# blairstar/NaturalDiffusion

Measured on AMD Instinct MI355X. Metric: images/sec at 15-step Natural Inference (CIFAR10 32x32, NCSN++), 3-stream throughput, higher is better.
Workload: dtype bf16; 1 GPU; CIFAR10 NI 15-step step_15_weight_173.npz B=512/GPU NCSN++ 61.8M bf16, ni_step fp64 history; nfe=15, batch_per_gpu=512, streams=3

## Files before the change

include/natinf_ncsnpp.h:

```cpp
#ifndef NATINF_NCSNPP_H
#define NATINF_NCSNPP_H

#include <stdint.h>
#include "natinf.h"

#ifdef __cplusplus
extern "C" {
#endif

typedef struct natinf_ncsnpp* natinf_ncsnpp_t;

#define NATINF_NCSNPP_KEEP_ACTIVATIONS 1
#define NATINF_NCSNPP_DDPM 2

int64_t natinf_ncsnpp_param_count(void);
int64_t natinf_ncsnpp_packed_bytes(void);
int64_t natinf_ncsnpp_handle_param_count(natinf_ncsnpp_t h);
int64_t natinf_ncsnpp_handle_packed_bytes(natinf_ncsnpp_t h);
int64_t natinf_ncsnpp_workspace_bytes(natinf_ncsnpp_t h, int max_batch);

int natinf_ncsnpp_create(natinf_ncsnpp_t* out, int flags);
int natinf_ncsnpp_destroy(natinf_ncsnpp_t h);

int natinf_ncsnpp_describe(natinf_ncsnpp_t h, char* buf, int cap);

int natinf_ncsnpp_load(natinf_ncsnpp_t h, const float* params_f32, int64_t n_params,
                       void* packed, int64_t packed_bytes, natinf_stream_t stream);

int natinf_ncsnpp_share(natinf_ncsnpp_t h, natinf_ncsnpp_t loaded);

int natinf_ncsnpp_forward(natinf_ncsnpp_t h, const float* x, const float* labels, float* out, int B,
                          void* workspace, int64_t workspace_bytes, natinf_stream_t stream);

int natinf_ncsnpp_describe_gemms(natinf_ncsnpp_t h, int B, char* buf, int cap);

int natinf_debug_gemm(int variant, int M, int N, int K0, int K1, int taps, int logW, int batch,
                      const void* a0, const void* a1, const void* b, const float* bias_n, void* c, int c_f32, float scale,
                      int iters, natinf_stream_t stream);
int natinf_debug_quant_fp8_rows(const float* w, void* q, float* row_scale, int rows, int cols, natinf_stream_t stream);
int natinf_debug_gemm_fused(int variant, int M, int N, int K, const void* a, const void* b, const float* bias_n, const float* bias_m,
                            const float* rowvec, const float* gate, int log_rows_per_sample, const void* resid_bf16, const float* resid_f32,
                            float scale, int act, void* c, int c_f32, float* gn_part, int* bm_out, int fp32_slab, natinf_stream_t stream);
int natinf_debug_set_conv_operand(int logW, const void* a1, int c1);
int natinf_debug_gemm_fp8(int M, int N, int K, const void* a8, const float* a_scale, const void* a_mx, const void* b8, const float* b_scale,
                          const float* bias_n, void* c, void* c_mx, int c_mode, int iters, natinf_stream_t stream);
int natinf_debug_conv_gn_up(int flags);
int natinf_debug_conv_gn(int res, int B, int N, int cin, int c1, const void* x, const float* scale, const float* shift, const void* w_packed, void* w_frag,
                         const void* a1, const float* bias_n, const void* resid, float out_scale, void* out, float* gn_part, int iters,
                         natinf_stream_t stream);
int natinf_set_gemm_variant(int variant);
int natinf_set_gemm_epilogue(int fp32_slab);
int natinf_set_gemm_pref512(int on);
int natinf_set_gemm_half_issue(int on);
int natinf_set_gemm_round_model(int on);
int natinf_set_gemm_w128(int on);
int natinf_set_gemm_raster(int rows);
int natinf_set_fuse_gn(int on);
int natinf_set_conv_gn_wide(int mask);
int natinf_set_conv_gn_w128(int mask);
int natinf_set_conv_gn_w128_min_k(int shape, int k);
int natinf_set_conv_gn_regw(int on);
int natinf_set_fuse_up(int on);
int natinf_set_fuse_head(int on);
int natinf_set_fuse_gn8(int on);
int natinf_set_fuse_gn4(int on);
int natinf_set_fuse_fin(int on);
int natinf_set_conv_gn_warm(int mask);
int natinf_set_attn256(int on);
int natinf_set_attn_proj(int on);
int natinf_set_attn_waves8(int on);
int natinf_set_attn_block(int on);
int natinf_set_attn_qkv(int on);
int natinf_set_conv_gn8_tile(int one_image);
int natinf_set_gemm_splitk(int on);
int natinf_debug_set_splitk_workspace(float* ws, int max_slices);
int natinf_debug_timestamps(void* dev_buf16);

int natinf_ncsnpp_profile(natinf_ncsnpp_t h, int enable);
int natinf_ncsnpp_profile_read(natinf_ncsnpp_t h, double* ms_by_class , int64_t* launches_by_class );

int natinf_gemm_profile(int enable);
int natinf_gemm_profile_read(char* buf, int cap);

int natinf_ncsnpp_debug_tap(natinf_ncsnpp_t h, int module_idx, float* out, int64_t capacity_elems,
                            natinf_stream_t stream);

#ifdef __cplusplus
}
#endif
#endif
```

naturaldiffusion_amd/_lib.py:

```python
from __future__ import annotations

import ctypes as C
import os
from pathlib import Path

os.environ.setdefault("GPU_MAX_HW_QUEUES", "8")

_HERE = Path(__file__).resolve().parent
LIB_PATH = Path(os.environ.get("NATINF_LIB", _HERE / "libnatinf.so"))

if not LIB_PATH.exists():
    raise ImportError(
        f"{LIB_PATH} not found: build it with `make -C {_HERE / 'csrc'}` "
        "(or `python -c 'import __graft_entry__ as g; g.build()'`). "
        "naturaldiffusion_amd has no CPU or eager-PyTorch fallback.")

lib = C.CDLL(str(LIB_PATH))

_p, _i32, _i64, _f32, _f64 = C.c_void_p, C.c_int, C.c_int64, C.c_float, C.c_double

SIGNATURES = {
    "natinf_abi_version": (C.c_int, []),
    "natinf_strerror": (C.c_char_p, [_i32]),
    "natinf_probe": (C.c_int, []),
    "natinf_step_f64hist": (C.c_int, [_p, _p, _p, _p, _p, _p, _p, _i32, _f64, _i32, _f64, _f64, _f32, _f32, _i64, _p]),
    "natinf_step_f32hist": (C.c_int, [_p, _p, _p, _p, _p, _p, _p, _i32, _f32, _i32, _f32, _f32, _f32, _f32, _i64, _p]),
    "natinf_weighted_sum_f64": (C.c_int, [_p, _p, _p, _p, _i32, _i64, _p]),
    "natinf_randn_philox_f32": (C.c_int, [_p, _i64, _i64, _p, _i64, _i64, C.c_uint64, _p]),
    "natinf_randn_philox_col_f32": (C.c_int, [_p, _i64, _i64, _p, _i64, _i64, C.c_uint64, C.c_uint32, _p]),
    "natinf_step_f64hist_noise": (C.c_int, [_p, _p, _p, _p, _p, _p, _p, _i32, _f64, _p, _p, _i32, _i32, _f64, _f64, _f32,
                                            C.c_uint64, _p, _i64, _i64, _i64, _i64, _p]),
    "natinf_to_pixel_u8": (C.c_int, [_p, _p, _i32, _i32, _i32, _i32, _i32, _p]),
    "natinf_step_f32prod": (C.c_int, [_p, _p, _p, _f32, _i64, _i64, _p, _p, _p, _p, _p, _i32, _f32, _p, _p, _i32,
                                      _i32, _f32, _f32, _i64, _p]),
    "natinf_step_f32prod_noise": (C.c_int, [_p, _p, _p, _f32, _i64, _i64, _p, _p, _p, _p, _p, _i32, _f32, _p, _p, _i32,
                                            _i32, _f32, _f32, C.c_uint64, _p, _i64, _i64, _i64, _p]),
    "natinf_weighted_sum_f32prod": (C.c_int, [_p, _p, _p, _p, _i32, _i64, _p]),
    "natinf_step_f16chain": (C.c_int, [_p, _p, _p, _p, _p, _p, _p, _p, _p, _i32, _f32, _f32, _i32, _f32, _f32, _f32,
                                       _f32, _i32, _i64, _p]),
    "natinf_weighted_mean_f16": (C.c_int, [_p, _p, _p, _p, _i32, _f32, _i64, _p]),
    "natinf_flow_input_f16": (C.c_int, [_p, _p, _p, _f32, _f32, _i64, _p]),
    "natinf_ncsnpp_param_count": (C.c_int64, []),
    "natinf_ncsnpp_workspace_bytes": (C.c_int64, [_p, _i32]),
    "natinf_ncsnpp_packed_bytes": (C.c_int64, []),
    "natinf_ncsnpp_handle_param_count": (_i64, [_p]),
    "natinf_ncsnpp_handle_packed_bytes": (_i64, [_p]),
    "natinf_ncsnpp_create": (C.c_int, [C.POINTER(_p), _i32]),
    "natinf_ncsnpp_describe": (C.c_int, [_p, C.c_char_p, _i32]),
    "natinf_ncsnpp_destroy": (C.c_int, [_p]),
    "natinf_ncsnpp_load": (C.c_int, [_p, _p, _i64, _p, _i64, _p]),
    "natinf_ncsnpp_share": (C.c_int, [_p, _p]),
    "natinf_ncsnpp_forward": (C.c_int, [_p, _p, _p, _p, _i32, _p, _i64, _p]),
    "natinf_ncsnpp_debug_tap": (C.c_int, [_p, _i32, _p, _i64, _p]),
    "natinf_ncsnpp_describe_gemms": (C.c_int, [_p, _i32, C.c_char_p, _i32]),
    "natinf_debug_gemm": (C.c_int, [_i32, _i32, _i32, _i32, _i32, _i32, _i32, _i32, _p, _p, _p, _p, _p, _i32, _f32, _i32, _p]),
    "natinf_set_gemm_variant": (C.c_int, [_i32]),
    "natinf_debug_timestamps": (C.c_int, [_p]),
    "natinf_set_gemm_epilogue": (C.c_int, [_i32]),
    "natinf_debug_gemm_fused": (C.c_int, [_i32, _i32, _i32, _i32, _p, _p, _p, _p, _p, _p, _i32, _p, _p, _f32, _i32, _p, _i32, _p, _p, _i32, _p]),
    "natinf_set_gemm_pref512": (C.c_int, [_i32]),
    "natinf_set_gemm_half_issue": (C.c_int, [_i32]),
    "natinf_set_gemm_raster": (C.c_int, [_i32]),
    "natinf_set_gemm_round_model": (C.c_int, [_i32]),
    "natinf_set_gemm_w128": (C.c_int, [_i32]),
    "natinf_set_fuse_gn": (C.c_int, [_i32]),
    "natinf_set_conv_gn_wide": (C.c_int, [_i32]),
    "natinf_set_attn_block": (C.c_int, [_i32]),
    "natinf_set_conv_gn_w128": (C.c_int, [_i32]),
    "natinf_set_conv_gn_w128_min_k": (C.c_int, [_i32, _i32]),
    "natinf_set_conv_gn_regw": (C.c_int, [_i32]),
    "natinf_set_fuse_up": (C.c_int, [_i32]),
    "natinf_set_fuse_head": (C.c_int, [_i32]),
    "natinf_set_fuse_gn8": (C.c_int, [_i32]),
    "natinf_set_fuse_gn4": (C.c_int, [_i32]),
    "natinf_set_fuse_fin": (C.c_int, [_i32]),
    "natinf_set_attn_proj": (C.c_int, [_i32]),
    "natinf_set_attn_waves8": (C.c_int, [_i32]),
    "natinf_set_attn_qkv": (C.c_int, [_i32]),
    "natinf_set_conv_gn_warm": (C.c_int, [_i32]),
    "natinf_set_attn256": (C.c_int, [_i32]),
    "natinf_set_conv_gn8_tile": (C.c_int, [_i32]),
    "natinf_set_gemm_splitk": (C.c_int, [_i32]),
    "natinf_debug_set_splitk_workspace": (C.c_int, [_p, _i32]),
    "natinf_debug_set_conv_operand": (C.c_int, [_i32, _p, _i32]),
    "natinf_debug_conv_gn": (C.c_int, [_i32, _i32, _i32, _i32, _i32, _p, _p, _p, _p, _p, _p, _p, _p, _f32, _p, _p, _i32, _p]),
    "natinf_debug_conv_gn_up": (C.c_int, [_i32]),
    "natinf_ncsnpp_profile": (C.c_int, [_p, _i32]),
    "natinf_ncsnpp_profile_read": (C.c_int, [_p, C.POINTER(C.c_double), C.POINTER(C.c_int64)]),
    "natinf_debug_quant_fp8_rows": (C.c_int, [_p, _p, _p, _i32, _i32, _p]),
    "natinf_debug_gemm_fp8": (C.c_int, [_i32, _i32, _i32, _p, _p, _p, _p, _p, _p, _p, _p, _i32, _i32, _p]),
    "natinf_dit_create": (C.c_int, [C.POINTER(_p), _i32, _i32, _i32, _i32]),
    "natinf_dit_create_sized": (C.c_int, [C.POINTER(_p), _i32, _i32, _i32, _i32, _i32]),
    "natinf_dit_input_size": (C.c_int, [_p]),
    "natinf_dit_attention_bf16": (C.c_int, [_p, _p, _p, _i32, _p, _i32, _i32, _i32, _i32, _i32, _i32, _p]),
    "natinf_dit_destroy": (C.c_int, [_p]),
    "natinf_dit_param_count": (C.c_int64, [_p]),
    "natinf_dit_packed_bytes": (C.c_int64, [_p]),
    "natinf_dit_workspace_bytes": (C.c_int64, [_p, _i32]),
    "natinf_dit_load": (C.c_int, [_p, _p, _i64, _p, _i64, _p]),
    "natinf_dit_forward": (C.c_int, [_p, _p, _p, _p, _p, _i32, _p, _i64, _p]),
    "natinf_mmdit_create": (C.c_int, [C.POINTER(_p), _i32, _i32, _i32, _i32, _i32, _i32, _i32, _i32]),
    "natinf_mmdit_destroy": (C.c_int, [_p]),
    "natinf_mmdit_param_count": (C.c_int64, [_p]),
    "natinf_mmdit_packed_bytes": (C.c_int64, [_p]),
    "natinf_mmdit_workspace_bytes": (C.c_int64, [_p, _i32]),
    "natinf_mmdit_load": (C.c_int, [_p, _p, _i64, _p, _i64, _p]),
    "natinf_mmdit_forward": (C.c_int, [_p, _p, _p, _p, _p, _p, _i32, _p, _i64, _p]),
    "natinf_attention_hd64_bf16": (C.c_int, [_p, _p, _i32, _i64, _p, _p, _i32, _i64, _i32, _i32, _i32, _i32, C.c_float, _p]),
    "natinf_inception_create": (C.c_int, [_p, _i32, _i32]),
    "natinf_inception_destroy": (C.c_int, [_p]),
    "natinf_set_inception_conv": (C.c_int, [_i32]),
    "natinf_debug_conv_ring": (C.c_int, [_i32] * 14 + [_p, _p, _p, _p, _p, _p, _i32, _p]),
    "natinf_inception_param_count": (_i64, [_p]),
    "natinf_inception_packed_bytes": (_i64, [_p]),
    "natinf_inception_workspace_bytes": (_i64, [_p, _i32]),
    "natinf_inception_load": (C.c_int, [_p, _p, _i64, _p, _i64, _p]),
    "natinf_inception_forward": (C.c_int, [_p, _p, _i32, _p, _i32, _p, _i64, _p]),
    "natinf_gemm_profile": (C.c_int, [_i32]),
    "natinf_gemm_profile_read": (C.c_int, [_p, _i32]),
    "natinf_set_mmdit_stream16": (C.c_int, [_i32]),
    "natinf_set_dit_stream16": (C.c_int, [_i32]),
    "natinf_set_mmdit_text_flat": (C.c_int, [_i32]),
    "natinf_attention_profile": (C.c_int, [_i32]),
    "natinf_set_mmdit_text_stream": (C.c_int, [_i32]),
    "natinf_set_flash_mode": (C.c_int, [_i32]),
    "natinf_attention_profile_read": (C.c_int, [_p, _p]),
    "natinf_vae_create": (C.c_int, [C.POINTER(_p), _i32, _i32]),
    "natinf_vae_destroy": (C.c_int, [_p]),
    "natinf_vae_param_count": (C.c_int64, [_p]),
    "natinf_vae_packed_bytes": (C.c_int64, [_p]),
    "natinf_vae_workspace_bytes": (C.c_int64, [_p, _i32]),
    "natinf_vae_load": (C.c_int, [_p, _p, _i64, _p, _i64, _p]),
    "natinf_vae_decode": (C.c_int, [_p, _p, _p, _i32, _p, _i64, _p]),
}

for _name, (_res, _args) in SIGNATURES.items():
    try:
        _fn = getattr(lib, _name)
    except AttributeError as e:
        raise ImportError(f"{LIB_PATH} does not export {_name}; rebuild it") from e
    _fn.restype, _fn.argtypes = _res, _args

SD3_CFG_ON_VELOCITY = 1


def check(rc: int, what: str) -> None:
    if rc != 0:
        raise RuntimeError(f"{what} failed: {lib.natinf_strerror(rc).decode()} ({rc})")


def stream_ptr(stream=None) -> int:
    import torch
    s = stream if stream is not None else torch.cuda.current_stream()
    return int(s.cuda_stream)


def ptr(t) -> int:
    return 0 if t is None else int(t.data_ptr())


def require_gpu() -> None:
    import torch
    if not torch.cuda.is_available():
        raise RuntimeError("naturaldiffusion_amd needs an MI355X (gfx950) GPU: torch.cuda.is_available() is False "
                           "and there is no CPU fallback")
    check(lib.natinf_probe(), "natinf_probe")
```

naturaldiffusion_amd/csrc/attn_blk256.h:

```cpp
#pragma once
#include "attn_qkv.h"
#include "attn256.h"

namespace ncsn {

constexpr int ABLK_STAGES = 4, ABLK_LDS_BYTES = ABLK_STAGES * A256_STAGE + QKV_BIAS_BYTES;

__device__ __forceinline__ float dpp_row_sum_tau(float a, float b) {
    asm volatile("s_nop 4" : "+v"(a), "+v"(b));
    a += __builtin_bit_cast(float, __builtin_amdgcn_update_dpp(0, __builtin_bit_cast(int, a), 0x128, 0xF, 0xF, true));
    b += __builtin_bit_cast(float, __builtin_amdgcn_update_dpp(0, __builtin_bit_cast(int, b), 0x128, 0xF, 0xF, true));
    asm volatile("" : "+v"(a), "+v"(b));
    a += __builtin_bit_cast(float, __builtin_amdgcn_update_dpp(0, __builtin_bit_cast(int, a), 0xB1, 0xF, 0xF, true));
    b += __builtin_bit_cast(float, __builtin_amdgcn_update_dpp(0, __builtin_bit_cast(int, b), 0xB1, 0xF, 0xF, true));
    asm volatile("" : "+v"(a), "+v"(b));
    a += __builtin_bit_cast(float, __builtin_amdgcn_update_dpp(0, __builtin_bit_cast(int, a), 0x4E, 0xF, 0xF, true));
    b += __builtin_bit_cast(float, __builtin_amdgcn_update_dpp(0, __builtin_bit_cast(int, b), 0x4E, 0xF, 0xF, true));
    asm volatile("" : "+v"(a), "+v"(b));
    float v = a + b;
    asm volatile("s_nop 1" : "+v"(v));
    v += __builtin_bit_cast(float, __builtin_amdgcn_update_dpp(0, __builtin_bit_cast(int, v), 0x141, 0xF, 0xF, true));
    asm volatile("" : "+v"(v));
    return v;
}
// ... 167 lines not shown
#pragma unroll
    for (int kt = 0; kt < NKT; ++kt) {
        asm volatile("s_waitcnt vmcnt(8)" ::: "memory");
        __builtin_amdgcn_s_barrier();
        issue(kt + 3);
        __builtin_amdgcn_sched_barrier(0);
        const unsigned char* sK = smem + (kt & 3) * A256_STAGE;
#pragma unroll
        for (int tl = 0; tl < 4; ++tl)
#pragma unroll
            for (int c = 0; c < 8; ++c) {
                const int row = 32 * (tl >> 1) + 4 * (tl & 1) + krow;
                const bf16x8 fa = *reinterpret_cast<const bf16x8*>(sK + row * 512 + (((4 * c + q) ^ r) << 4));
                acc[0][4 * kt + tl] = __builtin_amdgcn_mfma_f32_16x16x32_bf16(fa, qf[0][c], acc[0][4 * kt + tl], 0, 0, 0);
                acc[1][4 * kt + tl] = __builtin_amdgcn_mfma_f32_16x16x32_bf16(fa, qf[1][c], acc[1][4 * kt + tl], 0, 0, 0);
            }
    }
    float inv[2];
#pragma unroll
    for (int g = 0; g < 2; ++g) {
        float mx = -INFINITY;
#pragma unroll
        for (int t = 0; t < 16; ++t)
#pragma unroll
            for (int i = 0; i < 4; ++i) mx = fmaxf(mx, acc[g][t][i]);
        mx = fmaxf(mx, __shfl_xor(mx, 16));
        mx = fmaxf(mx, __shfl_xor(mx, 32));
        float sum = 0.f;
#pragma unroll
        for (int t = 0; t < 16; ++t)
#pragma unroll
            for (int i = 0; i < 4; ++i) { const float p = __expf((acc[g][t][i] - mx) * scale); acc[g][t][i] = p; sum += p; }
        sum += __shfl_xor(sum, 16);
        sum += __shfl_xor(sum, 32);
        inv[g] = 1.0f / sum;
        __builtin_amdgcn_sched_barrier(0);
    }
    bf16x8 pf[2][8];
#pragma unroll
    for (int c = 0; c < 8; ++c)
#pragma unroll
        for (int g = 0; g < 2; ++g)
#pragma unroll
            for (int i = 0; i < 4; ++i) { pf[g][c][i] = (bf16)(acc[g][2 * c][i] * inv[g]); pf[g][c][4 + i] = (bf16)(acc[g][2 * c + 1][i] * inv[g]); }
    __builtin_amdgcn_sched_barrier(0);
    f32x4 oacc[2][16];
#pragma unroll
    for (int dt = 0; dt < 16; ++dt) { oacc[0][dt] = f32x4{0.f, 0.f, 0.f, 0.f}; oacc[1][dt] = f32x4{0.f, 0.f, 0.f, 0.f}; }
#pragma unroll
    for (int vt = 0; vt < NKT; ++vt) {
        asm volatile("s_waitcnt vmcnt(8)" ::: "memory");
        __builtin_amdgcn_s_barrier();
        issue(NKT + vt + 3);
        __builtin_amdgcn_sched_barrier(0);
        const unsigned char* sV = smem + ((NKT + vt) & 3) * A256_STAGE;
#pragma unroll
        for (int cc = 0; cc < 2; ++cc)
#pragma unroll
            for (int dt = 0; dt < 16; ++dt) {
                const bf16x8 fv = *reinterpret_cast<const bf16x8*>(sV + (16 * dt + r) * 128 + (((4 * cc + q) ^ (r >> 1)) << 4));
                oacc[0][dt] = __builtin_amdgcn_mfma_f32_16x16x32_bf16(fv, pf[0][2 * vt + cc], oacc[0][dt], 0, 0, 0);
                oacc[1][dt] = __builtin_amdgcn_mfma_f32_16x16x32_bf16(fv, pf[1][2 * vt + cc], oacc[1][dt], 0, 0, 0);
            }
    }
    bf16x8 of[2][8];
#pragma unroll
    for (int g = 0; g < 2; ++g)
#pragma unroll
        for (int kc = 0; kc < 8; ++kc)
#pragma unroll
            for (int i = 0; i < 4; ++i) { of[g][kc][i] = (bf16)oacc[g][2 * kc][i]; of[g][kc][4 + i] = (bf16)oacc[g][2 * kc + 1][i]; }
    __builtin_amdgcn_sched_barrier(0);
    int le;
    asm volatile("v_mbcnt_lo_u32_b32 %0, -1, 0\n\tv_mbcnt_hi_u32_b32 %0, -1, %0" : "=v"(le));
    const int re = le & 15, qe = le >> 4;
    float2* const sred = reinterpret_cast<float2*>(smem);
    float2 part[16];
#pragma unroll
    for (int t = 0; t < 4; ++t) {
        asm volatile("s_waitcnt vmcnt(0)" ::: "memory");
        __syncthreads();
        if (t + 3 < 4) issue(2 * NKT + t + 3);
        __builtin_amdgcn_sched_barrier(0);
        const unsigned char* sW = smem + ((2 * NKT + t) & 3) * A256_STAGE;
        f32x4 a3[2][4];
#pragma unroll
        for (int ntl = 0; ntl < 4; ++ntl) { a3[0][ntl] = f32x4{0.f, 0.f, 0.f, 0.f}; a3[1][ntl] = f32x4{0.f, 0.f, 0.f, 0.f}; }
#pragma unroll
        for (int ntl = 0; ntl < 4; ++ntl)
#pragma unroll
            for (int kc = 0; kc < 8; ++kc) {
                const bf16x8 fa = *reinterpret_cast<const bf16x8*>(sW + (ntl * 8 + kc) * 1024 + le * 16);
                a3[0][ntl] = __builtin_amdgcn_mfma_f32_16x16x32_bf16(fa, of[0][kc], a3[0][ntl], 0, 0, 0);
                a3[1][ntl] = __builtin_amdgcn_mfma_f32_16x16x32_bf16(fa, of[1][kc], a3[1][ntl], 0, 0, 0);
            }
#pragma unroll
        for (int pr = 0; pr < 2; ++pr) {
            const int n = 64 * t + 32 * pr + 8 * qe;
            const float4 b0 = *reinterpret_cast<const float4*>(b3 + n), b1 = *reinterpret_cast<const float4*>(b3 + n + 4);
            float s0[2], ss0[2], s1[2], ss1[2];
#pragma unroll
            for (int g = 0; g < 2; ++g) {
                const int64_t row = (int64_t)b * T + tok0 + 8 * (re >> 2) + 4 * g + (re & 3);
                const bf16x8 rx = *reinterpret_cast<const bf16x8*>(x + row * x_ld + n);
                const f32x4 lo = a3[g][2 * pr], hi = a3[g][2 * pr + 1];
                float v[8] = {lo[0] + b0.x, lo[1] + b0.y, lo[2] + b0.z, lo[3] + b0.w, hi[0] + b1.x, hi[1] + b1.y, hi[2] + b1.z, hi[3] + b1.w};
                bf16x8 w;
#pragma unroll
                for (int i = 0; i < 8; ++i) { v[i] = (v[i] + (float)rx[i]) * out_scale; w[i] = (bf16)v[i]; }
                *reinterpret_cast<bf16x8*>(o + row * o_ld + n) = w;
                s0[g] = (v[0] + v[1]) + (v[2] + v[3]);  ss0[g] = (v[0] * v[0] + v[1] * v[1]) + (v[2] * v[2] + v[3] * v[3]);
                s1[g] = (v[4] + v[5]) + (v[6] + v[7]);  ss1[g] = (v[4] * v[4] + v[5] * v[5]) + (v[6] * v[6] + v[7] * v[7]);
            }
            part[4 * t + 2 * pr] = make_float2(dpp_row_sum_tau(s0[0], s0[1]), dpp_row_sum_tau(ss0[0], ss0[1]));
            part[4 * t + 2 * pr + 1] = make_float2(dpp_row_sum_tau(s1[0], s1[1]), dpp_row_sum_tau(ss1[0], ss1[1]));
        }
    }
    if (gn_part) {
        __syncthreads();
        if (re == 0) {
#pragma unroll
            for (int k = 0; k < 16; ++k) sred[wave * 64 + 8 * (k >> 1) + 2 * qe + (k & 1)] = part[k];
        }
        __syncthreads();
        if (tid < 64) {
            float s = 0.f, ss = 0.f;
#pragma unroll
            for (int w = 0; w < 8; ++w) { s += sred[w * 64 + tid].x; ss += sred[w * 64 + tid].y; }
            gn_part[(int64_t)b * gn_quads + tid] = make_float2(s, ss);
        }
    }
}

constexpr int ABLK2_IMG = 131072, ABLK2_LDS_BYTES = ABLK2_IMG + A256_STAGE;
static_assert(4 * QKV_STAGE <= ABLK2_IMG && ABLK2_LDS_BYTES <= 163840, "the q phase's four stages inside the image's bytes; image + one W3 tile in 160 KB");

__global__ __launch_bounds__(256) void k_attn_fold_w(const float* __restrict__ w0, const float* __restrict__ w1, const float* __restrict__ w2, const float* __restrict__ w3,
                                                      const float* __restrict__ b0, const float* __restrict__ b2, const float* __restrict__ b3,
                                                      float* __restrict__ wqk, float* __restrict__ cq, float* __restrict__ wvo, float* __restrict__ bo)
{
    const int o = threadIdx.x, i = blockIdx.x;
    float a = 0.f, c = 0.f;
    if (i < 256) {
        for (int m = 0; m < 256; ++m) { a += w0[i * 256 + m] * w1[o * 256 + m]; c += w2[i * 256 + m] * w3[m * 256 + o]; }
        wqk[i * 256 + o] = a; wvo[i * 256 + o] = c;
    } else {
        for (int m = 0; m < 256; ++m) { a += b0[m] * w1[o * 256 + m]; c += b2[m] * w3[m * 256 + o]; }
        cq[o] = a; bo[o] = c + b3[o];
    }
}

__global__ __launch_bounds__(512, 1) void k_attn_blk256_v2(const bf16* __restrict__ x, int x_ld, const float* __restrict__ gsc, const float* __restrict__ gsh,
                                                          const bf16* __restrict__ wqf, const float* __restrict__ cq, float scale, const bf16* __restrict__ wvof,
                                                          const float* __restrict__ bo, bf16* __restrict__ o, int o_ld, float out_scale, float2* __restrict__ gn_part, int gn_quads)
{
    constexpr int T = 256, C = 256, NTQ = 8;
    extern __shared__ __attribute__((aligned(16))) unsigned char smem[];
    lds_poison();
    typedef __attribute__((address_space(3))) void lds_void;
    typedef __attribute__((address_space(3))) unsigned char lds_u8;
    const int tid = threadIdx.x, lane = tid & 63, r = lane & 15, q = lane >> 4;
    const int wave = __builtin_amdgcn_readfirstlane(tid >> 6);
    const int b = blockIdx.x;
    const int tok0 = wave * 32;
    const unsigned lds0 = (unsigned)(uintptr_t)((lds_u8*)smem);

    constexpr int NST = 4, AHEAD = NST - 1;
    auto issue_w = [&](int i) __attribute__((always_inline)) {
        unsigned char* st = smem + (i & (NST - 1)) * QKV_STAGE;
        int l;
        asm volatile("v_mbcnt_lo_u32_b32 %0, -1, 0\n\tv_mbcnt_hi_u32_b32 %0, -1, %0" : "=v"(l));
        const bf16* base = wqf + (int64_t)i * (QKV_STAGE / 2);
#pragma unroll
        for (int j = 0; j < QKV_STAGE / 8192; ++j) {
            const int p = wave * (QKV_STAGE / 8192) + j;
            __builtin_amdgcn_global_load_lds(base + p * 512 + l * 8, (lds_void*)(st + p * 1024), 16, 0, 0);
        }
    };
    issue_w(0); issue_w(1); issue_w(2);
    float* const sBias = reinterpret_cast<float*>(smem + ABLK2_IMG);
    const unsigned lds_bias = lds0 + ABLK2_IMG;
    if (tid < 64) reinterpret_cast<float4*>(sBias)[tid] = reinterpret_cast<const float4*>(cq)[tid];

    bf16x8 qf[2][8];
    {
        bf16x8 hf[2][8];
        {
            const bf16* xb = x + ((int64_t)b * T + tok0 + 8 * (r >> 2) + (r & 3)) * x_ld + 8 * q;
            bf16x8 raw[2][8];
#pragma unroll
            for (int g = 0; g < 2; ++g)
#pragma unroll
                for (int kc = 0; kc < 8; ++kc) raw[g][kc] = *reinterpret_cast<const bf16x8*>(xb + (int64_t)(4 * g) * x_ld + 32 * kc);
            const float* sc = gsc + (int64_t)b * C + 8 * q;
            const float* sh = gsh + (int64_t)b * C + 8 * q;
#pragma unroll
            for (int kc = 0; kc < 8; ++kc) {
                const float4 s0 = *reinterpret_cast<const float4*>(sc + 32 * kc), s1 = *reinterpret_cast<const float4*>(sc + 32 * kc + 4);
                const float4 h0 = *reinterpret_cast<const float4*>(sh + 32 * kc), h1 = *reinterpret_cast<const float4*>(sh + 32 * kc + 4);
                const float s[8] = {s0.x, s0.y, s0.z, s0.w, s1.x, s1.y, s1.z, s1.w}, h[8] = {h0.x, h0.y, h0.z, h0.w, h1.x, h1.y, h1.z, h1.w};
#pragma unroll
                for (int g = 0; g < 2; ++g)
#pragma unroll
                    for (int j = 0; j < 8; ++j) hf[g][kc][j] = (bf16)((float)raw[g][kc][j] * s[j] + h[j]);
            }
        }
        int le;
        asm volatile("v_mbcnt_lo_u32_b32 %0, -1, 0\n\tv_mbcnt_hi_u32_b32 %0, -1, %0" : "=v"(le));
        const int qe = le >> 4;
        auto q_tile = [&](auto t_tag, bf16x8 (&w)[2]) __attribute__((always_inline)) {
            constexpr int t = decltype(t_tag)::value;
            constexpr int ahead = 2 * ((t + 1 < NTQ) + (t + 2 < NTQ));
            asm volatile("s_waitcnt vmcnt(%0) lgkmcnt(0)" :: "n"(ahead) : "memory");
            __builtin_amdgcn_s_barrier();
            if constexpr (t + AHEAD < NTQ) issue_w(t + AHEAD);
            __builtin_amdgcn_sched_barrier(0);
            const unsigned char* sW = smem + (t & (NST - 1)) * QKV_STAGE;
            f32x4 a[2][2];
#pragma unroll
            for (int ntl = 0; ntl < 2; ++ntl) {
                a[ntl][0] = f32x4{0.f, 0.f, 0.f, 0.f}; a[ntl][1] = a[ntl][0];
#pragma unroll
                for (int kc = 0; kc < 8; ++kc) {
                    const bf16x8 fa = *reinterpret_cast<const bf16x8*>(sW + (ntl * 8 + kc) * 1024 + le * 16);
                    a[ntl][0] = __builtin_amdgcn_mfma_f32_16x16x32_bf16(fa, hf[0][kc], a[ntl][0], 0, 0, 0);
                    a[ntl][1] = __builtin_amdgcn_mfma_f32_16x16x32_bf16(fa, hf[1][kc], a[ntl][1], 0, 0, 0);
                }
            }
            const int n = 32 * t + 8 * qe;
            f32x4 b0, b1;
            asm volatile("ds_read_b128 %0, %2\n\tds_read_b128 %1, %2 offset:16" : "=&v"(b0), "=&v"(b1) : "v"(lds_bias + (unsigned)n * 4u) : "memory");
            asm volatile("s_waitcnt lgkmcnt(0)" : "+v"(b0), "+v"(b1) :: "memory");
#pragma unroll
            for (int g = 0; g < 2; ++g)
#pragma unroll
                for (int i = 0; i < 4; ++i) { w[g][i] = (bf16)(a[0][g][i] + b0[i]); w[g][4 + i] = (bf16)(a[1][g][i] + b1[i]); }
        };
        using std::integral_constant;
#define NATINF_BLK2_Q(t) { bf16x8 w[2]; q_tile(integral_constant<int, t>{}, w); qf[0][t] = w[0]; qf[1][t] = w[1]; }
        NATINF_BLK2_Q(0) NATINF_BLK2_Q(1) NATINF_BLK2_Q(2) NATINF_BLK2_Q(3) NATINF_BLK2_Q(4) NATINF_BLK2_Q(5) NATINF_BLK2_Q(6) NATINF_BLK2_Q(7)
#undef NATINF_BLK2_Q
        asm volatile("s_waitcnt vmcnt(0) lgkmcnt(0)" ::: "memory");
        __syncthreads();
#pragma unroll
        for (int g = 0; g < 2; ++g) {
            const int row = tok0 + 8 * (r >> 2) + 4 * g + (r & 3);
            const int key = 3 * (row & 1) + 4 * ((row >> 1) & 1) + 8 * ((row >> 3) & 1);
#pragma unroll
            for (int kc = 0; kc < 8; ++kc) *reinterpret_cast<bf16x8*>(smem + row * 512 + (((4 * kc + q) ^ key) << 4)) = hf[g][kc];
        }
    }
    __syncthreads();

    f32x4 acc[2][16];
#pragma unroll
    for (int t = 0; t < 16; ++t) { acc[0][t] = f32x4{0.f, 0.f, 0.f, 0.f}; acc[1][t] = f32x4{0.f, 0.f, 0.f, 0.f}; }
    {
        const int krow = 8 * (r >> 2) + (r & 3);
        const int keyr = 3 * (r & 1) + 4 * ((r >> 1) & 1) + 8 * ((r >> 2) & 1);
#pragma unroll
        for (int kt = 0; kt < 4; ++kt)
#pragma unroll
            for (int tl = 0; tl < 4; ++tl)
#pragma unroll
                for (int c = 0; c < 8; ++c) {
                    const int row = 64 * kt + 32 * (tl >> 1) + 4 * (tl & 1) + krow;
                    const bf16x8 fa = *reinterpret_cast<const bf16x8*>(smem + row * 512 + (((4 * c + q) ^ keyr) << 4));
                    acc[0][4 * kt + tl] = __builtin_amdgcn_mfma_f32_16x16x32_bf16(fa, qf[0][c], acc[0][4 * kt + tl], 0, 0, 0);
                    acc[1][4 * kt + tl] = __builtin_amdgcn_mfma_f32_16x16x32_bf16(fa, qf[1][c], acc[1][4 * kt + tl], 0, 0, 0);
                }
    }
    float inv[2];
#pragma unroll
    for (int g = 0; g < 2; ++g) {
        float mx = -INFINITY;
#pragma unroll
        for (int t = 0; t < 16; ++t)
#pragma unroll
            for (int i = 0; i < 4; ++i) mx = fmaxf(mx, acc[g][t][i]);
        mx = fmaxf(mx, __shfl_xor(mx, 16));
        mx = fmaxf(mx, __shfl_xor(mx, 32));
        float sum = 0.f;
#pragma unroll
        for (int t = 0; t < 16; ++t)
#pragma unroll
            for (int i = 0; i < 4; ++i) { const float p = __expf((acc[g][t][i] - mx) * scale); acc[g][t][i] = p; sum += p; }
        sum += __shfl_xor(sum, 16);
        sum += __shfl_xor(sum, 32);
        inv[g] = 1.0f / sum;
        __builtin_amdgcn_sched_barrier(0);
    }
    bf16x8 pf[2][8];
#pragma unroll
    for (int c = 0; c < 8; ++c)
#pragma unroll
        for (int g = 0; g < 2; ++g)
#pragma unroll
            for (int i = 0; i < 4; ++i) { pf[g][c][i] = (bf16)(acc[g][2 * c][i] * inv[g]); pf[g][c][4 + i] = (bf16)(acc[g][2 * c + 1][i] * inv[g]); }
    __builtin_amdgcn_sched_barrier(0);

    constexpr int NP = 4;
    auto issue3 = [&](int i) __attribute__((always_inline)) {
        unsigned char* st = i == 0 ? smem + ABLK2_IMG : smem + (i - 1) * A256_STAGE;
        int l;
        asm volatile("v_mbcnt_lo_u32_b32 %0, -1, 0\n\tv_mbcnt_hi_u32_b32 %0, -1, %0" : "=v"(l));
        const bf16* base = wvof + (int64_t)i * (A256_STAGE / 2);
#pragma unroll
        for (int j = 0; j < NP; ++j) {
            const int p = wave * NP + j;
            __builtin_amdgcn_global_load_lds(base + p * 512 + l * 8, (lds_void*)(st + p * 1024), 16, 0, 0);
        }
    };
    issue3(0);
    f32x4 oacc[2][16];
#pragma unroll
    for (int dt = 0; dt < 16; ++dt) { oacc[0][dt] = f32x4{0.f, 0.f, 0.f, 0.f}; oacc[1][dt] = f32x4{0.f, 0.f, 0.f, 0.f}; }
    {
        typedef short s16x4 __attribute__((ext_vector_type(4)));
        typedef __attribute__((address_space(3))) s16x4 lds_s16x4;
        const int qp = r >> 2, pp = r & 3;
        const int keyt = 3 * (qp & 1) + 4 * (qp >> 1) + 8 * (q & 1);
        const unsigned abase = lds0 + (unsigned)((8 * q + qp) * 512 + 8 * (pp & 1));
        const unsigned kh = (unsigned)(keyt >> 1), kl = (unsigned)(keyt & 1) ^ (unsigned)(pp >> 1);
#pragma unroll
        for (int vt = 0; vt < 4; ++vt)
#pragma unroll
            for (int cc = 0; cc < 2; ++cc)
#pragma unroll
                for (int dt = 0; dt < 16; ++dt) {
                    const unsigned a = abase + (unsigned)((64 * vt + 32 * cc) * 512) + ((((unsigned)dt ^ kh) << 5) | (kl << 4));
                    const s16x4 lo = __builtin_amdgcn_ds_read_tr16_b64_v4i16((lds_s16x4*)(uintptr_t)a);
                    const s16x4 hi = __builtin_amdgcn_ds_read_tr16_b64_v4i16((lds_s16x4*)(uintptr_t)(a + 4 * 512));
                    typedef short s16x8 __attribute__((ext_vector_type(8)));
                    const s16x8 both = {lo[0], lo[1], lo[2], lo[3], hi[0], hi[1], hi[2], hi[3]};
                    const bf16x8 fv = __builtin_bit_cast(bf16x8, both);
                    oacc[0][dt] = __builtin_amdgcn_mfma_f32_16x16x32_bf16(fv, pf[0][2 * vt + cc], oacc[0][dt], 0, 0, 0);
                    oacc[1][dt] = __builtin_amdgcn_mfma_f32_16x16x32_bf16(fv, pf[1][2 * vt + cc], oacc[1][dt], 0, 0, 0);
                }
    }
    bf16x8 of[2][8];
#pragma unroll
    for (int g = 0; g < 2; ++g)
#pragma unroll
        for (int kc = 0; kc < 8; ++kc)
#pragma unroll
            for (int i = 0; i < 4; ++i) { of[g][kc][i] = (bf16)oacc[g][2 * kc][i]; of[g][kc][4 + i] = (bf16)oacc[g][2 * kc + 1][i]; }
    __builtin_amdgcn_sched_barrier(0);
    asm volatile("s_waitcnt lgkmcnt(0)" ::: "memory");
    __syncthreads();
    issue3(1); issue3(2); issue3(3);

    int le;
    asm volatile("v_mbcnt_lo_u32_b32 %0, -1, 0\n\tv_mbcnt_hi_u32_b32 %0, -1, %0" : "=v"(le));
    const int re = le & 15, qe = le >> 4;
    float2 part[16];
#pragma unroll
    for (int t = 0; t < 4; ++t) {
        if (t == 0) {
            asm volatile("s_waitcnt vmcnt(0)" ::: "memory");
            __syncthreads();
        }
        __builtin_amdgcn_sched_barrier(0);
        const unsigned char* sW = t == 0 ? smem + ABLK2_IMG : smem + (t - 1) * A256_STAGE;
        f32x4 a3[2][4];
#pragma unroll
        for (int ntl = 0; ntl < 4; ++ntl) { a3[0][ntl] = f32x4{0.f, 0.f, 0.f, 0.f}; a3[1][ntl] = f32x4{0.f, 0.f, 0.f, 0.f}; }
#pragma unroll
        for (int ntl = 0; ntl < 4; ++ntl)
#pragma unroll
            for (int kc = 0; kc < 8; ++kc) {
                const bf16x8 fa = *reinterpret_cast<const bf16x8*>(sW + (ntl * 8 + kc) * 1024 + le * 16);
                a3[0][ntl] = __builtin_amdgcn_mfma_f32_16x16x32_bf16(fa, of[0][kc], a3[0][ntl], 0, 0, 0);
                a3[1][ntl] = __builtin_amdgcn_mfma_f32_16x16x32_bf16(fa, of[1][kc], a3[1][ntl], 0, 0, 0);
            }
#pragma unroll
        for (int pr = 0; pr < 2; ++pr) {
            const int n = 64 * t + 32 * pr + 8 * qe;
            const float4 b0 = *reinterpret_cast<const float4*>(bo + n), b1 = *reinterpret_cast<const float4*>(bo + n + 4);
            float s0[2], ss0[2], s1[2], ss1[2];
#pragma unroll
            for (int g = 0; g < 2; ++g) {
                const int64_t row = (int64_t)b * T + tok0 + 8 * (re >> 2) + 4 * g + (re & 3);
                const bf16x8 rx = *reinterpret_cast<const bf16x8*>(x + row * x_ld + n);
                const f32x4 lo = a3[g][2 * pr], hi = a3[g][2 * pr + 1];
                float v[8] = {lo[0] + b0.x, lo[1] + b0.y, lo[2] + b0.z, lo[3] + b0.w, hi[0] + b1.x, hi[1] + b1.y, hi[2] + b1.z, hi[3] + b1.w};
                bf16x8 w;
#pragma unroll
                for (int i = 0; i < 8; ++i) { v[i] = (v[i] + (float)rx[i]) * out_scale; w[i] = (bf16)v[i]; }
                *reinterpret_cast<bf16x8*>(o + row * o_ld + n) = w;
                s0[g] = (v[0] + v[1]) + (v[2] + v[3]);  ss0[g] = (v[0] * v[0] + v[1] * v[1]) + (v[2] * v[2] + v[3] * v[3]);
                s1[g] = (v[4] + v[5]) + (v[6] + v[7]);  ss1[g] = (v[4] * v[4] + v[5] * v[5]) + (v[6] * v[6] + v[7] * v[7]);
            }
            part[4 * t + 2 * pr] = make_float2(dpp_row_sum_tau(s0[0], s0[1]), dpp_row_sum_tau(ss0[0], ss0[1]));
            part[4 * t + 2 * pr + 1] = make_float2(dpp_row_sum_tau(s1[0], s1[1]), dpp_row_sum_tau(ss1[0], ss1[1]));
        }
    }
    if (gn_part) {
        float2* const sred = reinterpret_cast<float2*>(smem + 3 * A256_STAGE);
        __syncthreads();
        if (re == 0) {
#pragma unroll
            for (int k = 0; k < 16; ++k) sred[wave * 64 + 8 * (k >> 1) + 2 * qe + (k & 1)] = part[k];
        }
        __syncthreads();
        if (tid < 64) {
            float s = 0.f, ss = 0.f;
#pragma unroll
            for (int w = 0; w < 8; ++w) { s += sred[w * 64 + tid].x; ss += sred[w * 64 + tid].y; }
            gn_part[(int64_t)b * gn_quads + tid] = make_float2(s, ss);
        }
    }
}

}
```

naturaldiffusion_amd/csrc/gemm_dma.h:

```cpp
#pragma once
#include "ncsnpp_kernels.h"

#ifndef NATINF_SETPRIO
#define NATINF_SETPRIO 0
#endif

namespace ncsn {

template <int WM, int WN, int TM, int TN, int AVAIL>
struct EpiCfg {
    static constexpr int CROW = WN * TN * 16 + 4;
    static constexpr int bytes(int rb) { return WM * rb * 16 * CROW * 4; }
    static constexpr int RB = bytes(TM) <= AVAIL ? TM : (bytes(TM / 2) <= AVAIL ? TM / 2 : (bytes(TM / 4) <= AVAIL ? TM / 4 : 1));
    static constexpr int SLAB_ROWS = WM * RB * 16;
    static constexpr int SLAB_BYTES = bytes(RB);
    static_assert(TM % RB == 0 && SLAB_BYTES <= AVAIL, "epilogue staging does not fit");
    static constexpr int PROW = WN * TN * 16 * 2 + 16;
    static constexpr int PACK_SLAB = WM * TM * 16 * PROW;
    static constexpr int PACK_BYTES = PACK_SLAB + WM * WN * TN * 4 * 8;
    static constexpr bool PACK_OK = PACK_BYTES <= AVAIL;
    static constexpr int NEED = PACK_OK && PACK_BYTES > SLAB_BYTES ? PACK_BYTES : SLAB_BYTES;
};

template <int WM, int WN, int TM, int TN>
// ... 136 lines not shown
                asm volatile("");
#pragma unroll
                for (int e = 0; e < 4; ++e) v[e] += rbm[i];
            }
        }
        if constexpr (LAZY_RV) { v[0] += lrv[j].x; v[1] += lrv[j].y; v[2] += lrv[j].z; v[3] += lrv[j].w; }
        if constexpr (RES) {
            const bf16x4_t x = __builtin_bit_cast(bf16x4_t, rs[i][j]);
#pragma unroll
            for (int e = 0; e < 4; ++e) v[e] += (float)x[e];
        }
        if constexpr (SCALE_ALWAYS) {
#pragma unroll
            for (int e = 0; e < 4; ++e) v[e] *= scale;
        } else if (!OUT8 && scale != 1.0f) {
            asm volatile("");
#pragma unroll
            for (int e = 0; e < 4; ++e) v[e] *= scale;
        }
        if constexpr (ACT != ACT_NONE && !ACT8) apply_act4(v, ACT);
        if constexpr (GN) {
            gs[sm][j] += (v[0] + v[1]) + (v[2] + v[3]);
            gq[sm][j] += (v[0] * v[0] + v[1] * v[1]) + (v[2] * v[2] + v[3] * v[3]);
        }
    };
    auto act8 = [&](float (&v0)[4], float (&v1)[4]) __attribute__((always_inline)) {
        float v8[8] = {v0[0], v0[1], v0[2], v0[3], v1[0], v1[1], v1[2], v1[3]};
        if constexpr (ACT == ACT_GELU_TANH) gelu_tanh_fast8(v8); else silu_fast8(v8);
#pragma unroll
        for (int e = 0; e < 4; ++e) { v0[e] = v8[e]; v1[e] = v8[4 + e]; }
    };
    constexpr int EB = OUT8 ? 1 : 2;
    unsigned char* wbase = smem + (wm * TM * 16 + r) * PROW + (wn * TN * 16 + q * 4) * EB;
    if constexpr (!OUT8 && PAIR) {
        unsigned char* wb2 = smem + (wm * TM * 16 + r) * PROW + (wn * TN * 16) * 2;
#pragma unroll
        for (int i = 0; i < TM; ++i) {
            fetch_rowvec(i);
#pragma unroll
            for (int p = 0; p < TN / 2; ++p) {
                float v0[4], v1[4];
                value(i, 2 * p, v0);
                value(i, 2 * p + 1, v1);
                if constexpr (ACT8) act8(v0, v1);
                bf16x4_t o0, o1;
#pragma unroll
                for (int e = 0; e < 4; ++e) { o0[e] = (bf16)v0[e]; o1[e] = (bf16)v1[e]; }
                const uint2 a = __builtin_bit_cast(uint2, o0), b = __builtin_bit_cast(uint2, o1);
                *reinterpret_cast<uint4*>(wb2 + i * 16 * PROW + ncol(2 * p) * 2) = make_uint4(a.x, a.y, b.x, b.y);
            }
        }
    } else if constexpr (!OUT8) {
#pragma unroll
        for (int i = 0; i < TM; ++i) {
            fetch_rowvec(i);
            if constexpr (ACT8) {
#pragma unroll
                for (int j = 0; j < TN; j += 2) {
                    float v0[4], v1[4];
                    value(i, j, v0);
                    value(i, j + 1, v1);
                    act8(v0, v1);
                    bf16x4_t o0, o1;
#pragma unroll
                    for (int e = 0; e < 4; ++e) { o0[e] = (bf16)v0[e]; o1[e] = (bf16)v1[e]; }
                    *reinterpret_cast<uint2*>(wbase + i * 16 * PROW + j * 32) = __builtin_bit_cast(uint2, o0);
                    *reinterpret_cast<uint2*>(wbase + i * 16 * PROW + (j + 1) * 32) = __builtin_bit_cast(uint2, o1);
                }
            } else {
#pragma unroll
            for (int j = 0; j < TN; ++j) {
                float v[4];
                value(i, j, v);
                bf16x4_t o;
#pragma unroll
                for (int e = 0; e < 4; ++e) o[e] = (bf16)v[e];
                *reinterpret_cast<uint2*>(wbase + i * 16 * PROW + j * 32) = __builtin_bit_cast(uint2, o);
            }
            }
        }
    } else {
#pragma unroll
        for (int i = 0; i < TM; ++i) {
            const int m = m0 + wm * TM * 16 + i * 16 + r;
            unsigned e8pair = 0;
#pragma unroll
            for (int b = 0; b < TN / 2; ++b) {
                float v0[4], v1[4];
                value(i, 2 * b, v0);
                value(i, 2 * b + 1, v1);
                if constexpr (ACT8) act8(v0, v1);
                float amax = fmaxf(fmaxf(fmaxf(fabsf(v0[0]), fabsf(v0[1])), fmaxf(fabsf(v0[2]), fabsf(v0[3]))),
                                   fmaxf(fmaxf(fabsf(v1[0]), fabsf(v1[1])), fmaxf(fabsf(v1[2]), fabsf(v1[3]))));
                amax = group4_max_nonneg(amax);
                float inv;
                const unsigned e8 = mx_scale_of(amax, inv);
                *reinterpret_cast<unsigned*>(wbase + i * 16 * PROW + (2 * b) * 16) = pack_fp8x4<false>(v0[0] * inv, v0[1] * inv, v0[2] * inv, v0[3] * inv);
                *reinterpret_cast<unsigned*>(wbase + i * 16 * PROW + (2 * b + 1) * 16) = pack_fp8x4<false>(v1[0] * inv, v1[1] * inv, v1[2] * inv, v1[3] * inv);
                e8pair |= e8 << (8 * b);
            }
            static_assert(TN == 4, "scale bytes are stored as one 16-bit pair per row and wave");
            const int nb = n0 + wn * 64;
            if (q == 0 && m < g.M && nb < g.N)
                *reinterpret_cast<unsigned short*>(g.c_mx + (int64_t)z * g.c_mx_bs + ((int64_t)(nb >> 7) * g.c_mx_ld + m) * 4 + ((nb >> 5) & 3)) = (unsigned short)e8pair;
        }
    }
    float2* const sred = reinterpret_cast<float2*>(smem + Cfg::PACK_SLAB);
    if constexpr (GN) {
#pragma unroll
        for (int sm = 0; sm < NSAMP; ++sm)
#pragma unroll
            for (int j = 0; j < TN; ++j) { gs[sm][j] = dpp_row_sum(gs[sm][j]); gq[sm][j] = dpp_row_sum(gq[sm][j]); }
        if (r == 0) {
#pragma unroll
            for (int sm = 0; sm < NSAMP; ++sm)
#pragma unroll
                for (int j = 0; j < TN; ++j) sred[(NSAMP > 1 ? sm : wm) * (BN_ / 4) + wn * TN * 4 + (ncol(j) >> 2)] = make_float2(gs[sm][j], gq[sm][j]);
        }
    }
    __syncthreads();
    NATINF_TS(3);
    constexpr int CPR = BN_ * EB / 16, RPS = THREADS / CPR, NSW = BM_ / RPS;
    const int cchunk = tid % CPR, rsub = tid / CPR, n = n0 + cchunk * (16 / EB);
    if (n < g.N) {
        const unsigned char* src = smem + rsub * PROW + cchunk * 16;
        if constexpr (OUT8) {
            uint8_t* dst = reinterpret_cast<uint8_t*>(g.c) + (int64_t)z * g.c_bs + (int64_t)(m0 + rsub) * g.c_ld + n;
            if (m0 + BM_ <= g.M) SlabCopy<0, NSW, RPS, PROW, false>::run(src, dst, g.c_ld, m0 + rsub, g.M);
            else SlabCopy<0, NSW, RPS, PROW, true>::run(src, dst, g.c_ld, m0 + rsub, g.M);
        } else {
            bf16* dst = reinterpret_cast<bf16*>(g.c) + (int64_t)z * g.c_bs + (int64_t)(m0 + rsub) * g.c_ld + n;
            if (m0 + BM_ <= g.M) SlabCopy<0, NSW, RPS, PROW, false>::run(src, dst, g.c_ld, m0 + rsub, g.M);
            else SlabCopy<0, NSW, RPS, PROW, true>::run(src, dst, g.c_ld, m0 + rsub, g.M);
        }
    }
    NATINF_TS(4);
    if constexpr (GN) {
        if (tid < BN_ / 4 && n0 + tid * 4 < g.N) {
            if constexpr (NSAMP > 1) {
#pragma unroll
                for (int sm = 0; sm < NSAMP; ++sm)
                    if (m0 + sm * (BM_ / NSAMP) < g.M)
                        reinterpret_cast<float2*>(g.gn_part)[(int64_t)((m0 / BM_) * NSAMP + sm) * g.gn_quads + (n0 >> 2) + tid] = sred[sm * (BN_ / 4) + tid];
            } else {
                float s = 0.f, qq = 0.f;
#pragma unroll
                for (int w = 0; w < WM; ++w) { s += sred[w * (BN_ / 4) + tid].x; qq += sred[w * (BN_ / 4) + tid].y; }
                reinterpret_cast<float2*>(g.gn_part)[(int64_t)(m0 / BM_) * g.gn_quads + (n0 >> 2) + tid] = make_float2(s, qq);
            }
        }
        if constexpr (FIN) {
            static_assert((WM == 1 || NSAMP == 1) && BN_ <= THREADS, "one channel per thread; several samples per tile: one wave row");
            const int n = n0 + tid;
            if (g.fin_scale && tid < BN_ && n < g.N) {
                constexpr int HWS = BM_ / NSAMP;
                const int cg = g.fin_cg, qpg = cg >> 2, q0 = (n / cg) * qpg - (n0 >> 2);
                const float inv = 1.0f / (float)(cg * HWS), ga = g.fin_gamma[n], be = g.fin_beta[n];
#pragma unroll
                for (int sm = 0; sm < NSAMP; ++sm) {
                    if (m0 + sm * HWS >= g.M) break;
                    float s = 0.f, qq = 0.f;
                    for (int i = 0; i < qpg; ++i) {
                        if constexpr (NSAMP == 1 && WM > 1) {
                            float ps = 0.f, pq = 0.f;
#pragma unroll
                            for (int w = 0; w < WM; ++w) { ps += sred[w * (BN_ / 4) + q0 + i].x; pq += sred[w * (BN_ / 4) + q0 + i].y; }
                            s += ps; qq += pq;
                        } else { const float2 v = sred[sm * (BN_ / 4) + q0 + i]; s += v.x; qq += v.y; }
                    }
                    const float mean = s * inv;
                    float var = qq * inv - mean * mean;
                    var = var < 0.f ? 0.f : var;
                    const float sc = (1.0f / sqrtf(var + g.fin_eps)) * ga;
                    const int64_t o = (int64_t)(m0 / HWS + sm) * g.fin_ld + n;
                    g.fin_scale[o] = sc * g.fin_mul;
                    g.fin_shift[o] = (be - mean * sc) * g.fin_mul;
                }
            }
        }
    }
}

template <int WM, int WN, int TM, int TN, class Cfg>
__device__ __forceinline__ void dma_tile_epilogue(const GemmArgs& g, unsigned char* smem, f32x4 (&acc)[TM][TN],
                                                  int m0, int n0, int z, int tid, int lane, int wm, int wn)
{
    constexpr int BN_ = WN * TN * 16, BM_ = WM * TM * 16, THREADS = WM * WN * 64;
    float* sC = reinterpret_cast<float*>(smem);
    NATINF_TS(2);
#ifdef NATINF_DEV
    if (g.c_mode == 102) {
        float t = 0.f;
#pragma unroll
        for (int i = 0; i < TM; ++i)
#pragma unroll
            for (int j = 0; j < TN; ++j) t += acc[i][j][0] + acc[i][j][1] + acc[i][j][2] + acc[i][j][3];
        if (t == 123.456f) reinterpret_cast<float*>(g.c)[tid] = t;
        return;
    }
#endif
    float st[4] = {0.f, 0.f, 0.f, 0.f};
    constexpr int CROW = Cfg::CROW, RB = Cfg::RB, CPR = BN_ / 8;
    constexpr int ROWS_PER_SWEEP = THREADS / CPR;
    constexpr int NP = TM / RB, NSW = Cfg::SLAB_ROWS / ROWS_PER_SWEEP;
    uint4 keep[NSW][2];
    const int cchunk = tid % CPR, rsub = tid / CPR;
    const int n = n0 + cchunk * 8;
    const bool n_in = n < g.N;
    float bn[8];
#pragma unroll
    for (int q = 0; q < 8; ++q) bn[q] = 0.f;
    if (g.bias_n && n_in && g.c_mode != OUT_F32_NCHW) {
        const float4 u = *reinterpret_cast<const float4*>(g.bias_n + n), w = *reinterpret_cast<const float4*>(g.bias_n + n + 4);
        bn[0] = u.x; bn[1] = u.y; bn[2] = u.z; bn[3] = u.w; bn[4] = w.x; bn[5] = w.y; bn[6] = w.z; bn[7] = w.w;
    }
    float dn[8];
#pragma unroll
    for (int q = 0; q < 8; ++q) dn[q] = 1.f;
    if (g.deq_n && n_in) {
        const float* pd = g.deq_n + (int64_t)z * g.deq_n_bs + n;
        const float4 u = *reinterpret_cast<const float4*>(pd), w = *reinterpret_cast<const float4*>(pd + 4);
        dn[0] = u.x; dn[1] = u.y; dn[2] = u.z; dn[3] = u.w; dn[4] = w.x; dn[5] = w.y; dn[6] = w.z; dn[7] = w.w;
    }
    asm volatile("s_waitcnt vmcnt(0)" : "+v"(dn[0]), "+v"(dn[1]), "+v"(dn[2]), "+v"(dn[3]), "+v"(dn[4]), "+v"(dn[5]), "+v"(dn[6]), "+v"(dn[7]));
    asm volatile("s_waitcnt vmcnt(0)" : "+v"(bn[0]), "+v"(bn[1]), "+v"(bn[2]), "+v"(bn[3]), "+v"(bn[4]), "+v"(bn[5]), "+v"(bn[6]), "+v"(bn[7]));
#pragma unroll
    for (int pass = 0; pass < NP; ++pass) {
        if (pass) __syncthreads();
#pragma unroll
        for (int ii = 0; ii < RB; ++ii)
#pragma unroll
            for (int j = 0; j < TN; ++j)
                *reinterpret_cast<f32x4*>(sC + (wm * RB * 16 + ii * 16 + (lane & 15)) * CROW + wn * TN * 16 + j * 16 + (lane >> 4) * 4) = acc[pass * RB + ii][j];
        __syncthreads();
        NATINF_TS(3 + 3 * pass);
        if (g.c_mode == OUT_F32_NCHW) {
            float* out = reinterpret_cast<float*>(g.c);
            const int nvalid = min(BN_, g.N - n0);
            for (int e = tid; e < Cfg::SLAB_ROWS * nvalid; e += THREADS) {
                const int s = e % Cfg::SLAB_ROWS, nn = e / Cfg::SLAB_ROWS;
                const int m = m0 + (s / (RB * 16)) * (TM * 16) + pass * RB * 16 + s % (RB * 16);
                if (m < g.M) {
                    float v = sC[s * CROW + nn];
                    if (g.bias_n) v += g.bias_n[n0 + nn];
                    v *= g.scale;
                    const int b = m >> g.logHW, p = m & ((1 << g.logHW) - 1);
                    out[((int64_t)b * g.N + n0 + nn) * ((int64_t)1 << g.logHW) + p] = v;
                }
            }
            continue;
        }
#pragma unroll
        for (int sw = 0; sw < NSW; ++sw) {
            const int s = sw * ROWS_PER_SWEEP + rsub;
            const int m = m0 + (s / (RB * 16)) * (TM * 16) + pass * RB * 16 + s % (RB * 16);
            if (m >= g.M || !n_in) continue;
            const float4 u = *reinterpret_cast<const float4*>(sC + s * CROW + cchunk * 8);
            const float4 w = *reinterpret_cast<const float4*>(sC + s * CROW + cchunk * 8 + 4);
            float v[8] = {u.x, u.y, u.z, u.w, w.x, w.y, w.z, w.w};
            if (g.deq_m || g.deq_n) {
                const float dm = g.deq_m ? g.deq_m[(int64_t)z * g.deq_m_bs + m] : 1.f;
#pragma unroll
                for (int q = 0; q < 8; ++q) v[q] *= dm * dn[q];
            }
#pragma unroll
            for (int q = 0; q < 8; ++q) v[q] += bn[q];
            if (g.bias_m) {
                const float bm = g.bias_m[m];
#pragma unroll
                for (int q = 0; q < 8; ++q) v[q] += bm;
            }
            if (g.rowvec) {
                const float* rv = g.rowvec + (int64_t)((m >> g.log_rows_per_sample) + z * g.z_samples) * g.rowvec_ld + n;
                const float4 s4 = *reinterpret_cast<const float4*>(rv), t4 = *reinterpret_cast<const float4*>(rv + 4);
                v[0] += s4.x; v[1] += s4.y; v[2] += s4.z; v[3] += s4.w; v[4] += t4.x; v[5] += t4.y; v[6] += t4.z; v[7] += t4.w;
            }
            if (g.gate) {
                const float* gv = g.gate + (int64_t)((m >> g.log_rows_per_sample) + z * g.z_samples) * g.gate_ld + n;
                const float4 s4 = *reinterpret_cast<const float4*>(gv), t4 = *reinterpret_cast<const float4*>(gv + 4);
                v[0] *= s4.x; v[1] *= s4.y; v[2] *= s4.z; v[3] *= s4.w; v[4] *= t4.x; v[5] *= t4.y; v[6] *= t4.z; v[7] *= t4.w;
            }
            if (g.resid) {
                const bf16x8 rs = *reinterpret_cast<const bf16x8*>(g.resid + (int64_t)z * g.c_bs + (int64_t)m * g.resid_ld + n);
#pragma unroll
                for (int q = 0; q < 8; ++q) v[q] += (float)rs[q];
            }
            if (g.resid_f32) {
                const float* rp = g.resid_f32 + (int64_t)z * g.c_bs + (int64_t)m * g.resid_f32_ld + n;
                const float4 s4 = *reinterpret_cast<const float4*>(rp), t4 = *reinterpret_cast<const float4*>(rp + 4);
                v[0] += s4.x; v[1] += s4.y; v[2] += s4.z; v[3] += s4.w; v[4] += t4.x; v[5] += t4.y; v[6] += t4.z; v[7] += t4.w;
            }
#pragma unroll
            for (int q = 0; q < 8; ++q) v[q] *= g.scale;
            apply_act8(v, g.act);
            if (g.gn_part) {
                st[0] += (v[0] + v[1]) + (v[2] + v[3]); st[1] += (v[0] * v[0] + v[1] * v[1]) + (v[2] * v[2] + v[3] * v[3]);
                st[2] += (v[4] + v[5]) + (v[6] + v[7]); st[3] += (v[4] * v[4] + v[5] * v[5]) + (v[6] * v[6] + v[7] * v[7]);
            }
            if (g.c_mode == OUT_BF16) {
                bf16x8 o;
#pragma unroll
                for (int q = 0; q < 8; ++q) o[q] = (bf16)v[q];
                keep[sw][0] = __builtin_bit_cast(uint4, o);
            } else if (g.c_mode == OUT_FP8_MX) {
                float amax = 0.f;
#pragma unroll
                for (int q = 0; q < 8; ++q) amax = fmaxf(amax, fabsf(v[q]));
                amax = fmaxf(amax, __shfl_xor(amax, 1));
                amax = fmaxf(amax, __shfl_xor(amax, 2));
                float inv;
                const unsigned e8 = mx_scale_of(amax, inv);
                keep[sw][0] = make_uint4(pack_fp8x4(v[0] * inv, v[1] * inv, v[2] * inv, v[3] * inv),
                                         pack_fp8x4(v[4] * inv, v[5] * inv, v[6] * inv, v[7] * inv), e8, 0u);
            } else {
                keep[sw][0] = __builtin_bit_cast(uint4, make_float4(v[0], v[1], v[2], v[3]));
                keep[sw][1] = __builtin_bit_cast(uint4, make_float4(v[4], v[5], v[6], v[7]));
            }
        }
        NATINF_TS(4 + 3 * pass);
#pragma unroll
        for (int sw = 0; sw < NSW; ++sw) {
            const int s = sw * ROWS_PER_SWEEP + rsub;
            const int m = m0 + (s / (RB * 16)) * (TM * 16) + pass * RB * 16 + s % (RB * 16);
            if (m >= g.M || !n_in) continue;
#ifdef NATINF_DEV
            if (g.c_mode == 103) {
                if (keep[sw][0].x == 0x12345678u) *reinterpret_cast<uint4*>(g.c) = keep[sw][0];
            } else
#endif
// ... 538 lines not shown
```

naturaldiffusion_amd/csrc/gemm_launch.h:

```cpp
#pragma once
#include <hip/hip_runtime.h>
#include <stdint.h>
#include <stdio.h>
#include <string.h>
#include <string>
#include <type_traits>
#include <utility>
#include <vector>

#include "ncsnpp_kernels.h"
#include "gemm_dma.h"
#include "gemm_w128.h"
#include "conv_gn2.h"
#include "gemm_fp8.h"

using namespace ncsn;

bool configure_conv_ring();
namespace { bool configure_ncsnpp_kernels();
            bool configure_dit_attention();
            bool configure_flash_attention(); }
namespace ncsn_cg3 { bool configure(); int tile_rows(int shape); int tile_cols(int shape); void launch(const void* gemm_args, int shape, int epi, void* stream); }

namespace {
// ... 194 lines not shown
    const bool n_ok256 = g.N % 256 == 0 || (w128 && g.N % 128 == 0);
    if (g_round_model && g.taps == 1 && !g.gn_part && g.batch == 1 && n_ok256 && K0 + K1 >= 1024 && mt256 * nt256 < 2 * NUM_CU) {
        const int64_t r256 = (mt256 * nt256 + NUM_CU - 1) / NUM_CU, r128 = (mt128 * nt128 + 2 * NUM_CU - 1) / (2 * NUM_CU);
        const int64_t c256 = w128 ? g_round_model_w128 : 15;
        if (mt128 * nt128 >= NUM_CU / 2) return c256 * r256 < 10 * r128 ? (w128 ? V_W128 : V_DMA_256x256_H) : V_DMA_128x128_P;
    }
    if (n_ok256 && K0 + K1 >= 1024 && mt256 * nt256 * g.batch >= NUM_CU) return w128 ? V_W128 : V_DMA_256x256_H;
    if (g_pref_512 && g.N <= 128 && K0 + K1 >= 1024 && ((g.M + 511) / 512) * g.batch >= 2 * NUM_CU &&
        (!g.gn_part || (g.taps == 9 && (1 << g.logHW) % 512 == 0)))
        return V_DMA_512x128_H;
    if (mt256 * nt128 * g.batch >= 2 * NUM_CU) return V_RING_256x128_W4;
    if (mt128 * nt128 * g.batch >= NUM_CU) return V_DMA_128x128_P;
    return V_RING_64x128;
}

int fp8_epi(const GemmArgs& g) {
    if (g.epi_fp32_slab || g.resid || g.gn_part) return 0;
    if ((g.rowvec || g.gate) && g.log_rows_per_sample < 30 && ((1 << g.log_rows_per_sample) % 256 != 0)) return 0;
    if (g.c_mode == OUT_F32 && g.resid_f32 && !g.bias_m && g.act == ACT_NONE && g.resid_f32_ld % 4 == 0 && g.c_ld % 4 == 0) return 3;
    if (g.resid_f32 || g.gate) return 0;
    if (g.c_mode == OUT_BF16 && g.act == ACT_NONE) return 1;
    if (g.c_mode == OUT_FP8_MX && g.act == ACT_GELU_TANH && g.c_mx && g.N % 32 == 0 && !g.bias_m && g.scale == 1.0f) return 2;
    return 0;
}
bool w128_fp8_ok(const GemmArgs& g) {
    return g.taps == 1 && !g.a1 && g.a0_C % 256 == 0 && g.N % 8 == 0 && g.M % 8 == 0 && (!g.a_mx || g.M % 256 == 0) &&
           (int64_t)g.M * g.a0_ld < (int64_t)1 << 32 && (int64_t)g.N * g.b_ld < (int64_t)1 << 32;
}
bool fp8_on_w128(const GemmArgs& g) { return g_w128 && w128_fp8_ok(g) && (fp8_epi(g) != 2 || g_w128 != 2); }
template <bool MXA>
void launch_gemm_fp8_t(const GemmArgs& g, hipStream_t s) {
    if (fp8_on_w128(g)) launch_family<FamF8W128<MXA>>(fp8_epi(g), g, s);
    else launch_family<FamF8<MXA>>(fp8_epi(g), g, s);
}
std::string gemm_row(int M, int N, int K0, int K1, int taps, int batch, const std::string& name, int epi) {
    char line[160];
    snprintf(line, sizeof(line), "%d %d %d %d %d %d %s/e%d", M, N, K0, K1, taps, batch, name.c_str(), epi);
    return line;
}
void record_gemm(const GemmArgs& g, const std::string& name, int epi) { *g_record += gemm_row(g.M, g.N, g.taps * g.a0_C, g.a1 ? g.a1_C : 0, g.taps, g.batch, name, epi) + "\n"; }
struct GemmProf {
    struct Rec { hipEvent_t a, b; std::string tag; };
    bool on = false; std::vector<Rec> ev; std::vector<std::pair<hipEvent_t, hipEvent_t>> pool;
    bool begin(Rec& r, hipStream_t s) {
        r.a = r.b = nullptr;
        if (!pool.empty()) { r.a = pool.back().first; r.b = pool.back().second; pool.pop_back(); }
        else if (hipEventCreate(&r.a) != hipSuccess || hipEventCreate(&r.b) != hipSuccess) { r.a = r.b = nullptr; (void)hipGetLastError(); return false; }
        (void)hipEventRecord(r.a, s);
        return true;
    }
    void end(Rec& r, hipStream_t s) { (void)hipEventRecord(r.b, s); ev.push_back(std::move(r)); }
} g_gemm_prof;
void launch_gemm_fp8(const GemmArgs& g, hipStream_t s) {
    GemmProf::Rec r;
    const bool prof = g_gemm_prof.on && !g_record && g_gemm_prof.begin(r, s);
    if (prof) r.tag = gemm_row(g.M, g.N, g.taps * g.a0_C, 0, g.taps, g.batch, std::string(fp8_on_w128(g) ? "w128_fp8" : "fp8_256x256") + (g.a_mx ? "_mxa" : ""), fp8_epi(g));
    if (g.a_mx) launch_gemm_fp8_t<true>(g, s); else launch_gemm_fp8_t<false>(g, s);
    if (prof) g_gemm_prof.end(r, s);
}

int packed_epi(const GemmArgs& g, int bm) {
    if (g.epi_fp32_slab || g.deq_m || g.deq_n || g.act == ACT_RELU) return 0;
    if (g.bias_m) return (g.c_mode == OUT_BF16 && !g.resid && !g.resid_f32 && !g.gate && !g.rowvec && !g.gn_part && g.act == ACT_NONE) ? 8 : 0;
    if ((g.rowvec || g.gate) && g.log_rows_per_sample < 30 && ((1 << g.log_rows_per_sample) % bm != 0)) return 0;
    if (g.c_mode == OUT_F32 && g.resid_f32 && !g.resid && !g.gn_part && g.act == ACT_NONE && g.resid_f32_ld % 4 == 0 && g.c_ld % 4 == 0) return 7;
    if (g.c_mode != OUT_BF16 || g.resid_f32 || g.gate) return 0;
    if (g.resid && (g.act != ACT_NONE || g.resid_ld % 4 != 0)) return 0;
    if (g.gn_part) return (g.act == ACT_NONE && g.M % bm == 0) ? (g.resid ? 6 : 2) : 0;
    if (g.resid) return 5;
    return g.act == ACT_NONE ? 1 : (g.act == ACT_SILU ? 3 : 4);
}
inline int effective_epi(int v, const GemmArgs& g) { const int e = packed_epi(g, variant_bm(v)); return ((epi_mask(v) >> e) & 1u) ? e : 0; }

thread_local int g_launch_error = 0;
thread_local bool g_fin_written = false;
int g_splitk = 1;
float* g_dbg_splitk_ws = nullptr; int g_dbg_splitk_max = 0;
int splitk_slices(const GemmArgs& g) {
    if (!g_splitk || !g.splitk_ws || g.splitk_max < 2 || g.batch != 1 || g.gn_scale || g.c_mode != OUT_BF16 || g.N % 8 || 256 % (g.N / 8)) return 1;
    if (g.gn_part && (g.M % SPLITK_ROWS || g.act != ACT_NONE || (g.taps == 9 && (1 << g.logHW) % SPLITK_ROWS))) return 1;
    if (g.bias_m || g.gate || g.resid_f32 || g.deq_m || g.deq_n) return 1;
    const int K0 = g.taps * g.a0_C, K1 = g.a1 ? g.a1_C : 0;
    if (K0 % 64 || K1 % 64 || (g.taps == 9 && !g.a0_padded) || K0 + K1 < 2048) return 1;
    const int64_t tiles = ((g.M + 127) / 128) * ((g.N + 127) / 128);
    if (tiles >= 2 * NUM_CU) return 1;
    int S = (int)((2 * NUM_CU + tiles - 1) / tiles);
    if (S > g.splitk_max) S = g.splitk_max;
    while (S > 1 && (K0 + K1) / 32 / S < 16) --S;
    return S;
}
int w128_splitk_slices(const GemmArgs& g) {
    if (!g_splitk || !g_w128 || !g.splitk_ws || g.splitk_max < 2 || g.batch != 1 || !w128_ok(g) || g.a0_C < 3072) return 1;
    if (g.c_mode != OUT_F32 || !g.resid_f32 || g.resid || g.rowvec || g.bias_m || g.gn_part || g.act != ACT_NONE || g.epi_fp32_slab || g.N % 4 || g.c_ld % 4 || g.resid_f32_ld % 4) return 1;
    const int64_t tiles = (int64_t)((g.M + 255) / 256) * ((g.N + 255) / 256) * g.batch;
    if (tiles * 2 > NUM_CU) return 1;
    int S = (int)(NUM_CU / tiles);
    if (S > g.splitk_max) S = g.splitk_max;
    while (S > 1 && g.a0_C / BK / S < 16) --S;
    return S;
}
int launch_gemm_run(const GemmArgs& g0, hipStream_t s);
int launch_gemm(const GemmArgs& g0, hipStream_t s) {
    if (!g_gemm_prof.on || g_record) return launch_gemm_run(g0, s);
    GemmProf::Rec r;
    std::string tag;
    g_record = &tag; (void)launch_gemm_run(g0, s); g_record = nullptr;
    while (!tag.empty() && tag.back() == '\n') tag.pop_back();
    if (!g_gemm_prof.begin(r, s)) return launch_gemm_run(g0, s);
    r.tag = std::move(tag);
    const int bm = launch_gemm_run(g0, s);
    g_gemm_prof.end(r, s);
    return bm;
}
int launch_gemm_run(const GemmArgs& g0, hipStream_t s) {
    if (g_force_variant == V_AUTO) {
        const int S8 = w128_splitk_slices(g0);
        if (S8 > 1) {
            if (g_record) { record_gemm(g0, "splitk" + std::to_string(S8) + "_w128_256x256", 7); return 256; }
            GemmArgs p = g0;
            p.splitk = S8; p.c = g0.splitk_ws; p.c_mode = OUT_F32;
            const int nM = (p.M + 255) / 256, nN = (p.N + 255) / 256;
            p.raster_g = 0;
            hipLaunchKernelGGL((k_gemm_w128<9>), dim3(nM * nN, S8, p.batch), dim3(256), W128Cfg::LDS_BYTES, s, p);
            const int64_t per = (int64_t)g0.M * (g0.N / 4);
            hipLaunchKernelGGL(k_splitk_reduce_f32, dim3((unsigned)((per + 255) / 256), (unsigned)g0.batch), dim3(256), 0, s, g0.splitk_ws, S8, (int64_t)g0.batch * g0.M * g0.N, g0.M, g0.N,
                               g0.bias_n, g0.gate, g0.gate_ld, g0.log_rows_per_sample, g0.z_samples, g0.resid_f32, g0.resid_f32_ld, g0.c_bs, g0.scale,
                               reinterpret_cast<float*>(g0.c), g0.c_ld, g0.stream_f16);
            return 256;
        }
    }
    const int S = g_force_variant == V_AUTO ? splitk_slices(g0) : 1;
    if (S > 1) {
        if (g_record) { record_gemm(g0, "splitk" + std::to_string(S) + "_ring128x128", 9); return SPLITK_ROWS; }
        GemmArgs p = g0;
        p.splitk = S; p.c = g0.splitk_ws; p.c_mode = OUT_F32; p.batch = S;
        p.bias_n = nullptr; p.rowvec = nullptr; p.resid = nullptr; p.scale = 1.0f; p.act = ACT_NONE; p.gn_part = nullptr;
        launch_tiles<CfgR128x128>(&k_gemm_ring<2, 2, 4, 4, 4, 9>, p, s);
        hipLaunchKernelGGL(k_splitk_reduce, dim3((unsigned)((g0.M + SPLITK_ROWS - 1) / SPLITK_ROWS)), dim3(256), 0, s, g0.splitk_ws, S, g0.M, g0.N,
                           g0.bias_n, g0.rowvec, g0.rowvec_ld, g0.log_rows_per_sample, reinterpret_cast<const bf16*>(g0.resid), g0.resid_ld, g0.scale,
                           g0.act, reinterpret_cast<bf16*>(g0.c), g0.c_ld, reinterpret_cast<float2*>(g0.gn_part), g0.gn_quads);
        return SPLITK_ROWS;
    }
    const GemmArgs& g = g0;
    const int v = choose_variant(g);
    if (g.taps == 9 && v != V_CONV_GN && g.a0_C % BK) {
        if (g_record) record_gemm(g, "invalid_conv3x3", 0); else g_launch_error = 1;
        return 256;
    }
    if (v == V_CONV_GN && !conv_gn_ok(g)) {
        if (g_record) record_gemm(g, "invalid_conv_gn", 0); else g_launch_error = 1;
        return 256;
    }
    if (g_record) {
        record_gemm(g, v == V_CONV_GN && conv_gn3_shape(g) >= 0 ? "conv_gn3" : variant_name(v), v == V_CONV_GN ? conv_gn_epi(g) : effective_epi(v, g));
        return v == V_CONV_GN ? conv_gn_part_rows(g) : variant_bm(v);
    }
    if (v == V_GENERIC) {
        const int nM = (g.M + BM - 1) / BM, nN = (g.N + BN - 1) / BN;
        hipLaunchKernelGGL(k_gemm_bf16, dim3(nM * nN, 1, g.batch), dim3(256), GEMM_LDS_BYTES, s, g);
    } else if (v == V_CONV_GN) {
        GemmArgs gw = g0;
        gw.w_warm = (g_cg_warm >> (g0.logW - 2)) & 1;
        const int e = conv_gn_epi(gw);
        if (const int sh3 = conv_gn3_shape(gw); sh3 >= 0) {
            ncsn_cg3::launch(&gw, sh3, e, (void*)s);
            g_fin_written = sh3 == 2 && gw.fin_scale && (e == 2 || e == 6) && gw.N == 256;
        } else launch_conv_gn2(ConvGnShapes{}, 1 << gw.logW, conv_gn_bm(gw), e, gw, s);
        return conv_gn_part_rows(gw);
    } else with_family(v, [&](auto f) { launch_family<decltype(f)>(effective_epi(v, g), g, s); });
    return variant_bm(v);
}
inline int grid1d(int64_t n, int block = 256, int cap = 4096) {
    int64_t g = (n + block - 1) / block; return (int)(g < 1 ? 1 : (g > cap ? cap : g));
}

}
```

naturaldiffusion_amd/csrc/ncsnpp.hip:

```cpp
#include <hip/hip_runtime.h>
#include <stdint.h>
#include <stdio.h>
#include <string.h>
#include <stdlib.h>
#include <functional>
#include <map>
#include <memory>
#include <string>
#include <vector>

#include "natinf_ncsnpp.h"
#include "gemm_launch.h"
#include "engine_core.h"
#include "head_conv.h"
#include "attn256.h"
#include "attn_qkv.h"
#include "attn_blk256.h"

namespace {

constexpr int NF = 128, IMG = 32, TEMB = 512, NLEVEL = 4;
constexpr int CH_MULT[NLEVEL] = {1, 2, 2, 2};
constexpr float GN_EPS = 1e-6f;
constexpr float INV_SQRT2 = 0.70710678118654752440f;
inline bool attn_at(int res) { return res == 16; }

enum Kind { K_LIN, K_CONV, K_RES, K_ATTN, K_GN, K_DOWN, K_UP };
const char* kind_name(int k) { static const char* n[] = {"lin", "conv", "res", "attn", "gn", "down", "up"}; return n[k]; }

struct Mod { int idx, kind, cin, cout, up, down, res; int64_t poff; };

enum { CLS_GEMM = 0, CLS_OTHER = 1, CLS_CONV_GN = 2, CLS_CONV_GN8 = 3, N_CLS = 4 };

int g_fuse_head = 1;
constexpr int ATTN_BLK_DEFAULT = 2;
int g_attn_blk = ATTN_BLK_DEFAULT;
int g_attn_qkv = 1;
int g_attn_w8 = 1;
int g_attn_proj = 1;
int g_fuse_gn8 = 1;
int g_fuse_fin = 3;
int g_fuse_gn4 = 1;
int g_fuse_gn = 1;
int g_fuse_up = 1;

}

struct natinf_ncsnpp : EngineCore {
    int flags = 0;
    std::vector<Mod> mods;
    std::vector<int> op_cls;
    bool prof = false;
    struct Rec { hipEvent_t a, b; int cls; };
    std::vector<Rec> recs;
    std::vector<hipEvent_t> pool;
    std::map<int, TRef> taps;
    uint64_t plan_sig = 0;
    int last_B = 0; unsigned char* last_ws = nullptr;
    std::vector<unsigned char> fin_done;
};

namespace {

bool configure_ncsnpp_kernels() {
    return hipFuncSetAttribute(reinterpret_cast<const void*>(&k_head_conv), hipFuncAttributeMaxDynamicSharedMemorySize, HeadConvCfg::LDS_BYTES) == hipSuccess &&
           hipFuncSetAttribute(reinterpret_cast<const void*>(&k_qkv256), hipFuncAttributeMaxDynamicSharedMemorySize, QKV_LDS_BYTES) == hipSuccess &&
           hipFuncSetAttribute(reinterpret_cast<const void*>(&k_attn256<false>), hipFuncAttributeMaxDynamicSharedMemorySize, A256_LDS_BYTES) == hipSuccess &&
           hipFuncSetAttribute(reinterpret_cast<const void*>(&k_attn256<true>), hipFuncAttributeMaxDynamicSharedMemorySize, A256_LDS_BYTES) == hipSuccess &&
           hipFuncSetAttribute(reinterpret_cast<const void*>(&k_attn256<true, 8>), hipFuncAttributeMaxDynamicSharedMemorySize, A256_LDS_BYTES) == hipSuccess &&
           hipFuncSetAttribute(reinterpret_cast<const void*>(&k_attn_blk256), hipFuncAttributeMaxDynamicSharedMemorySize, ABLK_LDS_BYTES) == hipSuccess &&
           hipFuncSetAttribute(reinterpret_cast<const void*>(&k_attn_blk256_v2), hipFuncAttributeMaxDynamicSharedMemorySize, ABLK2_LDS_BYTES) == hipSuccess;
}

struct Builder : PlanBuilder {
    natinf_ncsnpp& E;
    int dense_total = 0; int64_t dense_w = 0, dense_b = 0, dense_out = 0;

    const bool ddpm;
    const int NUM_RES;
    const float res_scale;
    explicit Builder(natinf_ncsnpp& e) : PlanBuilder(e), E(e), ddpm((e.flags & NATINF_NCSNPP_DDPM) != 0), NUM_RES(ddpm ? 2 : 4), res_scale(ddpm ? 1.0f : INV_SQRT2) {
        arena.keep = (e.flags & NATINF_NCSNPP_KEEP_ACTIVATIONS) != 0;
    }

    void op(int cls, OpFn f) { E.ops.push_back(std::move(f)); E.op_cls.push_back(cls); }

    void pack_conv(int64_t src, int64_t dst, int N, int Cin, int taps, int dst_ld, int koff, int tapstride, float wmul = 1.0f) {
        const int chunked = taps == 9 && Cin % BK == 0;
        E.packs.push_back([=](const PackCtx& p) {
            const int64_t n = (int64_t)N * Cin * taps;
            hipLaunchKernelGGL(k_pack_conv, dim3(grid1d(n, 256, 1 << 30)), dim3(256), 0, p.stream, p.params + src,
                               reinterpret_cast<bf16*>(p.packed + dst), N, Cin, taps, dst_ld, koff, tapstride, chunked, wmul);
        });
    }
    void pack_frag(int64_t src_packed, int64_t dst, int N, int ld, int cin, int c1) {
        E.packs.push_back([=](const PackCtx& p) {
            const int64_t n = (int64_t)(N / 16) * (9 * (cin / 32) + c1 / 32) * 64;
            hipLaunchKernelGGL(k_pack_frag, dim3(grid1d(n, 256, 1 << 30)), dim3(256), 0, p.stream, reinterpret_cast<const bf16*>(p.packed + src_packed),
                               reinterpret_cast<bf16*>(p.packed + dst), N, ld, cin, c1);
        });
    }
    void pack_transpose(int64_t src, int64_t dst, int K, int N, int dst_ld) {
        E.packs.push_back([=](const PackCtx& p) {
            hipLaunchKernelGGL(k_pack_transpose, dim3(grid1d((int64_t)K * N, 256, 1 << 30)), dim3(256), 0, p.stream,
                               p.params + src, reinterpret_cast<bf16*>(p.packed + dst), K, N, dst_ld);
        });
    }
    void pack_zero(int64_t dst, int64_t n) {
        E.packs.push_back([=](const PackCtx& p) {
            hipLaunchKernelGGL(k_fill_bf16_zero, dim3(grid1d(n, 256, 1 << 30)), dim3(256), 0, p.stream,
                               reinterpret_cast<bf16*>(p.packed + dst), n);
        });
    }

    struct GN { int64_t gamma, beta; };
    GN take_gn(int C) { GN g; g.gamma = pack_f32(take(C), C); g.beta = pack_f32(take(C), C); return g; }

    void emit_gn_stats(const TRef& x, GN gn, int64_t& sc, int64_t& sh, float out_mul = 1.0f) {
        if (emit_gn_from_parts(x, gn, sc, sh, out_mul)) return;
        const int HW = x.res * x.res;
        op(CLS_OTHER, [=](const Ctx& c) {
            hipLaunchKernelGGL(k_gn_stats, dim3(c.B), dim3(256), 0, c.stream, c.act(x), x.ld, x.C, HW,
                               c.w<float>(gn.gamma), c.w<float>(gn.beta), c.at<float>(sc), c.at<float>(sh), GN_EPS, out_mul);
        });
    }
    void emit_gn_apply(const TRef& x, int64_t sc, int64_t sh, const TRef& y, const TRef* xr, int act, int mode) {
        const int logW = ilog2(x.res), logHW = 2 * logW;
        const int rd = mode == RS_UP ? 2 * x.res : (mode == RS_DOWN ? x.res / 2 : x.res);
        const int rows_per_img = rd + 2 * y.pad;
        const TRef xrr = xr ? *xr : TRef();
        op(CLS_OTHER, [=](const Ctx& c) {
            hipLaunchKernelGGL(k_gn_apply, dim3((unsigned)((rows_per_img + GN_ROWS - 1) / GN_ROWS), (unsigned)c.B), dim3(256), 0, c.stream, c.act(x), x.ld, x.C,
                               logW, logHW, c.at<float>(sc), c.at<float>(sh), c.act(y),
                               xrr.off >= 0 ? c.act(xrr) : (bf16*)nullptr, act, mode, y.pad);
        });
    }
    TRef new_act(int res, int C, int pad = 0) {
        TRef t; t.off = arena.alloc((int64_t)(res + 2 * pad) * (res + 2 * pad) * C * 2); t.C = C; t.ld = C; t.res = res; t.pad = pad;
        return t;
    }

    void emit_res(const Mod& m, const TRef& x, const TRef& out) {
        const int cin = m.cin, cout = m.cout;
        const int ro = m.up ? m.res * 2 : (m.down ? m.res / 2 : m.res);
        const bool shortcut = cin != cout || m.up || m.down;
        const GN gn0 = take_gn(cin);
        const int64_t p_c0w = take((int64_t)cout * cin * 9), p_c0b = take(cout);
        const int64_t p_dw = take((int64_t)cout * TEMB), p_db = take(cout);
        const GN gn1 = take_gn(cout);
        const int64_t p_c1w = take((int64_t)cout * cout * 9), p_c1b = take(cout);
        const int64_t p_c2w = shortcut ? take((int64_t)cout * cin) : -1, p_c2b = shortcut ? take(cout) : -1;

        const int K0a = 9 * cin, K1tot = 9 * cout + (shortcut ? cin : 0);
        const bool fusable_res = g_fuse_gn && (ro == 32 || ro == 16 || (ro == 8 && g_fuse_gn8 && cout % 256 == 0) || (ro == 4 && g_fuse_gn4 && cout % 256 == 0));
        const bool fuse1 = fusable_res && cout % BK == 0;
        const bool fuse_up = fuse1 && ro > 8 && g_fuse_up && m.up && cin % BK == 0 && cout % 128 == 0;
        const bool fuse = (fusable_res && !m.up && !m.down && cin % BK == 0) || fuse_up;
        const float LOG2E = 1.4426950408889634f, LN2 = 0.6931471805599453f;
        const float gn_mul = fuse ? -LOG2E : 1.0f, w_mul = fuse ? -LN2 : 1.0f, gn_mul1 = fuse1 ? -LOG2E : 1.0f, w_mul1 = fuse1 ? -LN2 : 1.0f;
        const int64_t w0 = wres((int64_t)cout * K0a * 2), w1 = wres((int64_t)cout * K1tot * 2);
        pack_conv(p_c0w, w0, cout, cin, 9, K0a, 0, cin, w_mul);
        pack_conv(p_c1w, w1, cout, cout, 9, K1tot, 0, cout, w_mul1);
        if (shortcut && !ddpm) pack_conv(p_c2w, w1, cout, cin, 1, K1tot, 9 * cout, cin);
        if (shortcut && ddpm) pack_transpose(p_c2w, w1 + (int64_t)9 * cout * 2, cin, cout, K1tot);
        const int64_t w0f = (fuse && cout % 16 == 0) ? wres((int64_t)cout * K0a * 2) : -1, w1f = (fuse1 && cout % 16 == 0) ? wres((int64_t)cout * K1tot * 2) : -1;
        if (w0f >= 0) pack_frag(w0, w0f, cout, K0a, cin, 0);
        if (w1f >= 0) pack_frag(w1, w1f, cout, K1tot, cout, shortcut ? cin : 0);
        const int64_t b0 = pack_f32(p_c0b, cout), b1 = pack_f32(p_c1b, cout, shortcut ? p_c2b : -1);
        const int drow = dense_rows_next;
        pack_conv(p_dw, dense_w + (int64_t)drow * TEMB * 2, cout, TEMB, 1, TEMB, 0, TEMB);
        pack_f32_at(p_db, cout, dense_b + (int64_t)drow * 4);
        dense_rows_next += cout;

        const int64_t own_sc = arena.alloc((int64_t)std::max(cin, cout) * 4), own_sh = arena.alloc((int64_t)std::max(cin, cout) * 4);
        int64_t sc = own_sc, sh = own_sh;
        emit_gn_stats(x, gn0, sc, sh, gn_mul);
        TRef h, xr;
        if (!fuse) {
            h = new_act(ro, cin, 1);
            if (m.up || m.down) xr = new_act(ro, cin);
            emit_gn_apply(x, sc, sh, h, (m.up || m.down) ? &xr : nullptr, ACT_SILU, m.up ? RS_UP : (m.down ? RS_DOWN : RS_NONE));
        }

        const int SK_MAX = 4;
        const int64_t skws = (ro <= 8) ? arena.alloc((int64_t)SK_MAX * ro * ro * cout * 4) : -1;
        TRef t = new_act(ro, cout);
        const Part pt = register_output(t, fuse);
        const int logW = ilog2(ro), logHW = 2 * logW, HWo = ro * ro;
        const int dtotal = dense_total; const int64_t dout = dense_out;
        op(fuse ? (ro <= 8 ? CLS_CONV_GN8 : CLS_CONV_GN) : CLS_GEMM, [=](const Ctx& c) {
            GemmArgs g = gemm_defaults();
            if (fuse) { g.a0 = c.act(x); g.a0_ld = x.ld; g.gn_scale = c.at<float>(sc); g.gn_shift = c.at<float>(sh); g.gn_ld = cin; g.gn_folded = 1; g.a0_up = fuse_up; }
            else { g.a0 = c.act(h); g.a0_ld = h.ld; g.a0_padded = 1; }
            g.a0_C = cin; g.taps = 9; g.logW = logW; g.logHW = logHW;
            g.M = c.B * HWo; g.N = cout; g.b = c.w<bf16>(w0); g.b_ld = K0a;
            if (w0f >= 0) g.b_frag = c.w<bf16>(w0f);
            g.bias_n = c.w<float>(b0);
            g.rowvec = c.at<float>(dout) + drow; g.rowvec_ld = dtotal; g.log_rows_per_sample = logHW;
            if (skws >= 0) { g.splitk_ws = c.at<float>(skws); g.splitk_max = SK_MAX; }
            g.c = c.act(t); g.c_ld = t.ld;
            if (pt.valid) { g.gn_part = c.at<float>(pt.off); g.gn_quads = pt.quads; set_fin(g, pt, c); }
            g_fin_written = false;
            const int bm = launch_gemm(g, c.stream);
            if (pt.valid) c.part_bm[pt.id] = bm;
            if (pt.fin && pt.fin->check) c.fin_done[pt.id] = g_fin_written;
        });
        if (!fuse) arena.release(h.off);
        int64_t sc1 = own_sc, sh1 = own_sh;
        emit_gn_stats(t, gn1, sc1, sh1, gn_mul1);
        TRef u;
        if (!fuse1) {
            u = new_act(ro, cout, 1);
            emit_gn_apply(t, sc1, sh1, u, nullptr, ACT_SILU, RS_NONE);
            arena.release(t.off);
        }
        if (pt.valid) arena.release(pt.off);
        const TRef xs = ((m.up || m.down) && !fuse_up) ? xr : x;
        const float rs = res_scale;
        const Part po = register_output(out, fuse1);
        op(fuse1 ? (ro <= 8 ? CLS_CONV_GN8 : CLS_CONV_GN) : CLS_GEMM, [=](const Ctx& c) {
            GemmArgs g = gemm_defaults();
            if (fuse1) { g.a0 = c.act(t); g.a0_ld = t.ld; g.gn_scale = c.at<float>(sc1); g.gn_shift = c.at<float>(sh1); g.gn_ld = cout; g.gn_folded = 1; }
            else { g.a0 = c.act(u); g.a0_ld = u.ld; g.a0_padded = 1; }
            g.a0_C = cout; g.taps = 9; g.logW = logW; g.logHW = logHW;
            if (shortcut) { g.a1 = c.act(xs); g.a1_ld = xs.ld; g.a1_C = cin; g.a1_up = fuse_up; }
            else { g.resid = c.act(xs); g.resid_ld = xs.ld; }
            g.M = c.B * HWo; g.N = cout; g.b = c.w<bf16>(w1); g.b_ld = K1tot;
            if (w1f >= 0) g.b_frag = c.w<bf16>(w1f);
            g.bias_n = c.w<float>(b1); g.scale = rs;
            if (skws >= 0) { g.splitk_ws = c.at<float>(skws); g.splitk_max = SK_MAX; }
            g.c = c.act(out); g.c_ld = out.ld;
            if (po.valid) { g.gn_part = c.at<float>(po.off); g.gn_quads = po.quads; set_fin(g, po, c); }
            g_fin_written = false;
            const int bm = launch_gemm(g, c.stream);
            if (po.valid) c.part_bm[po.id] = bm;
            if (po.fin && po.fin->check) c.fin_done[po.id] = g_fin_written;
        });
        if (skws >= 0) arena.release(skws);
        if (fuse1) arena.release(t.off); else arena.release(u.off);
        if ((m.up || m.down) && !fuse_up) arena.release(xr.off);
        arena.release(own_sc); arena.release(own_sh);
        if (sc != own_sc) { arena.release(sc); arena.release(sh); }
        if (sc1 != own_sc) { arena.release(sc1); arena.release(sh1); }
        E.taps[m.idx] = out;
    }

    void emit_attn(const Mod& m, const TRef& x, const TRef& out) {
        const int C = m.cin, T = m.res * m.res;
        const GN gn = take_gn(C);
        int64_t pw[4], pb[4];
        for (int i = 0; i < 4; ++i) { pw[i] = take((int64_t)C * C); pb[i] = take(C); }
        const int64_t wqk = wres((int64_t)2 * C * C * 2), wv = wres((int64_t)C * C * 2), w3 = wres((int64_t)C * C * 2);
        pack_transpose(pw[0], wqk, C, C, C);
        pack_transpose(pw[1], wqk + (int64_t)C * C * 2, C, C, C);
        pack_transpose(pw[2], wv, C, C, C);
        pack_transpose(pw[3], w3, C, C, C);
        const int64_t bqk = wres((int64_t)2 * C * 4);
        pack_f32_at(pb[0], C, bqk); pack_f32_at(pb[1], C, bqk + (int64_t)C * 4);
        const int64_t bv = pack_f32(pb[2], C), b3 = pack_f32(pb[3], C);

        const int64_t own_sc = arena.alloc((int64_t)C * 4), own_sh = arena.alloc((int64_t)C * 4);
        int64_t sc = own_sc, sh = own_sh;
        emit_gn_stats(x, gn, sc, sh);
        const bool fuse_qkv = T == 256 && C == 256 && g_attn_qkv;
        TRef h = new_act(m.res, C);
        if (!fuse_qkv) emit_gn_apply(x, sc, sh, h, nullptr, ACT_NONE, RS_NONE);
        const int64_t qk = arena.alloc((int64_t)T * 2 * C * 2), vT = arena.alloc((int64_t)C * T * 2);
        const bool blk = fuse_qkv && g_attn_proj && g_attn_w8 && g_attn_blk;
        int64_t wqkvf = -1;
        const int64_t sc_q = sc, sh_q = sh;
        if (fuse_qkv) {
            wqkvf = wres((int64_t)3 * C * C * 2);
            const int64_t s0 = pw[0], s1 = pw[1], s2 = pw[2];
            E.packs.push_back([=](const PackCtx& p) {
                hipLaunchKernelGGL(k_pack_qkv_w, dim3(3 * 256), dim3(256), 0, p.stream, p.params + s0, p.params + s1, p.params + s2, reinterpret_cast<bf16*>(p.packed + wqkvf));
            });
            const int64_t sc_ = sc, sh_ = sh;
            if (!blk)
            op(CLS_GEMM, [=](const Ctx& c) {
                if (g_record) return;
                hipLaunchKernelGGL(k_qkv256, dim3((unsigned)c.B), dim3(512), QKV_LDS_BYTES, c.stream, (const bf16*)c.act(x), x.ld, c.at<float>(sc_), c.at<float>(sh_),
                                   c.w<bf16>(wqkvf), c.w<float>(bqk), c.w<float>(bv), c.at<bf16>(qk), c.at<bf16>(vT));
            });
        }
        if (!fuse_qkv)
        op(CLS_GEMM, [=](const Ctx& c) {
            GemmArgs g = gemm_defaults();
            g.a0 = c.act(h); g.a0_ld = C; g.a0_C = C; g.M = c.B * T; g.N = 2 * C;
            g.b = c.w<bf16>(wqk); g.b_ld = C; g.bias_n = c.w<float>(bqk);
            g.c = c.at<bf16>(qk); g.c_ld = 2 * C;
            launch_gemm(g, c.stream);
        });
        if (!fuse_qkv)
        op(CLS_GEMM, [=](const Ctx& c) {
            GemmArgs g = gemm_defaults();
            g.a0 = c.w<bf16>(wv); g.a0_ld = C; g.a0_C = C; g.a_bs = 0; g.M = C; g.N = T;
            g.b = c.act(h); g.b_ld = C; g.b_bs = (int64_t)T * C; g.bias_m = c.w<float>(bv);
            g.c = c.at<bf16>(vT); g.c_ld = T; g.c_bs = (int64_t)C * T; g.batch = c.B;
            launch_gemm(g, c.stream);
        });
        arena.release(h.off);
        const bool proj = T == 256 && C == 256 && g_attn_proj;
        int64_t w3f = -1;
        if (proj) {
            w3f = wres((int64_t)C * C * 2);
            const int64_t src = pw[3];
            E.packs.push_back([=](const PackCtx& p) {
                hipLaunchKernelGGL(k_pack_attn_w3, dim3(256), dim3(256), 0, p.stream, p.params + src, reinterpret_cast<bf16*>(p.packed + w3f));
            });
        }
        const bool blk2 = blk && g_attn_blk == 2;
        int64_t wqf2 = -1, wvof2 = -1, cq2 = -1, bo2 = -1;
        if (blk2) {
            const int64_t fq = wres((int64_t)C * C * 4), fv = wres((int64_t)C * C * 4);
            cq2 = wres((int64_t)C * 4); bo2 = wres((int64_t)C * 4);
            wqf2 = wres((int64_t)C * C * 2); wvof2 = wres((int64_t)C * C * 2);
            const int64_t w0_ = pw[0], w1_ = pw[1], w2_ = pw[2], w3_ = pw[3], b0_ = pb[0], b2_ = pb[2], b3_ = pb[3], cq_ = cq2, bo_ = bo2, wq_ = wqf2, wv_ = wvof2;
            E.packs.push_back([=](const PackCtx& p) {
                float* fqp = reinterpret_cast<float*>(p.packed + fq); float* fvp = reinterpret_cast<float*>(p.packed + fv);
                hipLaunchKernelGGL(k_attn_fold_w, dim3(257), dim3(256), 0, p.stream, p.params + w0_, p.params + w1_, p.params + w2_, p.params + w3_, p.params + b0_, p.params + b2_,
                                   p.params + b3_, fqp, reinterpret_cast<float*>(p.packed + cq_), fvp, reinterpret_cast<float*>(p.packed + bo_));
                hipLaunchKernelGGL(k_pack_qkv_w, dim3(256), dim3(256), 0, p.stream, (const float*)fqp, (const float*)fqp, (const float*)fqp, reinterpret_cast<bf16*>(p.packed + wq_), 1);
                hipLaunchKernelGGL(k_pack_attn_w3, dim3(256), dim3(256), 0, p.stream, (const float*)fvp, reinterpret_cast<bf16*>(p.packed + wv_));
            });
        }
        const Part po_attn = proj ? register_output(out) : Part();
        const float rs_attn = res_scale;
        TRef O = new_act(m.res, C);
        if (T == 256 && C == 256) {
            op(CLS_GEMM, [=](const Ctx& c) {
                if (g_record) return;
                if (blk2) {
                    hipLaunchKernelGGL(k_attn_blk256_v2, dim3((unsigned)c.B), dim3(512), ABLK2_LDS_BYTES, c.stream, (const bf16*)c.act(x), x.ld, c.at<float>(sc_q), c.at<float>(sh_q),
                                       c.w<bf16>(wqf2), c.w<float>(cq2), 1.0f / sqrtf((float)C), c.w<bf16>(wvof2), c.w<float>(bo2),
                                       c.act(out), out.ld, rs_attn, po_attn.valid ? c.at<float2>(po_attn.off) : (float2*)nullptr, po_attn.quads);
                    if (po_attn.valid) c.part_bm[po_attn.id] = 256;
                } else if (blk) {
                    hipLaunchKernelGGL(k_attn_blk256, dim3((unsigned)c.B), dim3(512), ABLK_LDS_BYTES, c.stream, (const bf16*)c.act(x), x.ld, c.at<float>(sc_q), c.at<float>(sh_q),
                                       c.w<bf16>(wqkvf), c.w<float>(bqk), c.w<float>(bv), c.at<bf16>(qk), c.at<bf16>(vT), 1.0f / sqrtf((float)C), c.w<bf16>(w3f), c.w<float>(b3),
                                       c.act(out), out.ld, rs_attn, po_attn.valid ? c.at<float2>(po_attn.off) : (float2*)nullptr, po_attn.quads);
                    if (po_attn.valid) c.part_bm[po_attn.id] = 256;
                } else if (proj) {
                    if (g_attn_w8) {
                        hipLaunchKernelGGL((k_attn256<true, 8>), dim3((unsigned)c.B), dim3(512), A256_LDS_BYTES, c.stream, c.at<bf16>(qk), 2 * C, C, c.at<bf16>(vT), c.act(out), out.ld,
                                           1.0f / sqrtf((float)C), c.w<bf16>(w3f), c.w<float>(b3), (const bf16*)c.act(x), x.ld, rs_attn,
                                           po_attn.valid ? c.at<float2>(po_attn.off) : (float2*)nullptr, po_attn.quads);
                        if (po_attn.valid) c.part_bm[po_attn.id] = 256;
                    } else {
                    hipLaunchKernelGGL(k_attn256<true>, dim3((unsigned)(2 * c.B)), dim3(256), A256_LDS_BYTES, c.stream, c.at<bf16>(qk), 2 * C, C, c.at<bf16>(vT), c.act(out), out.ld,
                                       1.0f / sqrtf((float)C), c.w<bf16>(w3f), c.w<float>(b3), (const bf16*)c.act(x), x.ld, rs_attn,
                                       po_attn.valid ? c.at<float2>(po_attn.off) : (float2*)nullptr, po_attn.quads);
                    if (po_attn.valid) c.part_bm[po_attn.id] = 128;
                    }
                }
                else
                    hipLaunchKernelGGL(k_attn256<false>, dim3((unsigned)(2 * c.B)), dim3(256), A256_LDS_BYTES, c.stream, c.at<bf16>(qk), 2 * C, C, c.at<bf16>(vT), c.act(O), C,
                                       1.0f / sqrtf((float)C), (const bf16*)nullptr, (const float*)nullptr, (const bf16*)nullptr, 0, 1.0f, (float2*)nullptr, 0);
            });
            arena.release(vT); arena.release(qk);
        } else {
        const int64_t S = arena.alloc((int64_t)T * T * 4);
            op(CLS_GEMM, [=](const Ctx& c) {
                GemmArgs g = gemm_defaults();
                g.a0 = c.at<bf16>(qk); g.a0_ld = 2 * C; g.a0_C = C; g.a_bs = (int64_t)T * 2 * C; g.M = T; g.N = T;
                g.b = c.at<bf16>(qk) + C; g.b_ld = 2 * C; g.b_bs = (int64_t)T * 2 * C;
                g.scale = 1.0f / sqrtf((float)C);
                g.c = c.at<float>(S); g.c_ld = T; g.c_bs = (int64_t)T * T; g.c_mode = OUT_F32; g.batch = c.B;
                launch_gemm(g, c.stream);
            });
            const int64_t P = arena.alloc((int64_t)T * T * 2);
            op(CLS_OTHER, [=](const Ctx& c) {
                const int64_t rows = (int64_t)c.B * T;
                hipLaunchKernelGGL(k_softmax_rows, dim3((unsigned)((rows + 3) / 4)), dim3(256), 0, c.stream,
                                   c.at<float>(S), c.at<bf16>(P), T, rows);
            });
            arena.release(S);
            op(CLS_GEMM, [=](const Ctx& c) {
                GemmArgs g = gemm_defaults();
                g.a0 = c.at<bf16>(P); g.a0_ld = T; g.a0_C = T; g.a_bs = (int64_t)T * T; g.M = T; g.N = C;
                g.b = c.at<bf16>(vT); g.b_ld = T; g.b_bs = (int64_t)C * T;
                g.c = c.act(O); g.c_ld = C; g.c_bs = (int64_t)T * C; g.batch = c.B;
                launch_gemm(g, c.stream);
            });
            arena.release(P); arena.release(vT); arena.release(qk);
        }
        if (proj) {
            arena.release(O.off); arena.release(own_sc); arena.release(own_sh);
            if (sc != own_sc) { arena.release(sc); arena.release(sh); }
            E.taps[m.idx] = out;
            return;
        }
        const Part po = register_output(out);
        const float rs = res_scale;
        op(CLS_GEMM, [=](const Ctx& c) {
            GemmArgs g = gemm_defaults();
            g.a0 = c.act(O); g.a0_ld = C; g.a0_C = C; g.M = c.B * T; g.N = C;
            g.b = c.w<bf16>(w3); g.b_ld = C; g.bias_n = c.w<float>(b3);
            g.resid = c.act(x); g.resid_ld = x.ld; g.scale = rs;
            g.c = c.act(out); g.c_ld = out.ld;
            if (po.valid) { g.gn_part = c.at<float>(po.off); g.gn_quads = po.quads; }
            const int bm = launch_gemm(g, c.stream);
            if (po.valid) c.part_bm[po.id] = bm;
        });
        arena.release(O.off); arena.release(own_sc); arena.release(own_sh);
        if (sc != own_sc) { arena.release(sc); arena.release(sh); }
        E.taps[m.idx] = out;
    }

    void emit_downconv(const Mod& m, const TRef& x, const TRef& out) {
        const int C = m.cin, ro = m.res / 2, Kd = 9 * C;
        const int64_t pw = take((int64_t)C * C * 9), pb = take(C);
        const int64_t w = wres((int64_t)C * Kd * 2);
        E.packs.push_back([=](const PackCtx& p) {
            const int64_t n = (int64_t)C * C * 9;
            hipLaunchKernelGGL(k_pack_conv, dim3(grid1d(n, 256, 1 << 30)), dim3(256), 0, p.stream, p.params + pw, reinterpret_cast<bf16*>(p.packed + w), C, C, 9, Kd, 0, C, 0, 1.0f);
        });
        const int64_t b = pack_f32(pb, C);
        const int64_t col = arena.alloc((int64_t)ro * ro * Kd * 2);
        const Part po = register_output(out);
        const int rin = m.res;
        op(CLS_GEMM, [=](const Ctx& c) {
            const int64_t M = (int64_t)c.B * ro * ro;
            if (!g_record) {
                const int64_t total = M * (Kd / 8);
                hipLaunchKernelGGL(k_inc_im2col, dim3(grid1d(total, 256, 1 << 30)), dim3(256), 0, c.stream, c.act(x), rin, rin, x.ld, C, 3, 3, 2, 0, 0, ro, ro, Kd,
                                   c.at<bf16>(col), total);
            }
            GemmArgs g = gemm_defaults();
            g.a0 = c.at<bf16>(col); g.a0_ld = Kd; g.a0_C = Kd; g.M = (int)M; g.N = C; g.b = c.w<bf16>(w); g.b_ld = Kd; g.bias_n = c.w<float>(b);
            g.log_rows_per_sample = 2 * ilog2(ro); g.logHW = 2 * ilog2(ro); g.logW = ilog2(ro);
            g.c = c.act(out); g.c_ld = out.ld;
            if (po.valid) { g.gn_part = c.at<float>(po.off); g.gn_quads = po.quads; }
            const int bm = launch_gemm(g, c.stream);
            if (po.valid) c.part_bm[po.id] = bm;
        });
        arena.release(col);
        E.taps[m.idx] = out;
    }
    int64_t ident_sc = -1, ident_sh = -1;
    void emit_upconv(const Mod& m, const TRef& x, const TRef& out) {
        const int C = m.cin, ro = m.res * 2, Ku = 9 * C;
        const int64_t pw = take((int64_t)C * C * 9), pb = take(C);
        const int64_t w = wres((int64_t)C * Ku * 2);
        pack_conv(pw, w, C, C, 9, Ku, 0, C);
        const int64_t b = pack_f32(pb, C);
        if (ident_sc < 0) {
            ident_sc = arena.alloc((int64_t)2 * NF * 4); ident_sh = arena.alloc((int64_t)2 * NF * 4);
            const int64_t isc = ident_sc, ish = ident_sh;
            op(CLS_OTHER, [=](const Ctx& c) {
                const int64_t n = (int64_t)c.B * 2 * NF;
                hipLaunchKernelGGL(k_fill_f32, dim3(grid1d(n, 256, 1 << 30)), dim3(256), 0, c.stream, c.at<float>(isc), 1.0f, n);
                hipLaunchKernelGGL(k_fill_f32, dim3(grid1d(n, 256, 1 << 30)), dim3(256), 0, c.stream, c.at<float>(ish), 0.0f, n);
            });
        }
        TRef u = new_act(ro, C, 1);
        emit_gn_apply(x, ident_sc, ident_sh, u, nullptr, ACT_NONE, RS_UP);
        const Part po = register_output(out);
        const int logW = ilog2(ro);
        op(CLS_GEMM, [=](const Ctx& c) {
            GemmArgs g = gemm_defaults();
            g.a0 = c.act(u); g.a0_ld = u.ld; g.a0_C = C; g.taps = 9; g.logW = logW; g.logHW = 2 * logW; g.a0_padded = 1;
            g.M = c.B * ro * ro; g.N = C; g.b = c.w<bf16>(w); g.b_ld = Ku; g.bias_n = c.w<float>(b); g.log_rows_per_sample = 2 * logW;
            g.c = c.act(out); g.c_ld = out.ld;
            if (po.valid) { g.gn_part = c.at<float>(po.off); g.gn_quads = po.quads; }
            const int bm = launch_gemm(g, c.stream);
            if (po.valid) c.part_bm[po.id] = bm;
        });
        arena.release(u.off);
        E.taps[m.idx] = out;
    }

    int dense_rows_next = 0;

    struct Fin { int64_t sc = -1, sh = -1, gamma = -1, beta = -1; int C = 0; float out_mul = 1.0f; bool claimed = false, check = false; };
    struct Part { int64_t off = -1; int quads = 0, id = -1, res = 0; bool valid = false; std::shared_ptr<Fin> fin; };
    static void set_fin(GemmArgs& g, const Part& p, const Ctx& c) {
        if (!p.fin || !p.fin->claimed) return;
        const Fin& f = *p.fin;
        g.fin_scale = c.at<float>(f.sc); g.fin_shift = c.at<float>(f.sh); g.fin_gamma = c.w<float>(f.gamma); g.fin_beta = c.w<float>(f.beta);
        g.fin_ld = f.C; g.fin_cg = f.C / 32; g.fin_mul = f.out_mul; g.fin_eps = GN_EPS;
    }
    std::map<std::pair<int64_t, int>, Part> parts;
    int n_parts = 0;
    static bool fusable(int res) { return res >= 16; }
    Part new_part(int res, int C) {
        Part p; p.quads = C / 4; p.res = res; p.id = n_parts++; p.valid = true;
        p.off = arena.alloc((int64_t)std::max(res * res / 64, 1) * p.quads * 8);
        return p;
    }
    Part register_output(const TRef& out, bool fused8 = false) {
        Part p;
        if (fusable(out.res) || (out.res <= 8 && fused8)) p = new_part(out.res, out.C);
        if (p.valid && out.res <= 8 && fused8 && (g_fuse_fin & 1) && out.C == 256) {
            p.fin = std::make_shared<Fin>();
            p.fin->sc = arena.alloc((int64_t)out.C * 4); p.fin->sh = arena.alloc((int64_t)out.C * 4); p.fin->C = out.C;
        }
        if (p.valid && out.res == 16 && fused8 && (g_fuse_fin & 2) && out.C == 256 && !ddpm) {
            p.fin = std::make_shared<Fin>();
            p.fin->sc = arena.alloc((int64_t)out.C * 4); p.fin->sh = arena.alloc((int64_t)out.C * 4); p.fin->C = out.C; p.fin->check = true;
        }
        parts[{out.off, out.coff}] = p;
        return p;
    }
    bool emit_gn_from_parts(const TRef& x, GN gn, int64_t& sc, int64_t& sh, float out_mul) {
        std::vector<Part> src;
        int ch = 0;
        while (ch < x.C) {
            auto it = parts.find({x.off, x.coff + ch});
            if (it == parts.end() || !it->second.valid || it->second.res != x.res) return false;
            src.push_back(it->second);
            ch += it->second.quads * 4;
        }
        if (ch != x.C || src.empty() || src.size() > 2) return false;
        const Part p0 = src[0], p1 = src.size() > 1 ? src[1] : Part();
        const int HW = x.res * x.res, C = x.C;
        if (src.size() == 1 && p0.fin && !p0.fin->claimed && p0.fin->C == C) {
            Fin& f = *p0.fin;
            f.gamma = gn.gamma; f.beta = gn.beta; f.out_mul = out_mul; f.claimed = true;
            sc = f.sc; sh = f.sh;
            if (f.check) {
                const std::shared_ptr<Fin> fp = p0.fin;
                const int64_t fsc = f.sc, fsh = f.sh;
                op(CLS_OTHER, [=](const Ctx& c) {
                    if (c.fin_done[p0.id]) return;
                    hipLaunchKernelGGL(k_gn_finalize, dim3(c.B), dim3(256), 0, c.stream, c.at<float2>(p0.off), HW / c.part_bm[p0.id], p0.quads, (const float2*)nullptr, 0, 0, C, HW,
                                       c.w<float>(gn.gamma), c.w<float>(gn.beta), c.at<float>(fsc), c.at<float>(fsh), GN_EPS, out_mul);
                });
            }
            return true;
        }
        const int64_t sc_ = sc, sh_ = sh;
        op(CLS_OTHER, [=](const Ctx& c) {
            const int tps0 = HW / c.part_bm[p0.id], tps1 = p1.valid ? HW / c.part_bm[p1.id] : 0;
            hipLaunchKernelGGL(k_gn_finalize, dim3(c.B), dim3(256), 0, c.stream, c.at<float2>(p0.off), tps0, p0.quads,
                               p1.valid ? c.at<float2>(p1.off) : (const float2*)nullptr, tps1, p1.valid ? p1.quads : 0, C, HW,
                               c.w<float>(gn.gamma), c.w<float>(gn.beta), c.at<float>(sc_), c.at<float>(sh_), GN_EPS, out_mul);
        });
        return true;
    }

    void list_modules() {
        auto add = [&](int kind, int cin, int cout, int up, int down, int res) {
            Mod m; m.idx = (int)E.mods.size(); m.kind = kind; m.cin = cin; m.cout = cout; m.up = up; m.down = down; m.res = res; m.poff = 0;
            E.mods.push_back(m);
        };
        add(K_LIN, NF, TEMB, 0, 0, 0); add(K_LIN, TEMB, TEMB, 0, 0, 0); add(K_CONV, 3, NF, 0, 0, IMG);
        std::vector<int> skip = {NF};
        int ch = NF, res = IMG;
        for (int l = 0; l < NLEVEL; ++l) {
            for (int b = 0; b < NUM_RES; ++b) {
                add(K_RES, ch, NF * CH_MULT[l], 0, 0, res); ch = NF * CH_MULT[l];
                if (attn_at(res)) add(K_ATTN, ch, ch, 0, 0, res);
                skip.push_back(ch);
            }
            if (l != NLEVEL - 1) { if (ddpm) add(K_DOWN, ch, ch, 0, 0, res); else add(K_RES, ch, ch, 0, 1, res); res /= 2; skip.push_back(ch); }
        }
        add(K_RES, ch, ch, 0, 0, res); add(K_ATTN, ch, ch, 0, 0, res); add(K_RES, ch, ch, 0, 0, res);
        for (int l = NLEVEL - 1; l >= 0; --l) {
            for (int b = 0; b < NUM_RES + 1; ++b) { add(K_RES, ch + skip.back(), NF * CH_MULT[l], 0, 0, res); skip.pop_back(); ch = NF * CH_MULT[l]; }
            if (attn_at(res)) add(K_ATTN, ch, ch, 0, 0, res);
            if (l != 0) { if (ddpm) add(K_UP, ch, ch, 0, 0, res); else add(K_RES, ch, ch, 1, 0, res); res *= 2; }
        }
        add(K_GN, ch, ch, 0, 0, res); add(K_CONV, ch, 3, 0, 0, res);
    }

    void build() {
        list_modules();
        auto& M = E.mods;
        struct Cat { TRef buf; int ch_h, ch_s; };
        std::vector<Cat> cats;
        std::vector<int> skip_ch, skip_res;
        {
            int ch = NF, res = IMG; skip_ch.push_back(NF); skip_res.push_back(IMG);
            for (int l = 0; l < NLEVEL; ++l) {
                for (int b = 0; b < NUM_RES; ++b) { ch = NF * CH_MULT[l]; skip_ch.push_back(ch); skip_res.push_back(res); }
                if (l != NLEVEL - 1) { res /= 2; skip_ch.push_back(ch); skip_res.push_back(res); }
            }
            int sp = (int)skip_ch.size();
            for (int l = NLEVEL - 1; l >= 0; --l) {
                for (int b = 0; b < NUM_RES + 1; ++b) {
                    --sp;
                    Cat c; c.ch_h = ch; c.ch_s = skip_ch[sp];
                    c.buf = new_act(res, c.ch_h + c.ch_s);
                    cats.push_back(c);
                    ch = NF * CH_MULT[l];
                }
                if (l != 0) res *= 2;
            }
        }
        const int P = (int)skip_ch.size();
        auto skip_slot = [&](int i) { const Cat& c = cats[P - 1 - i]; TRef t = c.buf; t.C = c.ch_s; t.coff = c.ch_h; return t; };
        auto h_slot = [&](int j) { const Cat& c = cats[j]; TRef t = c.buf; t.C = c.ch_h; t.coff = 0; return t; };

        for (auto& m : M) if (m.kind == K_RES) dense_total += m.cout;
        dense_w = wres((int64_t)dense_total * TEMB * 2); dense_b = wres((int64_t)dense_total * 4);
        dense_out = arena.alloc((int64_t)dense_total * 4);
        const int64_t emb = arena.alloc(128 * 2), t1 = arena.alloc(TEMB * 2), t2 = arena.alloc(TEMB * 2);

        size_t mi = 0;
        {
            const Mod& m0 = M[mi++]; const Mod& m1 = M[mi++]; (void)m0; (void)m1;
            const int64_t pw0 = take((int64_t)TEMB * NF), pb0 = take(TEMB), pw1 = take((int64_t)TEMB * TEMB), pb1 = take(TEMB);
            const int64_t w0 = wres((int64_t)TEMB * NF * 2), w1 = wres((int64_t)TEMB * TEMB * 2);
            pack_conv(pw0, w0, TEMB, NF, 1, NF, 0, NF); pack_conv(pw1, w1, TEMB, TEMB, 1, TEMB, 0, TEMB);
            const int64_t b0 = pack_f32(pb0, TEMB), b1 = pack_f32(pb1, TEMB);
            const int64_t dw = dense_w, db = dense_b, dout = dense_out; const int dtot = dense_total;
            op(CLS_OTHER, [=](const Ctx& c) {
                hipLaunchKernelGGL(k_time_embed, dim3(grid1d((int64_t)c.B * 128)), dim3(256), 0, c.stream, c.labels, c.at<bf16>(emb), c.B);
            });
            op(CLS_GEMM, [=](const Ctx& c) {
                GemmArgs g = gemm_defaults();
                g.a0 = c.at<bf16>(emb); g.a0_ld = NF; g.a0_C = NF; g.M = c.B; g.N = TEMB;
                g.b = c.w<bf16>(w0); g.b_ld = NF; g.bias_n = c.w<float>(b0); g.act = ACT_SILU;
                g.c = c.at<bf16>(t1); g.c_ld = TEMB;
                launch_gemm(g, c.stream);
                g = gemm_defaults();
                g.a0 = c.at<bf16>(t1); g.a0_ld = TEMB; g.a0_C = TEMB; g.M = c.B; g.N = TEMB;
                g.b = c.w<bf16>(w1); g.b_ld = TEMB; g.bias_n = c.w<float>(b1); g.act = ACT_SILU;
                g.c = c.at<bf16>(t2); g.c_ld = TEMB;
                launch_gemm(g, c.stream);
                g = gemm_defaults();
                g.a0 = c.at<bf16>(t2); g.a0_ld = TEMB; g.a0_C = TEMB; g.M = c.B; g.N = dtot;
                g.b = c.w<bf16>(dw); g.b_ld = TEMB; g.bias_n = c.w<float>(db);
                g.c = c.at<float>(dout); g.c_ld = dtot; g.c_mode = OUT_F32;
                launch_gemm(g, c.stream);
            });
        }
        int si = 0;
        TRef cur = skip_slot(si++);
        {
            const Mod& m = M[mi++];
            const int64_t pw = take((int64_t)NF * 27), pb = take(NF);
            const int64_t w = wres((int64_t)NF * 64 * 2);
            pack_zero(w, (int64_t)NF * 64);
            pack_conv(pw, w, NF, 3, 9, 64, 0, 3);
            const int64_t b = pack_f32(pb, NF);
            const int64_t a0 = arena.alloc((int64_t)IMG * IMG * 64 * 2);
            const TRef dst = cur;
            const Part po = register_output(dst);
            op(CLS_OTHER, [=](const Ctx& c) {
                const int64_t rows = (int64_t)c.B * IMG * IMG;
                hipLaunchKernelGGL(k_stem_im2col, dim3((unsigned)((rows * 8 + 255) / 256)), dim3(256), 0, c.stream, c.x, c.at<bf16>(a0), rows);
            });
            op(CLS_GEMM, [=](const Ctx& c) {
                const int64_t rows = (int64_t)c.B * IMG * IMG;
                GemmArgs g = gemm_defaults();
                g.a0 = c.at<bf16>(a0); g.a0_ld = 64; g.a0_C = 64; g.M = (int)rows; g.N = NF;
                g.b = c.w<bf16>(w); g.b_ld = 64; g.bias_n = c.w<float>(b);
                g.c = c.act(dst); g.c_ld = dst.ld;
                if (po.valid) { g.gn_part = c.at<float>(po.off); g.gn_quads = po.quads; }
                const int bm = launch_gemm(g, c.stream);
                if (po.valid) c.part_bm[po.id] = bm;
            });
            arena.release(a0);
            E.taps[m.idx] = dst;
        }
        int res = IMG;
        for (int l = 0; l < NLEVEL; ++l) {
            for (int b = 0; b < NUM_RES; ++b) {
                const Mod& m = M[mi++];
                const TRef dst = skip_slot(si++);
                if (attn_at(res)) {
                    TRef tmp = new_act(res, m.cout);
                    emit_res(m, cur, tmp);
                    emit_attn(M[mi++], tmp, dst);
                    arena.release(tmp.off);
                } else {
                    emit_res(m, cur, dst);
                }
                cur = dst;
            }
            if (l != NLEVEL - 1) {
                const Mod& m = M[mi++];
                const TRef dst = skip_slot(si++);
                if (ddpm) emit_downconv(m, cur, dst); else emit_res(m, cur, dst);
                cur = dst; res /= 2;
            }
        }
        {
            TRef a = new_act(res, cur.C), b = new_act(res, cur.C);
            emit_res(M[mi++], cur, a);
            emit_attn(M[mi++], a, b);
            arena.release(a.off);
            emit_res(M[mi++], b, h_slot(0));
            arena.release(b.off);
        }
        int j = 0;
        TRef last;
        for (int l = NLEVEL - 1; l >= 0; --l) {
            for (int b = 0; b < NUM_RES + 1; ++b) {
                const Mod& m = M[mi++];
                const bool level_end = b == NUM_RES;
                TRef in = cats[j].buf;
                TRef dst = level_end ? new_act(res, m.cout) : h_slot(j + 1);
                emit_res(m, in, dst);
                arena.release(cats[j].buf.off);
                last = dst; ++j;
            }
            if (attn_at(res)) {
                TRef dst = new_act(res, last.C);
                emit_attn(M[mi++], last, dst);
                arena.release(last.off);
                last = dst;
            }
            if (l != 0) {
                const Mod& m = M[mi++];
                if (ddpm) emit_upconv(m, last, h_slot(j)); else emit_res(m, last, h_slot(j));
                arena.release(last.off);
                res *= 2;
            }
        }
        {
            const Mod& mg = M[mi++]; const Mod& mc = M[mi++];
            const GN gn = take_gn(mg.cin);
            const int64_t pw = take((int64_t)3 * mc.cin * 9), pb = take(3);
            const int Kf = 9 * mc.cin;
            const int64_t w = wres((int64_t)3 * Kf * 2);
            pack_conv(pw, w, 3, mc.cin, 9, Kf, 0, mc.cin);
            const int64_t b = pack_f32(pb, 3);
            int64_t sc = arena.alloc((int64_t)mg.cin * 4), sh = arena.alloc((int64_t)mg.cin * 4);
            const int logW = ilog2(res), cinf = mc.cin;
            if (g_fuse_head && res == HeadConvCfg::RES && mc.cin == HeadConvCfg::C) {
                const int64_t w16 = wres((int64_t)16 * Kf * 2);
                pack_zero(w16, (int64_t)16 * Kf);
                pack_conv(pw, w16, 3, mc.cin, 9, Kf, 0, mc.cin, -0.6931471805599453f);
                emit_gn_stats(last, gn, sc, sh, -1.4426950408889634f);
                const TRef src = last;
                op(CLS_GEMM, [=](const Ctx& c) {
                    if (g_record) { *g_record += gemm_row(c.B * res * res, 3, Kf, 0, 9, 1, "head_conv", 0) + "\n"; return; }
                    hipLaunchKernelGGL(k_head_conv, dim3((unsigned)(c.B * (HeadConvCfg::RES / HeadConvCfg::ROWS))), dim3(256), HeadConvCfg::LDS_BYTES, c.stream,
                                       c.act(src), src.ld, c.at<float>(sc), c.at<float>(sh), c.w<bf16>(w16), c.w<float>(b), c.out);
                });
            } else {
            emit_gn_stats(last, gn, sc, sh);
            TRef u = new_act(res, mg.cin, 1);
            emit_gn_apply(last, sc, sh, u, nullptr, ACT_SILU, RS_NONE);
            op(CLS_GEMM, [=](const Ctx& c) {
                GemmArgs g = gemm_defaults();
                g.a0 = c.act(u); g.a0_ld = u.ld; g.a0_C = cinf; g.taps = 9; g.logW = logW; g.logHW = 2 * logW; g.a0_padded = 1;
                g.M = c.B * res * res; g.N = 3; g.b = c.w<bf16>(w); g.b_ld = Kf; g.bias_n = c.w<float>(b);
                g.c = c.out; g.c_mode = OUT_F32_NCHW;
                launch_gemm(g, c.stream);
            });
            }
            E.taps[mg.idx] = last;
        }
        finish();
        E.part_bm.assign(n_parts > 0 ? n_parts : 1, 128);
        E.fin_done.assign(n_parts > 0 ? n_parts : 1, 0);
    }
};

int64_t module_param_count(const Mod& m) {
    switch (m.kind) {
        case K_LIN: return (int64_t)m.cout * m.cin + m.cout;
        case K_CONV: return (int64_t)m.cout * m.cin * 9 + m.cout;
        case K_GN: return 2 * (int64_t)m.cin;
        case K_DOWN: case K_UP: return (int64_t)m.cout * m.cin * 9 + m.cout;
        case K_ATTN: return 2 * (int64_t)m.cin + 4 * ((int64_t)m.cin * m.cin + m.cin);
        case K_RES: {
            int64_t n = 2 * (int64_t)m.cin + (int64_t)m.cout * m.cin * 9 + m.cout + (int64_t)m.cout * TEMB + m.cout +
                        2 * (int64_t)m.cout + (int64_t)m.cout * m.cout * 9 + m.cout;
            if (m.cin != m.cout || m.up || m.down) n += (int64_t)m.cout * m.cin + m.cout;
            return n;
        }
    }
    return 0;
}

natinf_ncsnpp* make_engine(int flags) {
    natinf_ncsnpp* e = new natinf_ncsnpp();
    e->flags = flags;
    Builder b(*e);
    b.build();
    int64_t off = 0;
    for (auto& m : e->mods) { m.poff = off; off += module_param_count(m); }
    if (off != e->n_params) { delete e; return nullptr; }
    return e;
}

const natinf_ncsnpp& reference_engine() {
    static natinf_ncsnpp* e = [] {
        int* knobs[] = {&g_fuse_gn, &g_fuse_up, &g_fuse_head, &g_fuse_gn8, &g_fuse_gn4, &g_fuse_fin, &g_attn_qkv, &g_attn_proj};
        int saved[sizeof(knobs) / sizeof(knobs[0])];
        for (size_t i = 0; i < sizeof(knobs) / sizeof(knobs[0]); ++i) { saved[i] = *knobs[i]; *knobs[i] = 1; }
        g_fuse_fin = 3;
        natinf_ncsnpp* r = make_engine(0);
        for (size_t i = 0; i < sizeof(knobs) / sizeof(knobs[0]); ++i) *knobs[i] = saved[i];
        return r;
    }();
    return *e;
}

}

extern "C" {

int64_t natinf_ncsnpp_param_count(void) { return reference_engine().n_params; }
int64_t natinf_ncsnpp_packed_bytes(void) { return reference_engine().packed_bytes; }

int64_t natinf_ncsnpp_handle_param_count(natinf_ncsnpp_t h) { return h ? h->n_params : NATINF_EINVAL; }
int64_t natinf_ncsnpp_handle_packed_bytes(natinf_ncsnpp_t h) { return h ? h->packed_bytes : NATINF_EINVAL; }

int64_t natinf_ncsnpp_workspace_bytes(natinf_ncsnpp_t h, int max_batch) {
    if (!h || max_batch <= 0) return NATINF_EINVAL;
    return h->ws_per_image * (int64_t)max_batch;
}

static uint64_t plan_signature() {
    const int k[] = {g_fuse_head, g_attn_qkv, g_attn_w8, g_attn_proj, g_fuse_gn8, g_fuse_fin, g_fuse_gn4, g_fuse_gn, g_cg_wide, g_fuse_up,
                     g_attn_blk , g_cg3 };
    uint64_t h = 1469598103934665603ull;
    for (int v : k) h = (h ^ (uint64_t)(v & 0xff)) * 1099511628211ull;
    return h;
}

int natinf_ncsnpp_create(natinf_ncsnpp_t* out, int flags) {
    if (!out || (flags & ~(NATINF_NCSNPP_KEEP_ACTIVATIONS | NATINF_NCSNPP_DDPM))) return NATINF_EINVAL;
    natinf_ncsnpp* e = make_engine(flags);
    if (!e) return NATINF_ESTATE;
    e->plan_sig = plan_signature();
    *out = e;
    return NATINF_OK;
}

int natinf_ncsnpp_destroy(natinf_ncsnpp_t h) {
    if (!h) return NATINF_EINVAL;
    for (auto& r : h->recs) { (void)hipEventDestroy(r.a); (void)hipEventDestroy(r.b); }
    for (auto e : h->pool) (void)hipEventDestroy(e);
    delete h;
    return NATINF_OK;
}

int natinf_ncsnpp_describe(natinf_ncsnpp_t h, char* buf, int cap) {
    if (!h || !buf || cap <= 0) return NATINF_EINVAL;
    std::string s;
    char line[160];
    for (const auto& m : h->mods) {
        snprintf(line, sizeof(line), "%d %s %d %d %d %d %d %lld\n", m.idx, kind_name(m.kind), m.cin, m.cout, m.up, m.down, m.res,
                 (long long)m.poff);
        s += line;
    }
    if ((int)s.size() + 1 > cap) return NATINF_EINVAL;
    memcpy(buf, s.c_str(), s.size() + 1);
    return (int)s.size();
}

int natinf_ncsnpp_load(natinf_ncsnpp_t h, const float* params_f32, int64_t n_params, void* packed, int64_t packed_bytes,
                       natinf_stream_t stream) {
    return h ? h->load(params_f32, n_params, packed, packed_bytes, (hipStream_t)stream) : NATINF_EINVAL;
}

int natinf_ncsnpp_share(natinf_ncsnpp_t h, natinf_ncsnpp_t loaded) {
    if (!h || !loaded || h == loaded) return NATINF_EINVAL;
    if (!loaded->packed) return NATINF_ESTATE;
    if ((h->flags & NATINF_NCSNPP_DDPM) != (loaded->flags & NATINF_NCSNPP_DDPM) || h->n_params != loaded->n_params || h->packed_bytes != loaded->packed_bytes ||
        h->packs.size() != loaded->packs.size() || h->plan_sig != loaded->plan_sig)
        return NATINF_EINVAL;
    h->packed = loaded->packed;
    return NATINF_OK;
}

int natinf_ncsnpp_forward(natinf_ncsnpp_t h, const float* x, const float* labels, float* out, int B, void* workspace,
                          int64_t workspace_bytes, natinf_stream_t stream) {
    if (!h || !x || !labels || !out || !workspace || B <= 0) return NATINF_EINVAL;
    if (!h->packed) return NATINF_ESTATE;
    if (workspace_bytes < h->ws_per_image * (int64_t)B || (int64_t)B * IMG * IMG >= (1LL << 31)) return NATINF_EINVAL;
    if (!h->configured) {
        if (!configure_gemm_kernels()) return NATINF_ENODEV;
        h->configured = true;
    }
    Ctx c{B, reinterpret_cast<unsigned char*>(workspace), h->packed, (hipStream_t)stream, x, labels, out, h->part_bm.data()};
    c.fin_done = h->fin_done.data();
    g_launch_error = 0;
    if (!h->prof) {
        for (const auto& f : h->ops) f(c);
    } else {
        for (size_t i = 0; i < h->ops.size(); ++i) {
            natinf_ncsnpp::Rec r; r.cls = h->op_cls[i];
            for (hipEvent_t* e : {&r.a, &r.b}) {
                if (!h->pool.empty()) { *e = h->pool.back(); h->pool.pop_back(); }
                else if (hipEventCreate(e) != hipSuccess) return NATINF_ELAUNCH;
            }
            (void)hipEventRecord(r.a, c.stream);
            h->ops[i](c);
            (void)hipEventRecord(r.b, c.stream);
            h->recs.push_back(r);
        }
    }
    h->last_B = B; h->last_ws = c.ws;
    if (g_launch_error) { g_launch_error = 0; return NATINF_ESTATE; }
    return hipGetLastError() == hipSuccess ? NATINF_OK : NATINF_ELAUNCH;
}

int natinf_ncsnpp_describe_gemms(natinf_ncsnpp_t h, int B, char* buf, int cap) {
    if (!h || !buf || cap <= 0 || B <= 0) return NATINF_EINVAL;
    std::string out;
    g_record = &out;
    std::vector<int> scratch_bm(h->part_bm.size(), 128);
    std::vector<unsigned char> scratch_done(h->part_bm.size(), 0);
    Ctx c{B, reinterpret_cast<unsigned char*>(4096), reinterpret_cast<const unsigned char*>(4096), nullptr, nullptr, nullptr, nullptr, scratch_bm.data()};
    c.fin_done = scratch_done.data();
    for (size_t i = 0; i < h->ops.size(); ++i)
        if (h->op_cls[i] == CLS_GEMM || h->op_cls[i] == CLS_CONV_GN || h->op_cls[i] == CLS_CONV_GN8) h->ops[i](c);
    g_record = nullptr;
    if ((int)out.size() + 1 > cap) return NATINF_EINVAL;
    memcpy(buf, out.c_str(), out.size() + 1);
    return (int)out.size();
}

int natinf_debug_gemm(int variant, int M, int N, int K0, int K1, int taps, int logW, int batch,
                      const void* a0, const void* a1, const void* b, const float* bias_n, void* c, int c_f32, float scale,
                      int iters, natinf_stream_t stream) {
    if (variant < 0 || variant >= V_COUNT || !a0 || !b || !c || M <= 0 || N <= 0 || K0 <= 0 || K1 < 0 || iters <= 0 || (taps != 1 && taps != 9)) return NATINF_EINVAL;
    if (K0 % taps || N % 8 || (a1 != nullptr) != (K1 > 0)) return NATINF_EINVAL;
    if (taps == 9 && ((K0 / 9) % BK || logW < 1 || logW > 12 || M % (1 << (2 * logW)) || batch != 1)) return NATINF_EINVAL;
    if (!variant_shipped(variant) || variant == V_CONV_GN || variant == V_FP8_256x256) return NATINF_ESTATE;
#ifndef NATINF_DEV
    if (c_f32 >= 2) return NATINF_ESTATE;
#endif
    static bool configured = false;
    if (!configured) { if (!configure_gemm_kernels()) return NATINF_ENODEV; configured = true; }
    GemmArgs g = gemm_defaults();
    g.a0 = (const bf16*)a0; g.a0_C = K0 / taps; g.a0_ld = g.a0_C; g.taps = taps; g.logW = logW; g.logHW = 2 * logW; g.a0_padded = taps == 9;
    if (a1) { g.a1 = (const bf16*)a1; g.a1_C = K1; g.a1_ld = K1; }
    g.M = M; g.N = N; g.b = (const bf16*)b; g.b_ld = K0 + (a1 ? K1 : 0); g.batch = batch;
    if (batch > 1) { g.a_bs = (int64_t)M * g.a0_ld; g.b_bs = (int64_t)N * g.b_ld; g.c_bs = (int64_t)M * N; }
    g.bias_n = bias_n; g.scale = scale; g.c = c; g.c_ld = N; g.c_mode = c_f32 == 1 ? OUT_F32 : (c_f32 >= 2 ? 100 + c_f32 : OUT_BF16);
    g.dbg_ts = g_dbg_ts;
    g.splitk_ws = g_dbg_splitk_ws; g.splitk_max = g_dbg_splitk_max;
    const int saved = g_force_variant;
    g_force_variant = variant;
    g_launch_error = 0;
    for (int i = 0; i < iters; ++i) launch_gemm(g, (hipStream_t)stream);
    g_force_variant = saved;
    if (g_launch_error) { g_launch_error = 0; return NATINF_EINVAL; }
    return hipGetLastError() == hipSuccess ? NATINF_OK : NATINF_ELAUNCH;
}

int g_dbg_conv_logW = 0; const void* g_dbg_conv_a1 = nullptr; int g_dbg_conv_c1 = 0;
int natinf_debug_set_conv_operand(int logW, const void* a1, int c1) {
    if (logW < 0 || logW > 12 || c1 < 0 || c1 % BK || (c1 > 0) != (a1 != nullptr) || (logW == 0 && a1)) return NATINF_EINVAL;
    g_dbg_conv_logW = logW; g_dbg_conv_a1 = a1; g_dbg_conv_c1 = c1;
    return NATINF_OK;
}

int natinf_debug_gemm_fused(int variant, int M, int N, int K, const void* a, const void* b, const float* bias_n, const float* bias_m,
                            const float* rowvec, const float* gate, int log_rows_per_sample, const void* resid_bf16, const float* resid_f32,
                            float scale, int act, void* c, int c_f32, float* gn_part, int* bm_out, int fp32_slab, natinf_stream_t stream) {
    const int logW = g_dbg_conv_logW, c1 = g_dbg_conv_c1;
    const void* a1 = g_dbg_conv_a1;
    g_dbg_conv_logW = 0; g_dbg_conv_a1 = nullptr; g_dbg_conv_c1 = 0;
    if (variant < 0 || variant >= V_COUNT || !a || !b || !c || M <= 0 || N <= 0 || K <= 0 || c_f32 < 0 || c_f32 > 2) return NATINF_EINVAL;
    if (c_f32 == 2) {
        if (!logW || bias_m || rowvec || gate || resid_bf16 || resid_f32 || gn_part || act != ACT_NONE) return NATINF_EINVAL;
    } else if (N % 8) return NATINF_EINVAL;
    if (logW && (K % 9 || (K / 9) % BK || M % (1 << (2 * logW)))) return NATINF_EINVAL;
    if (!variant_shipped(variant) || variant == V_CONV_GN || variant == V_FP8_256x256) return NATINF_ESTATE;
    if (!configure_gemm_kernels()) return NATINF_ENODEV;
    GemmArgs g = gemm_defaults();
    g.a0 = (const bf16*)a; g.a0_C = K; g.a0_ld = K; g.M = M; g.N = N; g.b = (const bf16*)b; g.b_ld = K;
    if (logW) {
        g.taps = 9; g.a0_C = g.a0_ld = K / 9; g.logW = logW; g.logHW = 2 * logW; g.a0_padded = 1; g.b_ld = K + c1;
        if (a1) { g.a1 = (const bf16*)a1; g.a1_C = g.a1_ld = c1; }
    }
    g.bias_n = bias_n; g.bias_m = bias_m; g.rowvec = rowvec; g.rowvec_ld = N; g.gate = gate; g.gate_ld = N; g.log_rows_per_sample = log_rows_per_sample;
    g.resid = (const bf16*)resid_bf16; g.resid_ld = N; g.resid_f32 = resid_f32; g.resid_f32_ld = N;
    g.scale = scale; g.act = act; g.c = c; g.c_ld = N; g.c_mode = c_f32 == 2 ? OUT_F32_NCHW : (c_f32 ? OUT_F32 : OUT_BF16);
    g.gn_part = gn_part; g.gn_quads = N / 4; g.epi_fp32_slab = fp32_slab != 0;
    g.splitk_ws = g_dbg_splitk_ws; g.splitk_max = g_dbg_splitk_max;
    g.dbg_ts = g_dbg_ts;
    const int saved = g_force_variant;
    g_force_variant = variant;
    g_launch_error = 0;
    const int bm = launch_gemm(g, (hipStream_t)stream);
    g_force_variant = saved;
    if (bm_out) *bm_out = bm;
    if (g_launch_error) { g_launch_error = 0; return NATINF_EINVAL; }
    return hipGetLastError() == hipSuccess ? NATINF_OK : NATINF_ELAUNCH;
}

int g_dbg_cg_up = 0;
int natinf_debug_conv_gn_up(int flags) { if (flags & ~3) return NATINF_EINVAL; g_dbg_cg_up = flags; return NATINF_OK; }
int natinf_debug_conv_gn(int res, int B, int N, int cin, int c1, const void* x, const float* scale, const float* shift, const void* w_packed,
                         void* w_frag, const void* a1, const float* bias_n, const void* resid, float out_scale, void* out, float* gn_part, int iters,
                         natinf_stream_t stream) {
    if ((res != 32 && res != 16 && res != 8 && res != 4) || B <= 0 || N <= 0 || N % 8 || cin <= 0 || cin % 64 || c1 < 0 || c1 % 64 || (c1 > 0) != (a1 != nullptr) ||
        !x || !scale || !shift || !w_packed || !out || iters <= 0) return NATINF_EINVAL;
    static bool configured = false;
    if (!configured) { if (!configure_gemm_kernels()) return NATINF_ENODEV; configured = true; }
    GemmArgs g = gemm_defaults();
    g.a0 = (const bf16*)x; g.a0_ld = cin; g.a0_C = cin; g.taps = 9; g.logW = ilog2(res); g.logHW = 2 * g.logW;
    g.gn_scale = scale; g.gn_shift = shift; g.gn_ld = cin; g.gn_folded = 1;
    if (a1) { g.a1 = (const bf16*)a1; g.a1_ld = c1; g.a1_C = c1; }
    g.M = B * res * res; g.N = N; g.b = (const bf16*)w_packed; g.b_ld = 9 * cin + c1; g.bias_n = bias_n;
    g.resid = (const bf16*)resid; g.resid_ld = N; g.scale = out_scale; g.c = out; g.c_ld = N;
    g.gn_part = gn_part; g.gn_quads = N / 4;
    g.dbg_ts = g_dbg_ts;
    g.a0_up = g_dbg_cg_up & 1; g.a1_up = (a1 && (g_dbg_cg_up & 2)) ? 1 : 0;
    if (w_frag && N % 16 == 0) g.b_frag = (const bf16*)w_frag;
    if (!conv_gn_ok(g)) return NATINF_EINVAL;
    if (g.b_frag) {
        const int64_t n = (int64_t)(N / 16) * (9 * (cin / 32) + c1 / 32) * 64;
        hipLaunchKernelGGL(k_pack_frag, dim3(grid1d(n, 256, 1 << 30)), dim3(256), 0, (hipStream_t)stream, (const bf16*)w_packed, (bf16*)w_frag, N, g.b_ld, cin, c1);
    }
    for (int i = 0; i < iters; ++i) launch_gemm(g, (hipStream_t)stream);
    return hipGetLastError() == hipSuccess ? NATINF_OK : NATINF_ELAUNCH;
}

int natinf_debug_quant_fp8_rows(const float* w, void* q, float* row_scale, int rows, int cols, natinf_stream_t stream) {
    if (!w || !q || !row_scale || rows <= 0 || cols <= 0 || cols % 2) return NATINF_EINVAL;
    hipLaunchKernelGGL(k_pack_fp8_rows, dim3((unsigned)((rows + 3) / 4)), dim3(256), 0, (hipStream_t)stream, w, (uint8_t*)q, row_scale, rows, cols);
    return hipGetLastError() == hipSuccess ? NATINF_OK : NATINF_ELAUNCH;
}

int natinf_debug_gemm_fp8(int M, int N, int K, const void* a8, const float* a_scale, const void* a_mx, const void* b8, const float* b_scale,
                          const float* bias_n, void* c, void* c_mx, int c_mode, int iters, natinf_stream_t stream) {
    if (!a8 || !b8 || !c || M <= 0 || N <= 0 || K <= 0 || K % 128 || N % 8 || iters <= 0) return NATINF_EINVAL;
    static bool configured = false;
    if (!configured) { if (!configure_gemm_kernels()) return NATINF_ENODEV; configured = true; }
    GemmArgs g = gemm_defaults();
    g.a0 = (const bf16*)a8; g.a0_C = K; g.a0_ld = K; g.M = M; g.N = N; g.b = (const bf16*)b8; g.b_ld = K;
    const int act = c_mode >> 8; c_mode &= 0xff;
    if (act != ACT_NONE && act != ACT_GELU_TANH) return NATINF_EINVAL;
    g.deq_m = a_scale; g.deq_n = b_scale; g.bias_n = bias_n; g.c = c; g.c_ld = N; g.c_mode = c_mode; g.act = act;
    g.a_mx = (const uint8_t*)a_mx; g.a_mx_ld = M; g.c_mx = (uint8_t*)c_mx; g.c_mx_ld = M;
    if ((c_mode == OUT_FP8_MX && (!c_mx || N % 32)) || c_mode < 0 || c_mode > OUT_FP8_MX || c_mode == OUT_F32_NCHW) return NATINF_EINVAL;
    for (int i = 0; i < iters; ++i) launch_gemm_fp8(g, (hipStream_t)stream);
    return hipGetLastError() == hipSuccess ? NATINF_OK : NATINF_ELAUNCH;
}

int natinf_debug_timestamps(void* dev_buf16) {
#ifdef NATINF_DEV
    g_dbg_ts = reinterpret_cast<unsigned long long*>(dev_buf16); return NATINF_OK;
#else
    (void)dev_buf16; return NATINF_ESTATE;
#endif
}

int natinf_set_gemm_raster(int rows) { g_raster_g = rows; return NATINF_OK; }
int natinf_set_fuse_gn(int on) { g_fuse_gn = on != 0; return NATINF_OK; }
int natinf_set_fuse_gn8(int on) { g_fuse_gn8 = on != 0; return NATINF_OK; }
int natinf_set_attn256(int on) { return on ? NATINF_OK : NATINF_ESTATE; }
int natinf_set_conv_gn_warm(int mask) { if (mask < 0 || mask > 15) return NATINF_EINVAL; g_cg_warm = mask; return NATINF_OK; }
int natinf_set_attn_block(int on) { g_attn_blk = on < 0 ? ATTN_BLK_DEFAULT : (on > 2 ? 2 : on); return NATINF_OK; }
int natinf_set_attn_qkv(int on) { g_attn_qkv = on != 0; return NATINF_OK; }
int natinf_set_attn_waves8(int on) { g_attn_w8 = on != 0; return NATINF_OK; }
int natinf_set_attn_proj(int on) { g_attn_proj = on != 0; return NATINF_OK; }
int natinf_set_fuse_fin(int on) {
    if (on < 0 || on > 3) return NATINF_EINVAL;
    static const int mask[4] = {0, 3, 1, 2};
    g_fuse_fin = mask[on];
    return NATINF_OK;
}
int natinf_set_gemm_round_model(int on) { g_round_model = on != 0; g_round_model_w128 = on >= 10 ? on : 13; return NATINF_OK; }
int natinf_set_gemm_w128(int on) { g_w128 = on < 0 ? 0 : (on > 2 ? 2 : on); return NATINF_OK; }
int natinf_set_fuse_gn4(int on) { g_fuse_gn4 = on != 0; return NATINF_OK; }
int natinf_set_conv_gn8_tile(int one_image) { return one_image ? NATINF_OK : NATINF_ESTATE; }
int natinf_set_fuse_head(int on) { g_fuse_head = on != 0; return NATINF_OK; }
int natinf_set_conv_gn_w128(int mask) { if (mask < 0 || mask > 7) return NATINF_EINVAL; g_cg3 = mask; return NATINF_OK; }
int natinf_set_conv_gn_w128_min_k(int shape, int k) { if (shape < 0 || shape > 2 || k < 0) return NATINF_EINVAL; g_cg3_min_k[shape] = k; return NATINF_OK; }
int natinf_set_conv_gn_wide(int mask) { if (mask < 0 || mask > 3) return NATINF_EINVAL; g_cg_wide = mask; return NATINF_OK; }
int natinf_set_conv_gn_regw(int on) { return on ? NATINF_OK : NATINF_ESTATE; }
int natinf_set_fuse_up(int on) { g_fuse_up = on != 0; return NATINF_OK; }
int natinf_set_gemm_splitk(int on) { g_splitk = on != 0; return NATINF_OK; }
int natinf_debug_set_splitk_workspace(float* ws, int max_slices) { g_dbg_splitk_ws = ws; g_dbg_splitk_max = ws ? max_slices : 0; return NATINF_OK; }
int natinf_set_gemm_half_issue(int on) { return on ? NATINF_OK : NATINF_ESTATE; }
int natinf_set_gemm_pref512(int on) { g_pref_512 = on != 0; return NATINF_OK; }
int natinf_set_gemm_epilogue(int fp32_slab) { g_epi_fp32_slab = fp32_slab != 0; return NATINF_OK; }

int natinf_set_gemm_variant(int variant) {
    if (variant < 0 || variant >= V_COUNT) return NATINF_EINVAL;
    if (!variant_shipped(variant) || variant == V_CONV_GN || variant == V_FP8_256x256) return NATINF_ESTATE;
    g_force_variant = variant;
    return NATINF_OK;
}

int natinf_gemm_profile(int enable) { g_gemm_prof.on = enable != 0; return NATINF_OK; }
int natinf_gemm_profile_read(char* buf, int cap) {
    if (!buf || cap <= 0) return NATINF_EINVAL;
    std::map<std::string, std::pair<double, int64_t>> by;
    std::vector<std::string> order;
    int rc = NATINF_OK;
    for (auto& e : g_gemm_prof.ev) {
        float ms = 0.f;
        if (hipEventSynchronize(e.b) != hipSuccess || hipEventElapsedTime(&ms, e.a, e.b) != hipSuccess) { (void)hipGetLastError(); rc = NATINF_ELAUNCH; }
        else {
            auto it = by.find(e.tag);
            if (it == by.end()) { order.push_back(e.tag); it = by.emplace(e.tag, std::make_pair(0.0, (int64_t)0)).first; }
            it->second.first += ms; it->second.second += 1;
        }
        g_gemm_prof.pool.emplace_back(e.a, e.b);
    }
    g_gemm_prof.ev.clear();
    if (rc != NATINF_OK) return rc;
    std::string out;
    for (auto& t : order) {
        char tail[64];
        snprintf(tail, sizeof(tail), " %lld %.6f\n", (long long)by[t].second, by[t].first);
        out += t + tail;
    }
    if ((int)out.size() + 1 > cap) return NATINF_EINVAL;
    memcpy(buf, out.c_str(), out.size() + 1);
    return (int)out.size();
}
int natinf_ncsnpp_profile(natinf_ncsnpp_t h, int enable) {
    if (!h) return NATINF_EINVAL;
    h->prof = enable != 0;
    return NATINF_OK;
}

int natinf_ncsnpp_profile_read(natinf_ncsnpp_t h, double* ms_by_class, int64_t* launches_by_class) {
    if (!h || !ms_by_class || !launches_by_class) return NATINF_EINVAL;
    for (int i = 0; i < N_CLS; ++i) { ms_by_class[i] = 0.0; launches_by_class[i] = 0; }
    for (const auto& r : h->recs) {
        float ms = 0.f;
        if (hipEventSynchronize(r.b) != hipSuccess || hipEventElapsedTime(&ms, r.a, r.b) != hipSuccess) {
            (void)hipGetLastError();
            return NATINF_ELAUNCH;
        }
        ms_by_class[r.cls] += ms; launches_by_class[r.cls] += 1;
        h->pool.push_back(r.a); h->pool.push_back(r.b);
    }
    h->recs.clear();
    return NATINF_OK;
}

int natinf_ncsnpp_debug_tap(natinf_ncsnpp_t h, int module_idx, float* out, int64_t capacity_elems, natinf_stream_t stream) {
    if (!h || !out) return NATINF_EINVAL;
    if (!(h->flags & NATINF_NCSNPP_KEEP_ACTIVATIONS) || !h->last_ws) return NATINF_ESTATE;
    auto it = h->taps.find(module_idx);
    if (it == h->taps.end()) return NATINF_EINVAL;
    const TRef& t = it->second;
    const int HW = t.res * t.res;
    const int64_t total = (int64_t)h->last_B * t.C * HW;
    if (capacity_elems < total) return NATINF_EINVAL;
    const bf16* src = reinterpret_cast<const bf16*>(h->last_ws + t.off * h->last_B) + t.coff;
    hipLaunchKernelGGL(k_nhwc_to_nchw_f32, dim3(grid1d(total, 256, 1 << 30)), dim3(256), 0, (hipStream_t)stream, src, t.ld, t.C, HW, out, total);
    return hipGetLastError() == hipSuccess ? NATINF_OK : NATINF_ELAUNCH;
}

}
#include "dit_engine.inc"
#include "mmdit_engine.inc"
#include "vae_engine.inc"
#include "inception_engine.inc"
```

naturaldiffusion_amd/csrc/ncsnpp_kernels.h:

```cpp
#pragma once
#include <hip/hip_runtime.h>
#include <stdint.h>
#include <type_traits>

namespace ncsn {

typedef __bf16 bf16;
typedef __bf16 bf16x8 __attribute__((ext_vector_type(8)));
typedef float f32x4 __attribute__((ext_vector_type(4)));

#ifdef NATINF_ASM_PAD
#define NATINF_PAD_PRE "s_nop 7\n\ts_nop 7\n\t"
#define NATINF_PAD_POST "\n\ts_nop 7\n\ts_nop 7"
#else
#define NATINF_PAD_PRE ""
#define NATINF_PAD_POST ""
#endif

#define NATINF_M0_ASM_BEGIN _Pragma("clang diagnostic push") _Pragma("clang diagnostic ignored \"-Winline-asm\"")
#define NATINF_M0_ASM_END _Pragma("clang diagnostic pop")

__device__ __forceinline__ void lds_poison()
{
#ifdef NATINF_LDS_POISON
    typedef uint32_t poison_u4 __attribute__((ext_vector_type(4)));
    const poison_u4 v = {0x7fc07fc0u, 0x7fc07fc0u, 0x7fc07fc0u, 0x7fc07fc0u};
    for (uint32_t a = threadIdx.x * 16; a < 163840u; a += blockDim.x * 16)
        asm volatile("ds_write_b128 %0, %1" ::"v"(a), "v"(v) : "memory");
    asm volatile("s_waitcnt lgkmcnt(0)" ::: "memory");
    __syncthreads();
#endif
}

constexpr int BM = 128, BN = 128, BK = 64;
constexpr int LDS_ROW = BK;
constexpr int TILE_ELEMS = BM * LDS_ROW;
constexpr int C_ROW = BN + 4;
constexpr int GEMM_LDS_BYTES = BM * C_ROW * 4;
static_assert(4 * TILE_ELEMS * 2 <= GEMM_LDS_BYTES, "tile buffers must fit");

enum { OUT_BF16 = 0, OUT_F32 = 1, OUT_F32_NCHW = 2, OUT_FP8_MX = 3 };
enum { ACT_NONE = 0, ACT_SILU = 1, ACT_GELU_TANH = 2, ACT_RELU = 3 };

struct GemmArgs {
    const bf16* a0; int a0_ld; int a0_C;
    const bf16* a1; int a1_ld; int a1_C;
    int taps; int logW; int logHW;
    int a0_padded;
    int M, N;
    const bf16* b; int b_ld;
    int64_t a_bs, b_bs, c_bs; int batch;
    const float* bias_n; const float* bias_m;
    const float* rowvec; int rowvec_ld; int log_rows_per_sample;
    int z_samples;
    const float* gate; int gate_ld;
    const bf16* resid; int resid_ld;
    const float* resid_f32; int resid_f32_ld;
    float scale; int act;
    const float* deq_m; const float* deq_n; int64_t deq_m_bs, deq_n_bs;
    const uint8_t* a_mx; int a_mx_ld; int64_t a_mx_bs;
    uint8_t* c_mx; int c_mx_ld; int64_t c_mx_bs;
    int raster_g;
    int epi_fp32_slab;
    unsigned long long* dbg_ts;
    void* c; int c_ld; int c_mode;
    float* gn_part; int gn_quads;
    float* fin_scale; float* fin_shift; const float* fin_gamma; const float* fin_beta; int fin_ld; int fin_cg; float fin_mul; float fin_eps;
    const float* gn_scale; const float* gn_shift; int gn_ld; int gn_folded;
    const bf16* b_frag;
    int w_warm;
    int a0_up; int a1_up;
    float* splitk_ws; int splitk_max; int splitk;
    int stream_f16;
};

__device__ __forceinline__ float silu_f(float v) { return v / (1.0f + __expf(-v)); }
__device__ __forceinline__ float silu_fast(float v) { return v * __builtin_amdgcn_rcpf(1.0f + __expf(-v)); }
__device__ __forceinline__ float gelu_tanh_f(float v) {
    const float u = 0.7978845608028654f * (v + 0.044715f * v * v * v);
    const float e = __expf(2.0f * u);
    return 0.5f * v * (2.0f - 2.0f / (e + 1.0f));
}
__device__ __forceinline__ float gelu_tanh_fast(float v) {
    const float t = v * __builtin_fmaf(v * v, -0.10294324f, -2.3022082f);
    return v * __builtin_amdgcn_rcpf(1.0f + __builtin_amdgcn_exp2f(t));
}
__device__ __forceinline__ void pin8(float (&x)[8]) {
    asm volatile("" : "+v"(x[0]), "+v"(x[1]), "+v"(x[2]), "+v"(x[3]), "+v"(x[4]), "+v"(x[5]), "+v"(x[6]), "+v"(x[7]));
}
__device__ __forceinline__ void gelu_tanh_fast8(float (&v)[8]) {
    float t[8];
#pragma unroll
    for (int k = 0; k < 8; ++k) t[k] = v[k] * __builtin_fmaf(v[k] * v[k], -0.10294324f, -2.3022082f);
    pin8(t);
#pragma unroll
    for (int k = 0; k < 8; ++k) t[k] = __builtin_amdgcn_exp2f(t[k]);
    pin8(t);
#pragma unroll
    for (int k = 0; k < 8; ++k) t[k] = 1.0f + t[k];
    pin8(t);
#pragma unroll
    for (int k = 0; k < 8; ++k) t[k] = __builtin_amdgcn_rcpf(t[k]);
    pin8(t);
#pragma unroll
    for (int k = 0; k < 8; ++k) v[k] *= t[k];
}
__device__ __forceinline__ void silu_fast8(float (&v)[8]) {
    float t[8];
#pragma unroll
    for (int k = 0; k < 8; ++k) t[k] = __expf(-v[k]);
    pin8(t);
#pragma unroll
    for (int k = 0; k < 8; ++k) t[k] = 1.0f + t[k];
    pin8(t);
#pragma unroll
    for (int k = 0; k < 8; ++k) t[k] = __builtin_amdgcn_rcpf(t[k]);
    pin8(t);
#pragma unroll
    for (int k = 0; k < 8; ++k) v[k] *= t[k];
}
__device__ __forceinline__ float apply_act(float v, int act) {
    return act == ACT_SILU ? silu_f(v) : (act == ACT_GELU_TANH ? gelu_tanh_f(v) : (act == ACT_RELU ? fmaxf(v, 0.f) : v));
}
__device__ __forceinline__ unsigned mx_scale_of(float amax, float& inv) {
    const unsigned bits = __float_as_uint(amax);
    int e = (int)((bits >> 23) & 0xff) - 127 - 8 + ((bits & 0x7fffff) > 0x600000 ? 1 : 0);
    e = amax > 0.f ? (e < -127 ? -127 : (e > 127 ? 127 : e)) : 0;
    inv = __uint_as_float((unsigned)(127 - e) << 23);
    return (unsigned)(e + 127);
}
__device__ __forceinline__ float group4_max_nonneg(float a) {
    unsigned u = __float_as_uint(a);
    const auto r = __builtin_amdgcn_permlane16_swap(u, u, false, false);
    u = r[0] > r[1] ? r[0] : r[1];
    const auto t = __builtin_amdgcn_permlane32_swap(u, u, false, false);
    u = t[0] > t[1] ? t[0] : t[1];
    return __uint_as_float(u);
}
template <bool CLAMP = true>
__device__ __forceinline__ unsigned pack_fp8x4(float a, float b, float c, float d) {
    if constexpr (CLAMP) {
        a = __builtin_amdgcn_fmed3f(a, -448.f, 448.f); b = __builtin_amdgcn_fmed3f(b, -448.f, 448.f);
        c = __builtin_amdgcn_fmed3f(c, -448.f, 448.f); d = __builtin_amdgcn_fmed3f(d, -448.f, 448.f);
    }
    int w = __builtin_amdgcn_cvt_pk_fp8_f32(a, b, 0, false);
    w = __builtin_amdgcn_cvt_pk_fp8_f32(c, d, w, true);
    return (unsigned)w;
}

__device__ __forceinline__ void apply_act8(float (&v)[8], int act) {
    if (act == ACT_SILU) {
        silu_fast8(v);
    } else if (act == ACT_GELU_TANH) {
        gelu_tanh_fast8(v);
    } else if (act == ACT_RELU) {
#pragma unroll
        for (int q = 0; q < 8; ++q) v[q] = fmaxf(v[q], 0.f);
    }
}

__device__ __forceinline__ void apply_act4(float (&v)[4], int act) {
    if (act == ACT_SILU) {
#pragma unroll
        for (int q = 0; q < 4; ++q) v[q] = v[q] * __builtin_amdgcn_rcpf(1.0f + __expf(-v[q]));
    } else if (act == ACT_GELU_TANH) {
#pragma unroll
        for (int q = 0; q < 4; ++q) v[q] = gelu_tanh_fast(v[q]);
    } else if (act == ACT_RELU) {
#pragma unroll
        for (int q = 0; q < 4; ++q) v[q] = fmaxf(v[q], 0.f);
    }
}

__device__ __forceinline__ void tile_coords(int tile, int nM, int nN, int g, int& mt, int& nt) {
    if (g > 1) {
        const int per = g * nN, grp = tile / per, r = tile - grp * per, rows = min(g, nM - grp * g);
        nt = r / rows; mt = grp * g + (r - nt * rows);
    } else { mt = tile / nN; nt = tile - mt * nN; }
}

__device__ __forceinline__ int xcd_remap(int bid, int n) {
    const int q = n >> 3, r = n & 7, x = bid & 7, l = bid >> 3;
    return (x < r ? x * (q + 1) : r * (q + 1) + (x - r) * q) + l;
}

__device__ __forceinline__ void gemm_epilogue(const GemmArgs& g, unsigned char* smem, f32x4 (&acc)[4][4],
                                              int m0, int n0, int z, int tid, int lane, int wm, int wn)
{
    float* sC = reinterpret_cast<float*>(smem);
#pragma unroll
    for (int i = 0; i < 4; ++i)
#pragma unroll
        for (int j = 0; j < 4; ++j)
#pragma unroll
            for (int r = 0; r < 4; ++r)
                sC[(wm * 64 + i * 16 + (lane >> 4) * 4 + r) * C_ROW + wn * 64 + j * 16 + (lane & 15)] = acc[i][j][r];
    __syncthreads();

    if (g.c_mode == OUT_F32_NCHW) {
        float* out = reinterpret_cast<float*>(g.c);
        const int nvalid = min(BN, g.N - n0);
        for (int e = tid; e < BM * nvalid; e += 256) {
            const int r = e & (BM - 1), n = e >> 7;
            const int m = m0 + r;
            if (m < g.M) {
                float v = sC[r * C_ROW + n];
                if (g.bias_n) v += g.bias_n[n0 + n];
                v *= g.scale;
                const int b = m >> g.logHW, p = m & ((1 << g.logHW) - 1);
                out[((int64_t)b * g.N + n0 + n) * ((int64_t)1 << g.logHW) + p] = v;
            }
        }
        return;
    }

    const int cchunk = tid & 15;
    const int n = n0 + cchunk * 8;
    const bool n_in = n < g.N;
    float bn[8];
#pragma unroll
// ... 80 lines not shown
    const int nk0 = (K0 + BK - 1) / BK, nk1 = (K1 + BK - 1) / BK, nk = nk0 + nk1;

    const int colc = tid & 7;
    const int row0 = tid >> 3;
    int a_y[4], a_x[4];
    int64_t a_off0[4], a_off1[4], b_off[4];
    bool a_ok[4], b_ok[4];
    const int Wd = 1 << g.logW, Hd = 1 << (g.logHW - g.logW);
    const int Wa = g.a0_padded ? Wd + 2 : Wd;
#pragma unroll
    for (int i = 0; i < 4; ++i) {
        const int m = m0 + row0 + 32 * i;
        a_ok[i] = m < g.M;
        const int p = m & ((1 << g.logHW) - 1);
        a_y[i] = p >> g.logW; a_x[i] = p & (Wd - 1);
        a_off0[i] = g.a0_padded ? ((int64_t)((m >> g.logHW) * (Hd + 2) + a_y[i] + 1) * Wa + a_x[i] + 1) * g.a0_ld : (int64_t)m * g.a0_ld;
        a_off1[i] = (int64_t)m * g.a1_ld;
        const int n = n0 + row0 + 32 * i;
        b_ok[i] = n < g.N;
        b_off[i] = (int64_t)n * g.b_ld;
    }

    uint4 ra[4], rb[4];
    auto load_tile = [&](int kt) __attribute__((always_inline)) {
        if (kt < nk0) {
            const int kbase = kt * BK;
            int tap = 0, c0 = kbase;
            if (g.taps == 9) { const int cch = kt / 9; tap = kt - 9 * cch; c0 = cch * BK; }
            const int dy = g.taps == 9 ? tap / 3 - 1 : 0, dx = g.taps == 9 ? tap % 3 - 1 : 0;
            const int cc = c0 + colc * 8;
            const bool kin = cc < (g.taps == 9 ? g.a0_C : K0);
            const int64_t shift = (int64_t)(dy * Wa + dx) * g.a0_ld + cc;
#pragma unroll
            for (int i = 0; i < 4; ++i) {
                const bool ok = a_ok[i] && kin && (unsigned)(a_y[i] + dy) < (unsigned)Hd && (unsigned)(a_x[i] + dx) < (unsigned)Wd;
                ra[i] = ld_or_zero(ok ? a0 + a_off0[i] + shift : a0, ok);
            }
        } else {
            const int cc = (kt - nk0) * BK + colc * 8;
            const bool kin = cc < K1;
#pragma unroll
            for (int i = 0; i < 4; ++i)
                ra[i] = ld_or_zero((a_ok[i] && kin) ? a1 + a_off1[i] + cc : a1, a_ok[i] && kin);
        }
        {
            const int kk = (kt < nk0 ? kt * BK : K0 + (kt - nk0) * BK) + colc * 8;
            const bool kin = kt < nk0 ? (kk < K0) : (kk < K0 + K1);
#pragma unroll
            for (int i = 0; i < 4; ++i)
                rb[i] = ld_or_zero((b_ok[i] && kin) ? bp + b_off[i] + kk : bp, b_ok[i] && kin);
        }
    };
    auto store_tile = [&](int buf) __attribute__((always_inline)) {
        bf16* da = sA + buf * TILE_ELEMS;
        bf16* db = sB + buf * TILE_ELEMS;
#pragma unroll
        for (int i = 0; i < 4; ++i) {
            const int r = row0 + 32 * i;
            const int o = r * LDS_ROW + ((colc ^ ((r >> 1) & 7)) << 3);
            *reinterpret_cast<uint4*>(da + o) = ra[i];
            *reinterpret_cast<uint4*>(db + o) = rb[i];
        }
    };

    f32x4 acc[4][4];
#pragma unroll
    for (int i = 0; i < 4; ++i)
#pragma unroll
        for (int j = 0; j < 4; ++j) acc[i][j] = f32x4{0.f, 0.f, 0.f, 0.f};

    load_tile(0);
    store_tile(0);
    __syncthreads();

    const int frow = lane & 15, fq = lane >> 4, fswz = (frow >> 1) & 7;
    for (int kt = 0; kt < nk; ++kt) {
        const int cur = kt & 1;
        if (kt + 1 < nk) load_tile(kt + 1);
        const bf16* ta = sA + cur * TILE_ELEMS + (wm * 64 + frow) * LDS_ROW;
        const bf16* tb = sB + cur * TILE_ELEMS + (wn * 64 + frow) * LDS_ROW;
#pragma unroll
        for (int ks = 0; ks < 2; ++ks) {
            bf16x8 fa[4], fb[4];
            const int ko = (((ks << 2) | fq) ^ fswz) << 3;
#pragma unroll
            for (int i = 0; i < 4; ++i) {
                fa[i] = *reinterpret_cast<const bf16x8*>(ta + i * 16 * LDS_ROW + ko);
                fb[i] = *reinterpret_cast<const bf16x8*>(tb + i * 16 * LDS_ROW + ko);
            }
#pragma unroll
            for (int i = 0; i < 4; ++i)
#pragma unroll
                for (int j = 0; j < 4; ++j)
                    acc[i][j] = __builtin_amdgcn_mfma_f32_16x16x32_bf16(fa[i], fb[j], acc[i][j], 0, 0, 0);
        }
        if (kt + 1 < nk) store_tile(cur ^ 1);
        __syncthreads();
    }

    gemm_epilogue(g, smem, acc, m0, n0, z, tid, lane, wm, wn);
}

__global__ __launch_bounds__(256) void k_gn_stats(const bf16* __restrict__ x, int ld, int C, int HW,
                                                  const float* __restrict__ gamma, const float* __restrict__ beta,
                                                  float* __restrict__ scale, float* __restrict__ shift, float eps, float out_mul)
{
    __shared__ float s_part[2][16 * 128 + 64];
    __shared__ float s_sum[512], s_sq[512], s_mean[32], s_rstd[32];
    lds_poison();
    const int tid = threadIdx.x, b = blockIdx.x;
    const int cpp = C >> 3;
    const int lanes = 256 / cpp;
    if (tid < cpp * lanes) {
        const int chunk = tid % cpp, pl = tid / cpp;
        float s[8], q[8];
#pragma unroll
        for (int i = 0; i < 8; ++i) { s[i] = 0.f; q[i] = 0.f; }
        const bf16* base = x + (int64_t)b * HW * ld + chunk * 8;
        for (int p = pl; p < HW; p += lanes) {
            const bf16x8 v = *reinterpret_cast<const bf16x8*>(base + (int64_t)p * ld);
#pragma unroll
            for (int i = 0; i < 8; ++i) { const float f = (float)v[i]; s[i] += f; q[i] += f * f; }
        }
#pragma unroll
        for (int i = 0; i < 8; ++i) { s_part[0][pl * C + chunk * 8 + i] = s[i]; s_part[1][pl * C + chunk * 8 + i] = q[i]; }
    }
    __syncthreads();
    for (int c = tid; c < C; c += 256) {
        float s = 0.f, q = 0.f;
        for (int l = 0; l < lanes; ++l) { s += s_part[0][l * C + c]; q += s_part[1][l * C + c]; }
        s_sum[c] = s; s_sq[c] = q;
    }
    __syncthreads();
    const int cg = C >> 5;
    if (tid < 32) {
        float s = 0.f, q = 0.f;
        for (int i = 0; i < cg; ++i) { s += s_sum[tid * cg + i]; q += s_sq[tid * cg + i]; }
        const float inv = 1.0f / (float)(cg * HW);
        const float mean = s * inv;
        float var = q * inv - mean * mean;
        var = var < 0.f ? 0.f : var;
        s_mean[tid] = mean;
        s_rstd[tid] = 1.0f / sqrtf(var + eps);
    }
    __syncthreads();
    for (int c = tid; c < C; c += 256) {
        const int gi = c / cg;
        const float sc = s_rstd[gi] * gamma[c];
        scale[(int64_t)b * C + c] = sc * out_mul;
        shift[(int64_t)b * C + c] = (beta[c] - s_mean[gi] * sc) * out_mul;
    }
}

__global__ __launch_bounds__(256) void k_gn_finalize(const float2* __restrict__ P0, int tps0, int quads0,
                                                     const float2* __restrict__ P1, int tps1, int quads1, int C, int HW,
                                                     const float* __restrict__ gamma, const float* __restrict__ beta,
                                                     float* __restrict__ scale, float* __restrict__ shift, float eps, float out_mul)
{
    __shared__ float2 s_p[128];
    lds_poison();
    const int tid = threadIdx.x, b = blockIdx.x, nq = quads0 + quads1;
    float ga[2] = {0.f, 0.f}, be[2] = {0.f, 0.f};
#pragma unroll
    for (int k = 0; k < 2; ++k) {
        const int c = tid + 256 * k;
        if (c < C) { ga[k] = gamma[c]; be[k] = beta[c]; }
    }
    for (int q = tid; q < nq; q += 256) {
        const bool first = q < quads0;
        const float2* P = first ? P0 + (int64_t)b * tps0 * quads0 + q : P1 + (int64_t)b * tps1 * quads1 + (q - quads0);
        const int tps = first ? tps0 : tps1, st = first ? quads0 : quads1;
        float s = 0.f, qq = 0.f;
        int t = 0;
        for (; t + 4 <= tps; t += 4) {
            const float2 v0 = P[(int64_t)t * st], v1 = P[(int64_t)(t + 1) * st], v2 = P[(int64_t)(t + 2) * st], v3 = P[(int64_t)(t + 3) * st];
            s += v0.x; qq += v0.y; s += v1.x; qq += v1.y; s += v2.x; qq += v2.y; s += v3.x; qq += v3.y;
        }
        for (; t < tps; ++t) { const float2 v = P[(int64_t)t * st]; s += v.x; qq += v.y; }
        s_p[q] = make_float2(s, qq);
    }
    __syncthreads();
    const int cg = C >> 5, qpg = cg >> 2;
    const float inv = 1.0f / (float)(cg * HW);
#pragma unroll
    for (int k = 0; k < 2; ++k) {
        const int c = tid + 256 * k;
        if (c >= C) break;
        const int gi = c / cg;
        float s = 0.f, q = 0.f;
        for (int i = 0; i < qpg; ++i) { const float2 v = s_p[gi * qpg + i]; s += v.x; q += v.y; }
        const float mean = s * inv;
        float var = q * inv - mean * mean;
        var = var < 0.f ? 0.f : var;
        const float sc = (1.0f / sqrtf(var + eps)) * ga[k];
        scale[(int64_t)b * C + c] = sc * out_mul;
        shift[(int64_t)b * C + c] = (be[k] - mean * sc) * out_mul;
    }
}

enum { RS_NONE = 0, RS_UP = 1, RS_DOWN = 2 };
constexpr int GN_ROWS = 4;
#ifndef GN_UNROLL
#define GN_UNROLL 4
#endif
__global__ __launch_bounds__(256) void k_gn_apply(const bf16* __restrict__ x, int ld, int C, int logW, int logHW,
                                                  const float* __restrict__ scale, const float* __restrict__ shift,
                                                  bf16* __restrict__ y, bf16* __restrict__ xr, int act, int mode, int pad)
{
    const int cpp = C >> 3, lanes = 256 / cpp;
    const int chunk = threadIdx.x % cpp, pl = threadIdx.x / cpp;
    if (pl >= lanes) return;
    const int Ws = 1 << logW, Hs = 1 << (logHW - logW);
    const int Wd = mode == RS_UP ? 2 * Ws : (mode == RS_DOWN ? Ws >> 1 : Ws);
    const int Hd = mode == RS_UP ? 2 * Hs : (mode == RS_DOWN ? Hs >> 1 : Hs);
    const int Wp = Wd + 2 * pad, Hp = Hd + 2 * pad;
    const int b = blockIdx.y, row0 = blockIdx.x * GN_ROWS;
    const int nrows = min(GN_ROWS, Hp - row0);
    float sc[8], sh[8];
    {
        const float* ps = scale + (int64_t)b * C + chunk * 8;
        const float* ph = shift + (int64_t)b * C + chunk * 8;
        const float4 s0 = *reinterpret_cast<const float4*>(ps), s1 = *reinterpret_cast<const float4*>(ps + 4);
        const float4 h0 = *reinterpret_cast<const float4*>(ph), h1 = *reinterpret_cast<const float4*>(ph + 4);
        sc[0] = s0.x; sc[1] = s0.y; sc[2] = s0.z; sc[3] = s0.w; sc[4] = s1.x; sc[5] = s1.y; sc[6] = s1.z; sc[7] = s1.w;
        sh[0] = h0.x; sh[1] = h0.y; sh[2] = h0.z; sh[3] = h0.w; sh[4] = h1.x; sh[5] = h1.y; sh[6] = h1.z; sh[7] = h1.w;
    }
    const bf16* xb = x + (int64_t)b * Hs * Ws * ld + chunk * 8;
    bf16* yb = y + ((int64_t)b * Hp + row0) * Wp * C + chunk * 8;
    bf16* xrb = xr ? xr + (int64_t)b * Hd * Wd * C + chunk * 8 : nullptr;
    int rr = 0, xx = pl;
    while (xx >= Wp) { xx -= Wp; ++rr; }
    auto advance = [&](int& r, int& c) __attribute__((always_inline)) { c += lanes; while (c >= Wp) { c -= Wp; ++r; } };
    auto interior = [&](int r, int c) __attribute__((always_inline)) {
        const int Y = row0 + r - pad, X = c - pad;
        return r < nrows && Y >= 0 && Y < Hd && X >= 0 && X < Wd;
    };
    auto finish = [&](int r, int c, bool in, const bf16x8& v) __attribute__((always_inline)) {
        if (r >= nrows) return;
        bf16x8 o;
        if (!in) {
#pragma unroll
            for (int q = 0; q < 8; ++q) o[q] = (bf16)0.0f;
        } else {
#pragma unroll
            for (int q = 0; q < 8; ++q) {
                float f = (float)v[q] * sc[q] + sh[q];
                if (act == ACT_SILU) f = silu_fast(f);
                o[q] = (bf16)f;
            }
            if (xrb) *reinterpret_cast<bf16x8*>(xrb + ((int64_t)(row0 + r - pad) * Wd + (c - pad)) * C) = v;
        }
        *reinterpret_cast<bf16x8*>(yb + ((int64_t)r * Wp + c) * C) = o;
    };
    if (mode != RS_DOWN) {
        const int sh_ = mode == RS_UP ? 1 : 0;
        constexpr int U = GN_UNROLL;
        while (rr < nrows) {
            int r[U], c[U];
            bool in[U];
            bf16x8 v[U];
            r[0] = rr; c[0] = xx;
#pragma unroll
            for (int u = 1; u < U; ++u) { r[u] = r[u - 1]; c[u] = c[u - 1]; advance(r[u], c[u]); }
#pragma unroll
            for (int u = 0; u < U; ++u) {
                in[u] = interior(r[u], c[u]);
                if (in[u]) v[u] = *reinterpret_cast<const bf16x8*>(xb + ((int64_t)((row0 + r[u] - pad) >> sh_) * Ws + ((c[u] - pad) >> sh_)) * ld);
            }
#pragma unroll
            for (int u = 0; u < U; ++u) finish(r[u], c[u], in[u], v[u]);
            rr = r[U - 1]; xx = c[U - 1];
            advance(rr, xx);
        }
        return;
    }
    for (; rr < nrows; ) {
        const int Y = row0 + rr - pad, X = xx - pad;
        bf16x8 o;
        if (Y < 0 || Y >= Hd || X < 0 || X >= Wd) {
#pragma unroll
            for (int q = 0; q < 8; ++q) o[q] = (bf16)0.0f;
        } else {
            float ay[8], ax[8];
#pragma unroll
            for (int q = 0; q < 8; ++q) { ay[q] = 0.f; ax[q] = 0.f; }
#pragma unroll
            for (int d = 0; d < 4; ++d) {
                const bf16x8 v = *reinterpret_cast<const bf16x8*>(xb + ((int64_t)(2 * Y + (d >> 1)) * Ws + 2 * X + (d & 1)) * ld);
#pragma unroll
                for (int q = 0; q < 8; ++q) {
                    const float raw = (float)v[q];
                    float f = raw * sc[q] + sh[q];
                    if (act == ACT_SILU) f = silu_fast(f);
                    ay[q] += f; ax[q] += raw;
                }
            }
            bf16x8 ox;
#pragma unroll
            for (int q = 0; q < 8; ++q) { o[q] = (bf16)(ay[q] * 0.25f); ox[q] = (bf16)(ax[q] * 0.25f); }
            if (xrb) *reinterpret_cast<bf16x8*>(xrb + ((int64_t)Y * Wd + X) * C) = ox;
        }
        *reinterpret_cast<bf16x8*>(yb + ((int64_t)rr * Wp + xx) * C) = o;
        xx += lanes;
        while (xx >= Wp) { xx -= Wp; ++rr; }
    }
}

__global__ __launch_bounds__(256) void k_softmax_rows(const float* __restrict__ S, bf16* __restrict__ P, int T, int64_t rows)
{
    const int lane = threadIdx.x & 63;
    const int64_t row = (int64_t)blockIdx.x * 4 + (threadIdx.x >> 6);
    if (row >= rows) return;
    const float* s = S + row * T;
    float v[4];
    float mx = -INFINITY;
#pragma unroll
    for (int i = 0; i < 4; ++i) {
        const int c = lane + 64 * i;
        v[i] = c < T ? s[c] : -INFINITY;
        mx = fmaxf(mx, v[i]);
    }
#pragma unroll
    for (int o = 32; o > 0; o >>= 1) mx = fmaxf(mx, __shfl_xor(mx, o));
    float sum = 0.f;
#pragma unroll
    for (int i = 0; i < 4; ++i) { v[i] = (lane + 64 * i < T) ? __expf(v[i] - mx) : 0.f; sum += v[i]; }
#pragma unroll
    for (int o = 32; o > 0; o >>= 1) sum += __shfl_xor(sum, o);
    const float inv = 1.0f / sum;
#pragma unroll
    for (int i = 0; i < 4; ++i) {
        const int c = lane + 64 * i;
        if (c < T) P[row * T + c] = (bf16)(v[i] * inv);
    }
}

__global__ void k_time_embed(const float* __restrict__ labels, bf16* __restrict__ emb, int B)
{
    const int i = blockIdx.x * blockDim.x + threadIdx.x;
    if (i >= B * 128) return;
    const int b = i >> 7, j = i & 127, h = j & 63;
    const float freq = expf((float)h * -(9.210340371976184f / 63.0f));
    const float a = labels[b] * freq;
    emb[i] = (bf16)(j < 64 ? sinf(a) : cosf(a));
}

__global__ __launch_bounds__(256) void k_stem_im2col(const float* __restrict__ x, bf16* __restrict__ A, int64_t rows)
{
    const int64_t idx = (int64_t)blockIdx.x * 256 + threadIdx.x;
// ... 76 lines not shown
```

Baseline: 3412 images/s.

## Fold GroupNorm finalize into producer epilogues for concat inputs and attention blocks

Extends the in-epilogue GroupNorm finalize so each producer can write scale/shift into up to two tables, with a channel offset. This lets concatenated skip+hidden buffers and the fused 256x256 attention block emit normalized stats directly, instead of launching a separate k_gn_finalize kernel per GroupNorm. The goal is fewer small launches and less partial-sum traffic per forward. The cost is extra epilogue work and register pressure in the GEMM and attention kernels, plus per-concat scale tables in the arena. It also adds debug counters and table readback APIs.

```diff
diff --git a/include/natinf_ncsnpp.h b/include/natinf_ncsnpp.h
--- a/include/natinf_ncsnpp.h
+++ b/include/natinf_ncsnpp.h
@@ -65,6 +65,10 @@
 int natinf_set_fuse_gn8(int on);
 int natinf_set_fuse_gn4(int on);
 int natinf_set_fuse_fin(int on);
+int natinf_set_fin_all(int on);
+int natinf_ncsnpp_count_gn_finalize(natinf_ncsnpp_t h, int B);
+int natinf_ncsnpp_gn_table_count(natinf_ncsnpp_t h);
+int natinf_ncsnpp_debug_gn_table(natinf_ncsnpp_t h, int i, float* out, int64_t capacity_elems, natinf_stream_t stream);
 int natinf_set_conv_gn_warm(int mask);
 int natinf_set_attn256(int on);
 int natinf_set_attn_proj(int on);
diff --git a/naturaldiffusion_amd/_lib.py b/naturaldiffusion_amd/_lib.py
--- a/naturaldiffusion_amd/_lib.py
+++ b/naturaldiffusion_amd/_lib.py
@@ -74,6 +74,10 @@
     "natinf_set_fuse_gn8": (C.c_int, [_i32]),
     "natinf_set_fuse_gn4": (C.c_int, [_i32]),
     "natinf_set_fuse_fin": (C.c_int, [_i32]),
+    "natinf_set_fin_all": (C.c_int, [_i32]),
+    "natinf_ncsnpp_count_gn_finalize": (C.c_int, [_p, _i32]),
+    "natinf_ncsnpp_gn_table_count": (C.c_int, [_p]),
+    "natinf_ncsnpp_debug_gn_table": (C.c_int, [_p, _i32, _p, _i64, _p]),
     "natinf_set_attn_proj": (C.c_int, [_i32]),
     "natinf_set_attn_waves8": (C.c_int, [_i32]),
     "natinf_set_attn_qkv": (C.c_int, [_i32]),
diff --git a/naturaldiffusion_amd/csrc/attn_blk256.h b/naturaldiffusion_amd/csrc/attn_blk256.h
--- a/naturaldiffusion_amd/csrc/attn_blk256.h
+++ b/naturaldiffusion_amd/csrc/attn_blk256.h
@@ -343,7 +343,8 @@
 
 __global__ __launch_bounds__(512, 1) void k_attn_blk256_v2(const bf16* __restrict__ x, int x_ld, const float* __restrict__ gsc, const float* __restrict__ gsh,
                                                           const bf16* __restrict__ wqf, const float* __restrict__ cq, float scale, const bf16* __restrict__ wvof,
-                                                          const float* __restrict__ bo, bf16* __restrict__ o, int o_ld, float out_scale, float2* __restrict__ gn_part, int gn_quads)
+                                                          const float* __restrict__ bo, bf16* __restrict__ o, int o_ld, float out_scale, float2* __restrict__ gn_part, int gn_quads,
+                                                          FinTab fin0, FinTab fin1, float fin_eps)
 {
     constexpr int T = 256, C = 256, NTQ = 8;
     extern __shared__ __attribute__((aligned(16))) unsigned char smem[];
@@ -599,6 +600,24 @@
 #pragma unroll
             for (int w = 0; w < 8; ++w) { s += sred[w * 64 + tid].x; ss += sred[w * 64 + tid].y; }
             gn_part[(int64_t)b * gn_quads + tid] = make_float2(s, ss);
+            sred[512 + tid] = make_float2(s, ss);
+        }
+        if (fin0.scale || fin1.scale) {
+            __syncthreads();
+            if (tid < 256) {
+#pragma unroll
+                for (int f = 0; f < 2; ++f) {
+                    const FinTab& ft = f ? fin1 : fin0;
+                    if (!ft.scale) continue;
+                    const int cg = ft.cg, qpg = cg >> 2, cn = ft.coff + tid, q0 = ((cn / cg) * cg - ft.coff) >> 2;
+                    float s = 0.f, ss = 0.f;
+                    for (int i = 0; i < qpg; ++i) { const float2 v = sred[512 + q0 + i]; s += v.x; ss += v.y; }
+                    float sc, sh;
+                    gn_scale_shift(s, ss, 1.0f / (float)(cg * 256), ft.gamma[cn], ft.beta[cn], fin_eps, ft.mul, sc, sh);
+                    ft.scale[(int64_t)b * ft.ld + cn] = sc;
+                    ft.shift[(int64_t)b * ft.ld + cn] = sh;
+                }
+            }
         }
     }
 }
diff --git a/naturaldiffusion_amd/csrc/gemm_dma.h b/naturaldiffusion_amd/csrc/gemm_dma.h
--- a/naturaldiffusion_amd/csrc/gemm_dma.h
+++ b/naturaldiffusion_amd/csrc/gemm_dma.h
@@ -312,29 +312,32 @@
         if constexpr (FIN) {
             static_assert((WM == 1 || NSAMP == 1) && BN_ <= THREADS, "one channel per thread; several samples per tile: one wave row");
             const int n = n0 + tid;
-            if (g.fin_scale && tid < BN_ && n < g.N) {
-                constexpr int HWS = BM_ / NSAMP;
-                const int cg = g.fin_cg, qpg = cg >> 2, q0 = (n / cg) * qpg - (n0 >> 2);
-                const float inv = 1.0f / (float)(cg * HWS), ga = g.fin_gamma[n], be = g.fin_beta[n];
-#pragma unroll
-                for (int sm = 0; sm < NSAMP; ++sm) {
-                    if (m0 + sm * HWS >= g.M) break;
-                    float s = 0.f, qq = 0.f;
-                    for (int i = 0; i < qpg; ++i) {
-                        if constexpr (NSAMP == 1 && WM > 1) {
-                            float ps = 0.f, pq = 0.f;
-#pragma unroll
-                            for (int w = 0; w < WM; ++w) { ps += sred[w * (BN_ / 4) + q0 + i].x; pq += sred[w * (BN_ / 4) + q0 + i].y; }
-                            s += ps; qq += pq;
-                        } else { const float2 v = sred[sm * (BN_ / 4) + q0 + i]; s += v.x; qq += v.y; }
+            if (tid < BN_ && n < g.N) {
+#pragma unroll
+                for (int f = 0; f < 2; ++f) {
+                    const FinTab& ft = g.fin[f];
+                    if (!ft.scale) continue;
+                    constexpr int HWS = BM_ / NSAMP;
+                    const int cg = ft.cg, qpg = cg >> 2, cn = ft.coff + n, q0 = ((cn / cg) * cg - ft.coff - n0) >> 2;
+                    const float inv = 1.0f / (float)(cg * HWS), ga = ft.gamma[cn], be = ft.beta[cn];
+#pragma unroll
+                    for (int sm = 0; sm < NSAMP; ++sm) {
+                        if (m0 + sm * HWS >= g.M) break;
+                        float s = 0.f, qq = 0.f;
+                        for (int i = 0; i < qpg; ++i) {
+                            if constexpr (NSAMP == 1 && WM > 1) {
+                                float ps = 0.f, pq = 0.f;
+#pragma unroll
+                                for (int w = 0; w < WM; ++w) { ps += sred[w * (BN_ / 4) + q0 + i].x; pq += sred[w * (BN_ / 4) + q0 + i].y; }
+                                s += ps; qq += pq;
+                            } else { const float2 v = sred[sm * (BN_ / 4) + q0 + i]; s += v.x; qq += v.y; }
+                        }
+                        float sc, sh;
+                        gn_scale_shift(s, qq, inv, ga, be, g.fin_eps, ft.mul, sc, sh);
+                        const int64_t o = (int64_t)(m0 / HWS + sm) * ft.ld + cn;
+                        ft.scale[o] = sc;
+                        ft.shift[o] = sh;
                     }
-                    const float mean = s * inv;
-                    float var = qq * inv - mean * mean;
-                    var = var < 0.f ? 0.f : var;
-                    const float sc = (1.0f / sqrtf(var + g.fin_eps)) * ga;
-                    const int64_t o = (int64_t)(m0 / HWS + sm) * g.fin_ld + n;
-                    g.fin_scale[o] = sc * g.fin_mul;
-                    g.fin_shift[o] = (be - mean * sc) * g.fin_mul;
                 }
             }
         }
diff --git a/naturaldiffusion_amd/csrc/gemm_launch.h b/naturaldiffusion_amd/csrc/gemm_launch.h
--- a/naturaldiffusion_amd/csrc/gemm_launch.h
+++ b/naturaldiffusion_amd/csrc/gemm_launch.h
@@ -370,6 +370,7 @@
         return 256;
     }
     if (g_record) {
+        if (v == V_CONV_GN) g_fin_written = conv_gn3_shape(g) == 2 && g.fin[0].scale && (conv_gn_epi(g) == 2 || conv_gn_epi(g) == 6) && g.N == 256;
         record_gemm(g, v == V_CONV_GN && conv_gn3_shape(g) >= 0 ? "conv_gn3" : variant_name(v), v == V_CONV_GN ? conv_gn_epi(g) : effective_epi(v, g));
         return v == V_CONV_GN ? conv_gn_part_rows(g) : variant_bm(v);
     }
@@ -382,7 +383,7 @@
         const int e = conv_gn_epi(gw);
         if (const int sh3 = conv_gn3_shape(gw); sh3 >= 0) {
             ncsn_cg3::launch(&gw, sh3, e, (void*)s);
-            g_fin_written = sh3 == 2 && gw.fin_scale && (e == 2 || e == 6) && gw.N == 256;
+            g_fin_written = sh3 == 2 && gw.fin[0].scale && (e == 2 || e == 6) && gw.N == 256;
         } else launch_conv_gn2(ConvGnShapes{}, 1 << gw.logW, conv_gn_bm(gw), e, gw, s);
         return conv_gn_part_rows(gw);
     } else with_family(v, [&](auto f) { launch_family<decltype(f)>(effective_epi(v, g), g, s); });
diff --git a/naturaldiffusion_amd/csrc/ncsnpp.hip b/naturaldiffusion_amd/csrc/ncsnpp.hip
--- a/naturaldiffusion_amd/csrc/ncsnpp.hip
+++ b/naturaldiffusion_amd/csrc/ncsnpp.hip
@@ -40,6 +40,8 @@
 int g_attn_proj = 1;
 int g_fuse_gn8 = 1;
 int g_fuse_fin = 3;
+int g_fin_all = 1;
+thread_local int g_fin_launches = 0;
 int g_fuse_gn4 = 1;
 int g_fuse_gn = 1;
 int g_fuse_up = 1;
@@ -58,6 +60,9 @@
     uint64_t plan_sig = 0;
     int last_B = 0; unsigned char* last_ws = nullptr;
     std::vector<unsigned char> fin_done;
+    std::vector<unsigned char> op_fin;
+    struct GnTab { int64_t sc, sh; int C; };
+    std::vector<GnTab> gn_tabs;
 };
 
 namespace {
@@ -83,7 +88,7 @@
         arena.keep = (e.flags & NATINF_NCSNPP_KEEP_ACTIVATIONS) != 0;
     }
 
-    void op(int cls, OpFn f) { E.ops.push_back(std::move(f)); E.op_cls.push_back(cls); }
+    void op(int cls, OpFn f, bool fin = false) { E.ops.push_back(std::move(f)); E.op_cls.push_back(cls); E.op_fin.push_back(fin); }
 
     void pack_conv(int64_t src, int64_t dst, int N, int Cin, int taps, int dst_ld, int koff, int tapstride, float wmul = 1.0f) {
         const int chunked = taps == 9 && Cin % BK == 0;
@@ -117,7 +122,8 @@
     GN take_gn(int C) { GN g; g.gamma = pack_f32(take(C), C); g.beta = pack_f32(take(C), C); return g; }
 
     void emit_gn_stats(const TRef& x, GN gn, int64_t& sc, int64_t& sh, float out_mul = 1.0f) {
-        if (emit_gn_from_parts(x, gn, sc, sh, out_mul)) return;
+        if (emit_gn_from_parts(x, gn, sc, sh, out_mul)) { E.gn_tabs.push_back({sc, sh, x.C}); return; }
+        E.gn_tabs.push_back({sc, sh, x.C});
         const int HW = x.res * x.res;
         op(CLS_OTHER, [=](const Ctx& c) {
             hipLaunchKernelGGL(k_gn_stats, dim3(c.B), dim3(256), 0, c.stream, c.act(x), x.ld, x.C, HW,
@@ -206,7 +212,8 @@
             if (pt.fin && pt.fin->check) c.fin_done[pt.id] = g_fin_written;
         });
         if (!fuse) arena.release(h.off);
-        int64_t sc1 = own_sc, sh1 = own_sh;
+        const int64_t own_sc1 = arena.keep ? arena.alloc((int64_t)cout * 4) : own_sc, own_sh1 = arena.keep ? arena.alloc((int64_t)cout * 4) : own_sh;
+        int64_t sc1 = own_sc1, sh1 = own_sh1;
         emit_gn_stats(t, gn1, sc1, sh1, gn_mul1);
         TRef u;
         if (!fuse1) {
@@ -241,7 +248,7 @@
         if ((m.up || m.down) && !fuse_up) arena.release(xr.off);
         arena.release(own_sc); arena.release(own_sh);
         if (sc != own_sc) { arena.release(sc); arena.release(sh); }
-        if (sc1 != own_sc) { arena.release(sc1); arena.release(sh1); }
+        if (sc1 != own_sc1) { arena.release(sc1); arena.release(sh1); }
         E.taps[m.idx] = out;
     }
 
@@ -324,16 +331,18 @@
                 hipLaunchKernelGGL(k_pack_attn_w3, dim3(256), dim3(256), 0, p.stream, (const float*)fvp, reinterpret_cast<bf16*>(p.packed + wv_));
             });
         }
-        const Part po_attn = proj ? register_output(out) : Part();
+        const Part po_attn = proj ? register_output(out, false, blk2 && T == 256 && C == 256) : Part();
         const float rs_attn = res_scale;
         TRef O = new_act(m.res, C);
         if (T == 256 && C == 256) {
             op(CLS_GEMM, [=](const Ctx& c) {
+                FinTab ft[2] = {};
+                if (blk2 && po_attn.fin) fill_fin(ft, *po_attn.fin, c);
                 if (g_record) return;
                 if (blk2) {
                     hipLaunchKernelGGL(k_attn_blk256_v2, dim3((unsigned)c.B), dim3(512), ABLK2_LDS_BYTES, c.stream, (const bf16*)c.act(x), x.ld, c.at<float>(sc_q), c.at<float>(sh_q),
                                        c.w<bf16>(wqf2), c.w<float>(cq2), 1.0f / sqrtf((float)C), c.w<bf16>(wvof2), c.w<float>(bo2),
-                                       c.act(out), out.ld, rs_attn, po_attn.valid ? c.at<float2>(po_attn.off) : (float2*)nullptr, po_attn.quads);
+                                       c.act(out), out.ld, rs_attn, po_attn.valid ? c.at<float2>(po_attn.off) : (float2*)nullptr, po_attn.quads, ft[0], ft[1], GN_EPS);
                     if (po_attn.valid) c.part_bm[po_attn.id] = 256;
                 } else if (blk) {
                     hipLaunchKernelGGL(k_attn_blk256, dim3((unsigned)c.B), dim3(512), ABLK_LDS_BYTES, c.stream, (const bf16*)c.act(x), x.ld, c.at<float>(sc_q), c.at<float>(sh_q),
@@ -472,14 +481,21 @@
 
     int dense_rows_next = 0;
 
-    struct Fin { int64_t sc = -1, sh = -1, gamma = -1, beta = -1; int C = 0; float out_mul = 1.0f; bool claimed = false, check = false; };
+    struct FinSlot { int64_t sc = -1, sh = -1, gamma = -1, beta = -1; int ld = 0, coff = 0; float out_mul = 1.0f; };
+    struct Fin { int64_t sc = -1, sh = -1; int C = 0, n = 0; FinSlot slot[2]; bool claimed = false, check = false; };
     struct Part { int64_t off = -1; int quads = 0, id = -1, res = 0; bool valid = false; std::shared_ptr<Fin> fin; };
+    static void fill_fin(FinTab* t, const Fin& f, const Ctx& c) {
+        for (int i = 0; i < f.n; ++i) {
+            const FinSlot& s = f.slot[i];
+            t[i].scale = c.at<float>(s.sc); t[i].shift = c.at<float>(s.sh); t[i].gamma = c.w<float>(s.gamma); t[i].beta = c.w<float>(s.beta);
+            t[i].ld = s.ld; t[i].coff = s.coff; t[i].cg = s.ld / 32; t[i].mul = s.out_mul;
+        }
+    }
     static void set_fin(GemmArgs& g, const Part& p, const Ctx& c) {
-        if (!p.fin || !p.fin->claimed) return;
-        const Fin& f = *p.fin;
-        g.fin_scale = c.at<float>(f.sc); g.fin_shift = c.at<float>(f.sh); g.fin_gamma = c.w<float>(f.gamma); g.fin_beta = c.w<float>(f.beta);
-        g.fin_ld = f.C; g.fin_cg = f.C / 32; g.fin_mul = f.out_mul; g.fin_eps = GN_EPS;
-    }
+        if (!p.fin) return;
+        fill_fin(g.fin, *p.fin, c); g.fin_eps = GN_EPS;
+    }
+    std::map<int64_t, std::pair<int64_t, int64_t>> cat_tab;
     std::map<std::pair<int64_t, int>, Part> parts;
     int n_parts = 0;
     static bool fusable(int res) { return res >= 16; }
@@ -488,7 +504,7 @@
         p.off = arena.alloc((int64_t)std::max(res * res / 64, 1) * p.quads * 8);
         return p;
     }
-    Part register_output(const TRef& out, bool fused8 = false) {
+    Part register_output(const TRef& out, bool fused8 = false, bool attn_blk = false) {
         Part p;
         if (fusable(out.res) || (out.res <= 8 && fused8)) p = new_part(out.res, out.C);
         if (p.valid && out.res <= 8 && fused8 && (g_fuse_fin & 1) && out.C == 256) {
@@ -498,6 +514,10 @@
         if (p.valid && out.res == 16 && fused8 && (g_fuse_fin & 2) && out.C == 256 && !ddpm) {
             p.fin = std::make_shared<Fin>();
             p.fin->sc = arena.alloc((int64_t)out.C * 4); p.fin->sh = arena.alloc((int64_t)out.C * 4); p.fin->C = out.C; p.fin->check = true;
+        }
+        if (p.valid && attn_blk && g_fin_all && (g_fuse_fin & 2) && out.res == 16 && out.C == 256 && !ddpm) {
+            p.fin = std::make_shared<Fin>();
+            p.fin->sc = arena.alloc((int64_t)out.C * 4); p.fin->sh = arena.alloc((int64_t)out.C * 4); p.fin->C = out.C;
         }
         parts[{out.off, out.coff}] = p;
         return p;
@@ -514,28 +534,48 @@
         if (ch != x.C || src.empty() || src.size() > 2) return false;
         const Part p0 = src[0], p1 = src.size() > 1 ? src[1] : Part();
         const int HW = x.res * x.res, C = x.C;
-        if (src.size() == 1 && p0.fin && !p0.fin->claimed && p0.fin->C == C) {
-            Fin& f = *p0.fin;
-            f.gamma = gn.gamma; f.beta = gn.beta; f.out_mul = out_mul; f.claimed = true;
-            sc = f.sc; sh = f.sh;
-            if (f.check) {
-                const std::shared_ptr<Fin> fp = p0.fin;
-                const int64_t fsc = f.sc, fsh = f.sh;
-                op(CLS_OTHER, [=](const Ctx& c) {
-                    if (c.fin_done[p0.id]) return;
-                    hipLaunchKernelGGL(k_gn_finalize, dim3(c.B), dim3(256), 0, c.stream, c.at<float2>(p0.off), HW / c.part_bm[p0.id], p0.quads, (const float2*)nullptr, 0, 0, C, HW,
-                                       c.w<float>(gn.gamma), c.w<float>(gn.beta), c.at<float>(fsc), c.at<float>(fsh), GN_EPS, out_mul);
-                });
-            }
-            return true;
-        }
-        const int64_t sc_ = sc, sh_ = sh;
-        op(CLS_OTHER, [=](const Ctx& c) {
+        auto finalize = [=](const Ctx& c, int64_t sc_, int64_t sh_) {
+            if (g_record) { ++g_fin_launches; return; }
             const int tps0 = HW / c.part_bm[p0.id], tps1 = p1.valid ? HW / c.part_bm[p1.id] : 0;
             hipLaunchKernelGGL(k_gn_finalize, dim3(c.B), dim3(256), 0, c.stream, c.at<float2>(p0.off), tps0, p0.quads,
                                p1.valid ? c.at<float2>(p1.off) : (const float2*)nullptr, tps1, p1.valid ? p1.quads : 0, C, HW,
                                c.w<float>(gn.gamma), c.w<float>(gn.beta), c.at<float>(sc_), c.at<float>(sh_), GN_EPS, out_mul);
-        });
+        };
+        auto add_slot = [&](Fin& f, int64_t tsc, int64_t tsh, int coff) {
+            FinSlot& sl = f.slot[f.n++];
+            sl.sc = tsc; sl.sh = tsh; sl.gamma = gn.gamma; sl.beta = gn.beta; sl.ld = C; sl.coff = coff; sl.out_mul = out_mul;
+        };
+        if (src.size() == 1 && p0.fin && !p0.fin->claimed && p0.fin->n < 2 && p0.fin->C == C) {
+            Fin& f = *p0.fin;
+            add_slot(f, f.sc, f.sh, 0); f.claimed = true;
+            sc = f.sc; sh = f.sh;
+            if (f.check) {
+                const int64_t fsc = f.sc, fsh = f.sh;
+                op(CLS_OTHER, [=](const Ctx& c) {
+                    if (c.fin_done[p0.id]) return;
+                    finalize(c, fsc, fsh);
+                }, true);
+            }
+            return true;
+        }
+        if (g_fin_all && src.size() == 2 && p0.fin && p1.fin && p0.fin->n < 2 && p1.fin->n < 2 && (p0.quads * 4) % (C / 32) == 0 && (C / 32) % 4 == 0) {
+            auto it = cat_tab.find(x.off);
+            if (it != cat_tab.end() && it->second.first >= 0) {
+                const int64_t tsc = it->second.first, tsh = it->second.second;
+                it->second.first = -1;
+                add_slot(*p0.fin, tsc, tsh, 0); add_slot(*p1.fin, tsc, tsh, p0.quads * 4);
+                sc = tsc; sh = tsh;
+                const bool ck0 = p0.fin->check, ck1 = p1.fin->check;
+                if (ck0 || ck1)
+                    op(CLS_OTHER, [=](const Ctx& c) {
+                        if ((!ck0 || c.fin_done[p0.id]) && (!ck1 || c.fin_done[p1.id])) return;
+                        finalize(c, tsc, tsh);
+                    }, true);
+                return true;
+            }
+        }
+        const int64_t sc_ = sc, sh_ = sh;
+        op(CLS_OTHER, [=](const Ctx& c) { finalize(c, sc_, sh_); }, true);
         return true;
     }
 
@@ -582,6 +622,7 @@
                     --sp;
                     Cat c; c.ch_h = ch; c.ch_s = skip_ch[sp];
                     c.buf = new_act(res, c.ch_h + c.ch_s);
+                    if (g_fin_all) { const int64_t tsc = arena.alloc((int64_t)(c.ch_h + c.ch_s) * 4); cat_tab[c.buf.off] = {tsc, arena.alloc((int64_t)(c.ch_h + c.ch_s) * 4)}; }
                     cats.push_back(c);
                     ch = NF * CH_MULT[l];
                 }
@@ -808,7 +849,7 @@
 }
 
 static uint64_t plan_signature() {
-    const int k[] = {g_fuse_head, g_attn_qkv, g_attn_w8, g_attn_proj, g_fuse_gn8, g_fuse_fin, g_fuse_gn4, g_fuse_gn, g_cg_wide, g_fuse_up,
+    const int k[] = {g_fuse_head, g_attn_qkv, g_attn_w8, g_attn_proj, g_fuse_gn8, g_fuse_fin, g_fin_all, g_fuse_gn4, g_fuse_gn, g_cg_wide, g_fuse_up,
                      g_attn_blk , g_cg3 };
     uint64_t h = 1469598103934665603ull;
     for (int v : k) h = (h ^ (uint64_t)(v & 0xff)) * 1099511628211ull;
@@ -907,6 +948,21 @@
     if ((int)out.size() + 1 > cap) return NATINF_EINVAL;
     memcpy(buf, out.c_str(), out.size() + 1);
     return (int)out.size();
+}
+
+int natinf_ncsnpp_count_gn_finalize(natinf_ncsnpp_t h, int B) {
+    if (!h || B <= 0) return NATINF_EINVAL;
+    std::string out;
+    g_record = &out;
+    g_fin_launches = 0;
+    std::vector<int> scratch_bm(h->part_bm.size(), 128);
+    std::vector<unsigned char> scratch_done(h->part_bm.size(), 0);
+    Ctx c{B, reinterpret_cast<unsigned char*>(4096), reinterpret_cast<const unsigned char*>(4096), nullptr, nullptr, nullptr, nullptr, scratch_bm.data()};
+    c.fin_done = scratch_done.data();
+    for (size_t i = 0; i < h->ops.size(); ++i)
+        if (h->op_cls[i] == CLS_GEMM || h->op_cls[i] == CLS_CONV_GN || h->op_cls[i] == CLS_CONV_GN8 || h->op_fin[i]) h->ops[i](c);
+    g_record = nullptr;
+    return g_fin_launches;
 }
 
 int natinf_debug_gemm(int variant, int M, int N, int K0, int K1, int taps, int logW, int batch,
@@ -1053,6 +1109,7 @@
     g_fuse_fin = mask[on];
     return NATINF_OK;
 }
+int natinf_set_fin_all(int on) { g_fin_all = on != 0; return NATINF_OK; }
 int natinf_set_gemm_round_model(int on) { g_round_model = on != 0; g_round_model_w128 = on >= 10 ? on : 13; return NATINF_OK; }
 int natinf_set_gemm_w128(int on) { g_w128 = on < 0 ? 0 : (on > 2 ? 2 : on); return NATINF_OK; }
 int natinf_set_fuse_gn4(int on) { g_fuse_gn4 = on != 0; return NATINF_OK; }
@@ -1140,6 +1197,18 @@
     return hipGetLastError() == hipSuccess ? NATINF_OK : NATINF_ELAUNCH;
 }
 
+int natinf_ncsnpp_gn_table_count(natinf_ncsnpp_t h) { return h ? (int)h->gn_tabs.size() : NATINF_EINVAL; }
+int natinf_ncsnpp_debug_gn_table(natinf_ncsnpp_t h, int i, float* out, int64_t capacity_elems, natinf_stream_t stream) {
+    if (!h || !out || i < 0 || i >= (int)h->gn_tabs.size()) return NATINF_EINVAL;
+    if (!(h->flags & NATINF_NCSNPP_KEEP_ACTIVATIONS) || !h->last_ws) return NATINF_ESTATE;
+    const auto& t = h->gn_tabs[i];
+    const int64_t n = (int64_t)h->last_B * t.C;
+    if (capacity_elems < 2 * n) return NATINF_EINVAL;
+    if (hipMemcpyAsync(out, h->last_ws + t.sc * h->last_B, n * 4, hipMemcpyDeviceToDevice, (hipStream_t)stream) != hipSuccess ||
+        hipMemcpyAsync(out + n, h->last_ws + t.sh * h->last_B, n * 4, hipMemcpyDeviceToDevice, (hipStream_t)stream) != hipSuccess) return NATINF_ELAUNCH;
+    return t.C;
+}
+
 }
 #include "dit_engine.inc"
 #include "mmdit_engine.inc"
diff --git a/naturaldiffusion_amd/csrc/ncsnpp_kernels.h b/naturaldiffusion_amd/csrc/ncsnpp_kernels.h
--- a/naturaldiffusion_amd/csrc/ncsnpp_kernels.h
+++ b/naturaldiffusion_amd/csrc/ncsnpp_kernels.h
@@ -41,6 +41,8 @@
 
 enum { OUT_BF16 = 0, OUT_F32 = 1, OUT_F32_NCHW = 2, OUT_FP8_MX = 3 };
 enum { ACT_NONE = 0, ACT_SILU = 1, ACT_GELU_TANH = 2, ACT_RELU = 3 };
+
+struct FinTab { float* scale; float* shift; const float* gamma; const float* beta; int ld; int coff; int cg; float mul; };
 
 struct GemmArgs {
     const bf16* a0; int a0_ld; int a0_C;
@@ -65,7 +67,7 @@
     unsigned long long* dbg_ts;
     void* c; int c_ld; int c_mode;
     float* gn_part; int gn_quads;
-    float* fin_scale; float* fin_shift; const float* fin_gamma; const float* fin_beta; int fin_ld; int fin_cg; float fin_mul; float fin_eps;
+    FinTab fin[2]; float fin_eps;
     const float* gn_scale; const float* gn_shift; int gn_ld; int gn_folded;
     const bf16* b_frag;
     int w_warm;
@@ -452,6 +454,16 @@
     }
 }
 
+__device__ __forceinline__ void gn_scale_shift(float s, float q, float inv, float ga, float be, float eps, float out_mul, float& scale, float& shift)
+{
+    const float mean = s * inv;
+    float var = q * inv - mean * mean;
+    var = var < 0.f ? 0.f : var;
+    const float sc = (1.0f / sqrtf(var + eps)) * ga;
+    scale = sc * out_mul;
+    shift = (be - mean * sc) * out_mul;
+}
+
 __global__ __launch_bounds__(256) void k_gn_finalize(const float2* __restrict__ P0, int tps0, int quads0,
                                                      const float2* __restrict__ P1, int tps1, int quads1, int C, int HW,
                                                      const float* __restrict__ gamma, const float* __restrict__ beta,
@@ -489,12 +501,10 @@
         const int gi = c / cg;
         float s = 0.f, q = 0.f;
         for (int i = 0; i < qpg; ++i) { const float2 v = s_p[gi * qpg + i]; s += v.x; q += v.y; }
-        const float mean = s * inv;
-        float var = q * inv - mean * mean;
-        var = var < 0.f ? 0.f : var;
-        const float sc = (1.0f / sqrtf(var + eps)) * ga[k];
-        scale[(int64_t)b * C + c] = sc * out_mul;
-        shift[(int64_t)b * C + c] = (be[k] - mean * sc) * out_mul;
+        float sc, sh;
+        gn_scale_shift(s, q, inv, ga[k], be[k], eps, out_mul, sc, sh);
+        scale[(int64_t)b * C + c] = sc;
+        shift[(int64_t)b * C + c] = sh;
     }
 }
 
```

After: 3414 images/s, median of 2. Within noise of the previous version (+0.0%).
